# nschloe/flow

Measured on AMD Instinct MI355X. Metric: ipcs_time_steps_per_sec, higher is better.
Workload: dtype f64

## Files before the change

flow_amd/_hip.py:

```python
import ctypes
import os

import torch

from . import device

_HERE = os.path.dirname(os.path.abspath(__file__))
LIB_PATH = os.path.join(_HERE, 'csrc', 'libflow_hip.so')

REDUCE_WORK = 4096
MULTI_DOT_BLOCKS = 1024
GMRES_MAX_RESTART = 30
GMRES_PARTIALS = (GMRES_MAX_RESTART + 2) * 1024
GMRES_STATE = 1280
SPMV_ROWS_PER_BLOCK = 256
SPMV_NNZ_PER_BLOCK = 1022
PMG_NNZ_PER_BLOCK = 2044

c_double_p = ctypes.c_void_p
c_int_p = ctypes.c_void_p


class Operator(ctypes.Structure):
    _fields_ = [
# ... 38 lines not shown
        ('n', ctypes.c_int),
        ('nc', ctypes.c_int),
        ('agg_ptr', ctypes.c_void_p),
        ('agg_dofs', ctypes.c_void_p),
        ('agg_of', ctypes.c_void_p),
        ('lda', ctypes.c_int),
        ('Ainv', ctypes.c_void_p),
        ]


MG_MAX_LEVELS = 8


class MgS(ctypes.Structure):
    _fields_ = [
        ('nlevels', ctypes.c_int),
        ('Ah', Operator * MG_MAX_LEVELS),
        ('dinv', ctypes.c_void_p * MG_MAX_LEVELS),
        ('Ps', Operator * MG_MAX_LEVELS),
        ('R', Operator * MG_MAX_LEVELS),
        ('r', ctypes.c_void_p * MG_MAX_LEVELS),
        ('x', ctypes.c_void_p * MG_MAX_LEVELS),
        ('t', ctypes.c_void_p * MG_MAX_LEVELS),
        ('nc', ctypes.c_int), ('lda', ctypes.c_int),
        ('Ainv', ctypes.c_void_p),
        ('omega', ctypes.c_double),
        ('C', Operator * MG_MAX_LEVELS),
        ('up_rowblocks', ctypes.c_void_p * MG_MAX_LEVELS),
        ('up_nblocks', ctypes.c_int * MG_MAX_LEVELS),
        ]


class IluPlanS(ctypes.Structure):
    _fields_ = [
        ('n', ctypes.c_int), ('nnz', ctypes.c_int), ('ncolors', ctypes.c_int),
        ('nnz_l', ctypes.c_int), ('nnz_u', ctypes.c_int),
        ('off_l', ctypes.c_int), ('off_u', ctypes.c_int),
        ('off_d', ctypes.c_int), ('lu_size', ctypes.c_int),
        ('max_row', ctypes.c_int), ('nslices', ctypes.c_int),
        ('color_ptr_host', ctypes.c_void_p),
        ('slice_ptr_host', ctypes.c_void_p),
        ('rowptr', ctypes.c_void_p), ('cols', ctypes.c_void_p),
        ('diag', ctypes.c_void_p), ('src_pos', ctypes.c_void_p),
        ('old_of_new', ctypes.c_void_p), ('new_of_old', ctypes.c_void_p),
        ('slice_row', ctypes.c_void_p),
        ('l_slice_off', ctypes.c_void_p), ('l_cols', ctypes.c_void_p),
        ('l_pos', ctypes.c_void_p),
        ('u_slice_off', ctypes.c_void_p), ('u_cols', ctypes.c_void_p),
        ('u_pos', ctypes.c_void_p),
        ]


class IluS(ctypes.Structure):
    _fields_ = [
        ('plan', ctypes.POINTER(IluPlanS)),
        ('nblocks', ctypes.c_int),
        ('lu', ctypes.c_void_p),
        ('packed', ctypes.c_void_p),
        ('single_vector', ctypes.c_int),
        ('cycle', ctypes.c_void_p),
        ]


class TlS(ctypes.Structure):
    _fields_ = [
        ('fine', ctypes.POINTER(IluS)), ('coarse', ctypes.POINTER(IluS)),
        ('fine_op', ctypes.c_void_p), ('coarse_op', ctypes.c_void_p),
        ('pre', ctypes.c_int), ('post', ctypes.c_int),
        ('coarse_sweeps', ctypes.c_int),
        ('ends', ctypes.c_void_p), ('rptr', ctypes.c_void_p),
        ('rsrc', ctypes.c_void_p),
        ('bc_fine', ctypes.c_void_p), ('bc_coarse', ctypes.c_void_p),
        ('rscale', ctypes.c_void_p), ('work', ctypes.c_void_p),
        ]


class PmgLevelS(ctypes.Structure):
    _fields_ = [
        ('n', ctypes.c_int), ('nnz', ctypes.c_int), ('nblocks', ctypes.c_int),
        ('rowptr', ctypes.c_void_p), ('cols', ctypes.c_void_p),
        ('rowblocks', ctypes.c_void_p),
        ('vals', ctypes.c_void_p), ('diag', ctypes.c_void_p),
        ('dinv', ctypes.c_void_p),
        ('lam_min', ctypes.c_double), ('lam_max', ctypes.c_double),
        ('cols16', ctypes.c_void_p), ('cbase', ctypes.c_void_p),
        ('packed', ctypes.c_void_p), ('idrows', ctypes.c_void_p),
        ]


class PmgS(ctypes.Structure):
    _fields_ = [
        ('fine', PmgLevelS), ('coarse', PmgLevelS),
        ('pre', ctypes.c_int), ('post', ctypes.c_int),
        ('coarse_steps', ctypes.c_int),
        ('ends', ctypes.c_void_p),
        ('rptr', ctypes.c_void_p), ('rsrc', ctypes.c_void_p),
        ('bc_fine', ctypes.c_void_p), ('bc_coarse', ctypes.c_void_p),
        ('work', ctypes.c_void_p),
        ('scalar', ctypes.c_int),
        ]


class MassS(ctypes.Structure):
    _fields_ = [
        ('A', ctypes.POINTER(Operator)),
        ('dinv', ctypes.c_void_p),
        ('nblocks16', ctypes.c_int),
        ('rowblocks16', ctypes.c_void_p),
        ('vals16', ctypes.c_void_p),
        ('lam_min', ctypes.c_double), ('lam_max', ctypes.c_double),
        ('steps', ctypes.c_int),
        ('contraction', ctypes.c_double),
        ('work16', ctypes.c_void_p),
        ('packed16', ctypes.c_void_p),
        ('cbase16', ctypes.c_void_p),
        ('work16_rows', ctypes.c_int),
        ]


class MassStripsS(ctypes.Structure):
    _fields_ = [
        ('nlevels', ctypes.c_int),
        ('rowblocks16', ctypes.c_void_p * 16),
        ('nblocks16', ctypes.c_int * 16),
        ('row_lo_last', ctypes.c_int), ('row_hi_last', ctypes.c_int),
        ]


class MeshS(ctypes.Structure):
    _fields_ = [('nc', ctypes.c_int), ('xy', ctypes.c_void_p),
                ('c0', ctypes.c_int), ('c1', ctypes.c_int)]


class SpaceS(ctypes.Structure):
    _fields_ = [
        ('deg', ctypes.c_int),
        ('n', ctypes.c_int),
        ('nnz', ctypes.c_int),
        ('cell_dofs', ctypes.c_void_p),
        ('cptr', ctypes.c_void_p),
        ('csrc', ctypes.c_void_p),
        ('vptr', ctypes.c_void_p),
        ('vsrc', ctypes.c_void_p),
        ('r0', ctypes.c_int), ('r1', ctypes.c_int),
        ('nnz0', ctypes.c_int), ('nnz1', ctypes.c_int),
        ]


class CoefS(ctypes.Structure):
    _fields_ = [
        ('nl', ctypes.c_int),
        ('cell_stride', ctypes.c_int),
        ('values', ctypes.c_void_p),
        ('G', ctypes.c_void_p),
        ]


FORM_MAX_PROGRAM = 64
FORM_REGISTERS = 8
FORM_MAX_CONSTANTS = 32
FORM_MAX_FIELDS = 6
FORM_MAX_EXPRESSIONS = 4
FORM_MAX_POINTS = 256
FORM_SLOTS = 9
FORM_NEWTON_SLOTS = 12
PROFILE_CURVES_PER_LAUNCH = 32


class FormS(ctypes.Structure):
    _fields_ = [
        ('nprog', ctypes.c_int),
        ('prog', ctypes.c_int * (4 * FORM_MAX_PROGRAM)),
        ('nconst', ctypes.c_int),
        ('consts', ctypes.c_double * FORM_MAX_CONSTANTS),
        ('nfield', ctypes.c_int),
        ('field', ctypes.c_void_p * FORM_MAX_FIELDS),
        ('field_deg', ctypes.c_int * FORM_MAX_FIELDS),
        ('cell_dofs', ctypes.c_void_p * 2),
        ('nexpr', ctypes.c_int),
        ('expr', ctypes.c_void_p * FORM_MAX_EXPRESSIONS),
        ('expr_nl', ctypes.c_int * FORM_MAX_EXPRESSIONS),
        ('expr_table', ctypes.c_int * FORM_MAX_EXPRESSIONS),
        ('nq', ctypes.c_int),
        ('rule', ctypes.c_void_p),
        ('tables', ctypes.c_void_p),
        ('ntables', ctypes.c_int),
        ('nout', ctypes.c_int),
        ]


class PointGridS(ctypes.Structure):
    _fields_ = [
        ('nx', ctypes.c_int), ('ny', ctypes.c_int),
        ('x0', ctypes.c_double), ('y0', ctypes.c_double),
        ('hx_inv', ctypes.c_double), ('hy_inv', ctypes.c_double),
        ('start', ctypes.c_void_p),
        ('cells', ctypes.c_void_p),
        ]


STATS_MAX_FREQ = 8
STATS_COVARIANCE = 1
STATS_EXTREMA = 2


class StatsFreq(ctypes.Structure):
    _fields_ = [
        ('n', ctypes.c_int),
        ('c', ctypes.c_double * STATS_MAX_FREQ),
        ('s', ctypes.c_double * STATS_MAX_FREQ),
        ]


ISOLINE_LEVELS_PER_LAUNCH = 32


class IsolineLevels(ctypes.Structure):
    _fields_ = [
        ('n', ctypes.c_int),
        ('base', ctypes.c_int),
        ('c', ctypes.c_double * ISOLINE_LEVELS_PER_LAUNCH),
        ]


class NsParams(ctypes.Structure):
    _fields_ = [
        ('dt', ctypes.c_double), ('rho', ctypes.c_double),
        ('mu', ctypes.c_double), ('theta_i', ctypes.c_double),
        ('theta_e', ctypes.c_double),
        ]


ALLREDUCE_FN = ctypes.CFUNCTYPE(ctypes.c_int, ctypes.c_void_p, ctypes.c_int)


class PeerS(ctypes.Structure):
    _fields_ = [
        ('flags', ctypes.c_void_p), ('land', ctypes.c_void_p),
        ('land_cap', ctypes.c_int), ('spin_limit', ctypes.c_int),
        ('nb_flags', ctypes.c_void_p * 2), ('nb_land', ctypes.c_void_p * 2),
        ('seq_host', ctypes.POINTER(ctypes.c_ulonglong * 5)),
        ]


PEER_FLAGS = 16


class CommS(ctypes.Structure):
    _fields_ = [
        ('rank', ctypes.c_int), ('world', ctypes.c_int),
        ('buf', ctypes.c_void_p), ('capacity', ctypes.c_int),
        ('allreduce', ALLREDUCE_FN), ('user', ctypes.c_void_p),
        ('peer', ctypes.POINTER(PeerS)),
        ]


class RcclBinding(ctypes.Structure):
    _fields_ = [('comm', ctypes.c_void_p), ('buf', ctypes.c_void_p),
                ('stream', ctypes.c_void_p)]


class RowsS(ctypes.Structure):
    _fields_ = [
        ('n', ctypes.c_int), ('r0', ctypes.c_int), ('r1', ctypes.c_int),
        ('e0', ctypes.c_int), ('e1', ctypes.c_int), ('nhalo', ctypes.c_int),
        ('send_row', ctypes.c_int * 2), ('send_len', ctypes.c_int * 2),
        ('send_slot', ctypes.c_int * 2),
        ('recv_row', ctypes.c_int * 2), ('recv_len', ctypes.c_int * 2),
        ('recv_slot', ctypes.c_int * 2),
        ]


class MgShardS(ctypes.Structure):
    _fields_ = [
        ('mg', ctypes.POINTER(MgS)),
        ('Ah0', Operator), ('Ps0', Operator), ('Rg', Operator),
        ('Cg', Operator),
        ('up_rowblocks0', ctypes.c_void_p), ('up_nblocks0', ctypes.c_int),
        ('z_lo', ctypes.c_int), ('z_hi', ctypes.c_int),
        ]


class MomentumJvp(ctypes.Structure):
    _fields_ = [
        ('mesh', ctypes.POINTER(MeshS)),
        ('W', ctypes.POINTER(SpaceS)),
        ('bfmask', ctypes.c_void_p),
        ('ui', ctypes.c_void_p),
        ('prm', NsParams),
        ('scratch', ctypes.c_void_p),
        ('nbc', ctypes.c_int),
        ('bc_dofs', ctypes.c_void_p),
        ('bc_mask', ctypes.c_void_p),
        ]


_VP = ctypes.c_void_p
_I = ctypes.c_int
_D = ctypes.c_double
_P = ctypes.POINTER
SYMBOLS = {
    'flow_abi_version': [],
    'flow_launch_count': [_P(ctypes.c_ulonglong)],
    'flow_graph_mode': [_I, ctypes.c_longlong],
    'flow_graph_stats': [_P(ctypes.c_ulonglong)],
    'flow_xcd_tile_host': [_I, _I],
    'flow_spmv_tile_nnz': [_I],
    'flow_operator_apply': [_P(Operator), _VP, _VP, _VP],
    'flow_profile_spmv_begin': [_I, _I],
    'flow_profile_spmv_end': [_P(_D), _P(_I)],
    'flow_profile_event_overhead': [_P(_D), _VP],
    'flow_profile_marker': [_I, _VP],
    'flow_profile_stream_copy': [ctypes.c_size_t, _VP, _VP, _VP],
    'flow_profile_stream_read': [ctypes.c_size_t, _VP, _VP, _VP],
    'flow_operator_diag_inv': [_P(Operator), _VP, _VP, _VP],
    'flow_dot_host': [_I, _VP, _VP, _VP, _P(_D), _VP],
    'flow_norm_host': [_I, _VP, _I, _VP, _P(_D), _VP],
    'flow_axpby': [_I, _D, _VP, _D, _VP, _VP],
    'flow_vmul': [_I, _D, _VP, _VP, _VP, _VP],
    'flow_fill': [_I, _D, _VP, _VP],
    'flow_lincomb': [_I, _I, _P(_D), _P(_VP), _VP, _VP],
    'flow_fingerprint': [_I, _P(_VP), _P(_I), _VP, _VP, _VP],
    'flow_read_doubles': [_VP, _I, _P(_D), _VP],
    'flow_extrapolation_weights': [_I, _P(_D), _D, _I, _I, _P(_D)],
    'flow_scale_rows': [_I, _VP, _VP, _VP, _VP],
    'flow_cg_solve': [_P(Operator), _VP, _P(CoarseS), _P(MgS), _VP, _VP, _D, _D,
                      _I, _I, _I, _VP, ctypes.c_size_t, _P(_I), _P(_D), _VP],
    'flow_cg_solve_guarded': [_P(Operator), _VP, _P(CoarseS), _P(MgS), _VP, _VP,
                              _VP, _D, _D, _I, _I, _I, _VP, ctypes.c_size_t,
                              _P(_I), _P(_D), _P(_I), _VP],
    'flow_mg_apply': [_P(MgS), _I, _VP, _VP, _VP],
    'flow_two_level_apply': [_P(CoarseS), _VP, _VP, _VP, _VP, _VP],
    'flow_bicgstab_solve': [_P(Operator), _VP, _P(IluS), _VP, _VP, _D, _D, _I,
                            _I, _I, _VP, ctypes.c_size_t, _P(_I), _P(_D), _VP],
    'flow_gmres_solve': [_P(Operator), _VP, _P(IluS), _P(PmgS), _VP, _VP, _D,
                         _D, _I, _I, _I, _I, _I, _VP, ctypes.c_size_t, _P(_I),
                         _P(_D), _VP],
    'flow_pmg_pack': [_I, _I, _VP, _VP, _VP, _VP, _VP, _VP, _VP, _VP, _VP],
    'flow_pmg_pack1': [_I, _I, _I, _VP, _VP, _VP, _VP, _VP, _VP, _VP, _VP, _VP,
                       _VP, _VP, _VP, _VP],
    'flow_pmg_cols16': [_I, _VP, _VP, _VP, _VP, _VP, _VP, _VP],
    'flow_pmg_lambda_max': [_P(PmgLevelS), _I, _VP, _VP, _VP, _P(_D), _VP],
    'flow_pmg_apply': [_P(PmgS), _VP, _VP, _VP],
    'flow_tl_apply': [_P(TlS), _VP, _VP, _VP],
    'flow_aggregate_host': [_I, _VP, _VP, _VP, ctypes.c_double, _VP, _VP,
                            _P(ctypes.c_int)],
    'flow_peer_alloc': [ctypes.c_int, _P(ctypes.c_void_p), ctypes.c_char_p],
    'flow_peer_open': [ctypes.c_char_p, _P(ctypes.c_void_p)],
    'flow_peer_close': [_VP],
    'flow_peer_free': [_VP],
    'flow_peer_status': [_P(PeerS), _P(ctypes.c_ulonglong), _VP],
    'flow_mass_pack': [_I, _VP, _VP, _VP, _VP, _VP],
    'flow_mass_pack16': [_I, _I, _VP, _VP, _VP, _VP, _VP, _VP, _VP, _VP, _VP],
    'flow_mass_solve': [_P(MassS), _VP, _VP, _D, _D, _I, _I, _VP,
                        ctypes.c_size_t, _P(_I), _P(_D), _VP],
    'flow_mass_solve_increment': [_P(MassS), _VP, _VP, _VP, _VP, _D, _D, _I, _I, _VP,
                                  ctypes.c_size_t, _P(_I), _P(_D), _VP],
    'flow_gather_rows': [_I, _VP, _I, _VP, _I, _VP, _I, _VP],
    'flow_color_greedy_host': [_I, _VP, _VP, _VP, _P(_I)],
    'flow_color_iterate_host': [_I, _VP, _VP, _VP, _P(_I), _I],
    'flow_ilu0_factor': [_P(IluPlanS), _I, _VP, _VP, _VP, _VP],
    'flow_ilu0_pack': [_P(IluS), _VP, _VP],
    'flow_ilu0_solve': [_P(IluS), _VP, _VP, _VP, _VP],
    'flow_rccl_load': [ctypes.c_char_p],
    'flow_rccl_unique_id': [_VP],
    'flow_rccl_comm_create': [_VP, _I, _I, _P(_VP)],
    'flow_rccl_comm_destroy': [_VP],
    'flow_rccl_allreduce': [_VP, _I],
    'flow_shard_halo': [_P(CommS), _P(RowsS), _I, _VP, _I, _VP],
    'flow_shard_reduce_host': [_P(CommS), _P(RowsS), _I, _VP, _VP, _I, _I, _VP,
                               _P(_D), _VP],
    'flow_shard_cg_solve': [_P(CommS), _P(RowsS), _P(Operator), _VP, _VP, _VP,
                            _D, _D, _I, _I, _I, _VP, ctypes.c_size_t, _P(_I),
                            _P(_D), _P(_I), _VP],
    'flow_shard_mgcg_solve': [_P(CommS), _P(RowsS), _P(Operator), _VP,
                              _P(MgShardS), _VP, _VP, _D, _D, _I, _I, _I, _VP,
                              ctypes.c_size_t, _P(_I), _P(_D), _P(_I), _VP],
    'flow_shard_mass_solve': [_P(CommS), _P(RowsS), _P(MassS), _P(MassStripsS),
                              _VP, _VP, _VP, _VP, _D, _D, _I, _I, _VP,
                              ctypes.c_size_t, _P(_I), _P(_D), _VP],
    'flow_shard_gmres_solve': [_P(CommS), _P(RowsS), _P(Operator), _P(IluS),
                               _P(PmgS), _VP, _VP, _D, _D, _I, _I, _I, _I, _I,
                               _VP, ctypes.c_size_t, _P(_I), _P(_D), _VP],
    'flow_assemble_scalar_matrix': [_I, _P(MeshS), _P(SpaceS), _VP, _VP, _VP],
    'flow_assemble_pressure_rhs': [_P(MeshS), _P(SpaceS), _P(SpaceS), _VP, _VP,
                                   _D, _D, _I, _VP, _VP, _VP],
    'flow_assemble_correction_rhs': [_P(MeshS), _P(SpaceS), _P(SpaceS), _VP,
                                     _VP, _VP, _D, _D, _I, _VP, _VP, _VP],
    'flow_assemble_momentum': [_P(MeshS), _P(SpaceS), _P(SpaceS), _VP, _VP, _VP,
                               _VP, _P(CoefS), _P(CoefS), _P(NsParams), _VP,
                               _VP, _VP, ctypes.c_size_t, _VP],
    'flow_momentum_jvp_apply': [_P(MomentumJvp), _VP, _VP, _VP],
    'flow_assemble_source': [_P(MeshS), _P(SpaceS), _I, _P(CoefS), _VP, _VP,
                             _VP],
    'flow_assemble_magnitude': [_P(MeshS), _P(SpaceS), _I, _VP, _VP, _VP, _VP],
    'flow_assemble_div_adjoint': [_P(MeshS), _P(SpaceS), _P(SpaceS), _VP, _VP,
                                  _VP, _VP],
    'flow_bc_identity_rows': [_P(Operator), _VP, _VP, _I, _VP, _VP],
    'flow_bc_residual': [_I, _VP, _VP, _VP, _VP, _VP],
    'flow_bc_set_values': [_I, _VP, _VP, _VP, _VP],
    'flow_bc_symmetric_matrix': [_I, _VP, _VP, _VP, _VP, _VP, _VP],
    'flow_assemble_heat': [_P(MeshS), _P(SpaceS), _P(SpaceS), _VP, _D, _D, _I,
                           _VP, _VP, _VP, _VP, _VP, _VP],
    'flow_supg_tau': [_P(MeshS), _P(SpaceS), _VP, _D, _I, _VP, _VP, _VP],
    'flow_assemble_heat_supg_source': [_P(MeshS), _P(SpaceS), _P(SpaceS), _VP,
                                       _D, _D, _P(CoefS), _VP, _VP, _VP, _VP],
    'flow_form_functional': [_P(MeshS), _P(FormS), _VP, _VP, _P(_D), _VP],
    'flow_form_cell_values': [_P(MeshS), _P(FormS), _VP, _VP],
    'flow_form_load_vector': [_P(MeshS), _P(SpaceS), _P(FormS), _VP, _VP, _VP],
    'flow_form_matrix': [_P(MeshS), _P(SpaceS), _P(FormS), _VP, _VP, _VP],
    'flow_form_vector': [_P(MeshS), _P(SpaceS), _P(FormS), _VP, _VP, _VP],
    'flow_form_newton': [_P(MeshS), _P(SpaceS), _P(FormS), _VP, _VP, _VP,
                         _VP],
    'flow_form_facet_functional': [_P(MeshS), _P(FormS), _I, _VP, _VP, _VP, _VP,
                                   _P(_D), _VP],
    'flow_form_facet_values': [_P(MeshS), _P(FormS), _I, _VP, _VP, _VP, _VP,
                               _VP, _VP, _VP],
    'flow_form_interior_facet_functional': [_P(MeshS), _P(FormS), _I, _VP, _VP,
                                            _VP, _VP, _VP, _P(_D), _VP],
    'flow_form_interior_facet_values': [_P(MeshS), _P(FormS), _I, _VP, _VP,
                                        _VP, _VP, _VP],
    'flow_facet_cell_shares': [_P(MeshS), _I, _VP, _VP, _D, _VP, _VP],
    'flow_form_facet_matrix': [_P(MeshS), _P(SpaceS), _P(FormS), _I, _VP, _VP,
                               _I, _VP, _VP, _VP, _VP, _VP, _VP],
    'flow_form_facet_vector': [_P(MeshS), _P(SpaceS), _P(FormS), _I, _VP, _VP,
                               _I, _VP, _VP, _VP, _VP, _VP, _VP],
    'flow_form_cells_functional': [_P(MeshS), _P(FormS), _I, _VP, _VP, _VP,
                                   _P(_D), _VP],
    'flow_form_cells_values': [_P(MeshS), _P(FormS), _I, _VP, _VP, _VP],
    'flow_form_cells_matrix': [_P(MeshS), _P(SpaceS), _P(FormS), _I, _VP, _I,
                               _VP, _VP, _VP, _VP, _VP, _VP],
    'flow_form_cells_vector': [_P(MeshS), _P(SpaceS), _P(FormS), _I, _VP, _I,
                               _VP, _VP, _VP, _VP, _VP, _VP],
    'flow_form_rect_matrix': [_P(MeshS), _P(SpaceS), _P(SpaceS), _P(FormS),
                              _VP, _VP, _VP, _VP, _I, _VP],
    'flow_form_rect_facet_matrix': [_P(MeshS), _P(SpaceS), _P(SpaceS),
                                    _P(FormS), _I, _VP, _VP, _I, _VP, _VP,
                                    _VP, _VP, _VP, _I, _VP],
    'flow_form_rect_cells_matrix': [_P(MeshS), _P(SpaceS), _P(SpaceS),
                                    _P(FormS), _I, _VP, _I, _VP, _VP, _VP,
                                    _VP, _VP, _I, _VP],
    'flow_bc_rect_mask': [_VP, _VP, _I, _VP, _VP, _VP, _VP],
    'flow_plane_symmetric_part': [_I, _VP, _VP, _I, _VP, _VP, _VP],
    'flow_form_block_matrix': [_P(MeshS), _P(SpaceS), _I, _P(FormS), _P(_I),
                               _VP, _VP, ctypes.c_size_t, _VP],
    'flow_form_block_vector': [_P(MeshS), _P(SpaceS), _I, _P(FormS), _P(_I),
                               _VP, _VP, _VP],
    'flow_form_block_newton': [_P(MeshS), _P(SpaceS), _I, _P(FormS), _P(_I),
                               _P(_I), _VP, ctypes.c_size_t, _VP,
                               ctypes.c_size_t, _VP, _VP],
    'flow_bc_symmetric_blocks': [_I, _I, _VP, _VP, _VP, ctypes.c_size_t, _VP,
                                 _VP, ctypes.c_size_t, _VP],
    'flow_profile_cumsum': [_I, _P(_I), _I, _I, _VP, _VP, _VP],
    'flow_locate_points': [_P(MeshS), _P(PointGridS), _I, _VP, _VP, _VP, _VP],
    'flow_form_points': [_P(MeshS), _P(FormS), _I, _VP, _VP, _VP, _VP],
    'flow_advect_points': [_P(MeshS), _P(PointGridS), _P(SpaceS), _VP, _VP, _I,
                           _VP, _VP, _VP, _D, _I, _I, _VP],
    'flow_nearest_cells': [_P(MeshS), _P(PointGridS), _I, _VP, _VP, _I, _VP,
                           _VP, _VP, _VP, _VP],
    'flow_transfer_apply': [_P(SpaceS), _I, _I, _VP, _VP, _VP, _VP, _VP],
    'flow_project_load': [_P(MeshS), _P(SpaceS), _P(MeshS), _P(SpaceS), _I, _VP,
                          _VP, _I, _VP, _I, _VP, _VP, _VP, _VP],
    'flow_supermesh_norms': [_P(MeshS), _P(SpaceS), _P(MeshS), _P(SpaceS), _I,
                             _VP, _VP, _I, _VP, _VP, _I, _VP, _VP, _P(_D), _VP],
    'flow_jump_indicator': [_P(MeshS), _P(SpaceS), _I, _VP, _VP, _VP, _VP],
    'flow_recover_gradient': [_P(MeshS), _P(SpaceS), _I, _VP, _VP, _VP],
    'flow_zz_indicator': [_P(MeshS), _P(SpaceS), _I, _VP, _VP, _I, _VP, _VP,
                          _VP],
    'flow_distance_sweeps': [_P(MeshS), _P(SpaceS), _I, _VP, _VP, _VP, _VP],
    'flow_isoline_count': [_P(MeshS), _P(SpaceS), _VP, _P(IsolineLevels), _VP,
                           _VP],
    'flow_isoline_emit': [_P(MeshS), _P(SpaceS), _VP, _P(IsolineLevels), _VP,
                          _VP, _I, _VP, _VP, _VP, _VP, _VP, _VP],
    'flow_isoline_measure': [_P(MeshS), _P(SpaceS), _VP, _P(IsolineLevels),
                             _VP, _VP, _VP],
    'flow_region_init': [_P(SpaceS), _VP, _D, _I, _VP, _VP],
    'flow_region_sweeps': [_P(MeshS), _P(SpaceS), _I, _VP, _VP, _VP, _VP],
    'flow_region_moments': [_P(MeshS), _P(SpaceS), _VP, _D, _VP, _P(SpaceS), _I,
                            _VP, _VP, _VP, _VP],
    'flow_region_segment_sum': [_I, _VP, _VP, _I, _I, _VP, _VP, _VP],
    'flow_region_segment_minmax': [_I, _VP, _VP, _I, _I, _VP, _VP, _VP, _VP],
    'flow_multi_dot': [_I, _I, _VP, ctypes.c_size_t, _VP, _VP, _VP, _VP],
    'flow_combine': [_I, _I, _VP, ctypes.c_size_t, _I, _VP, _VP, _VP,
                     ctypes.c_size_t, _VP],
    'flow_operator_apply_block': [_P(Operator), _I, _VP, ctypes.c_size_t, _VP,
                                  ctypes.c_size_t, _VP],
    'flow_operator_apply_block_chunk': [_P(Operator), _I, _VP, ctypes.c_size_t,
                                        _VP, ctypes.c_size_t, _I, _VP],
    'flow_block_gram': [_I, _I, _VP, ctypes.c_size_t, _I, _VP, ctypes.c_size_t,
                        _VP, _VP, _VP],
    'flow_mixed_apply': [_P(MixedS), _VP, _VP, _VP],
    'flow_stats_update': [_I, _I, _I, _P(StatsFreq), _D, _D, _D, _VP, _VP,
                          ctypes.c_size_t, _VP],
    'flow_stats_merge': [_I, _I, _I, _I, _D, _D, _VP, _VP, ctypes.c_size_t,
                         _VP],
    }

_LIB = None


class HipError(RuntimeError):
    pass


class NotConverged(RuntimeError):
    '''Krylov / Newton non-convergence.  A RuntimeError, because callers of the
    reference catch exactly that (tests/test_boussinesq.py:254).'''


ABI_VERSION = 30


def load_library():
    global _LIB
    if _LIB is None:
        if not os.path.isfile(LIB_PATH):
            raise HipError(
                'libflow_hip.so not found at %s -- build it with '
                '`python -c "import __graft_entry__ as g; g.build()"` or '
                '`make -C flow_amd/csrc`' % LIB_PATH
                )
        lib = ctypes.CDLL(LIB_PATH)
        lib.flow_last_error.restype = ctypes.c_char_p
        lib.flow_last_error.argtypes = []
        for name, argtypes in SYMBOLS.items():
            fn = getattr(lib, name)
            fn.restype = ctypes.c_int
            fn.argtypes = argtypes
        got = lib.flow_abi_version()
        if got != ABI_VERSION:
            raise HipError(
                '%s is ABI version %d, these bindings are version %d: '
                'rebuild it (`make -C flow_amd/csrc`)'
                % (LIB_PATH, got, ABI_VERSION))
        _LIB = lib
    return _LIB


def launch_count():
    n = ctypes.c_ulonglong(0)
    check(load_library().flow_launch_count(ctypes.byref(n)))
    return int(n.value)


_GRAPHS = {'mode': None}


def graph_mode(mode, auto_rows=-1, sites=0):
    check(load_library().flow_graph_mode(int(mode) | (int(sites) << 4),
                                         int(auto_rows)))
    _GRAPHS['mode'] = int(mode)


def graphs_possible():
    if _GRAPHS['mode'] is not None:
        return _GRAPHS['mode'] != 0
    return os.environ.get('FLOW_AMD_GRAPHS', '0') not in ('', '0')


def graph_stats():
    v = (ctypes.c_ulonglong * 8)()
    check(load_library().flow_graph_stats(v))
    return {'graphs': int(v[0]), 'captures': int(v[1]), 'replays': int(v[2]),
            'nodes': int(v[3]), 'captures_cg': int(v[4]),
            'captures_gmres': int(v[5]), 'captures_mass': int(v[6])}


def spmv_tile_nnz(kind=0):
    return int(load_library().flow_spmv_tile_nnz(int(kind)))


def lib():
    handle = load_library()
    if not device.on_gpu():
        raise HipError(
            'flow_amd needs an AMD GPU (MI355X): the hot path has no CPU '
            'fallback'
            )
    return handle


def check(rc):
    if rc == 0:
        return
    msg = load_library().flow_last_error().decode('utf-8', 'replace')
    if rc == 1:
        raise NotConverged(msg)
    if rc == 2:
        raise ValueError(msg)
    raise HipError(msg)


def _ptr(t, dtype, numel=None, name='operand'):
    if t is None:
        return None
    if not isinstance(t, torch.Tensor):
        raise TypeError('%s: expected a torch tensor' % name)
    if t.dtype != dtype:
        raise TypeError('%s: dtype %s, expected %s' % (name, t.dtype, dtype))
    if not t.is_cuda:
        raise HipError('%s is not in device memory' % name)
    if not t.is_contiguous():
        raise ValueError('%s is not contiguous' % name)
    if numel is not None and t.numel() < numel:
        raise ValueError(
            '%s has %d elements, needs %d' % (name, t.numel(), numel)
            )
    return ctypes.c_void_p(t.data_ptr())


def f64(t, numel=None, name='fp64 operand'):
    return _ptr(t, torch.float64, numel, name)


def f32(t, numel=None, name='fp32 operand'):
    return _ptr(t, torch.float32, numel, name)


def f16(t, numel=None, name='fp16 operand'):
    return _ptr(t, torch.float16, numel, name)


def i32(t, numel=None, name='int32 operand'):
    return _ptr(t, torch.int32, numel, name)


def u8(t, numel=None, name='uint8 operand'):
    return _ptr(t, torch.uint8, numel, name)


def stream():
    return ctypes.c_void_p(device.stream_handle())


def copy(dst, src):
    assert dst.numel() == src.numel()
    if not dst.is_cuda:
        dst.copy_(src)
    elif dst.data_ptr() != src.data_ptr():
        check(lib().flow_axpby(dst.numel(), 1.0, f64(src, name='src'), 0.0,
                               f64(dst, name='dst'), stream()))
    return dst


def fill(t, value=0.0):
    if not t.is_cuda:
        t.fill_(float(value))
    elif t.numel() > 0:
        check(lib().flow_fill(t.numel(), float(value), f64(t), stream()))
    return t


def clone(t):
    out = torch.empty_like(t)
    return copy(out, t)
```

flow_amd/csrc/common.h:

```cpp
#pragma once
#include <hip/hip_runtime.h>

#include <algorithm>
#include <cstdarg>
#include <cstdio>
#include <functional>
#include <vector>

#include "../../include/flow_hip.h"

namespace flow {
extern unsigned long long g_launches;
}
#undef hipLaunchKernelGGL
#define hipLaunchKernelGGL(kernelName, numBlocks, numThreads, memPerBlock,        \
                           streamId, ...)                                       \
  do {                                                                          \
    ++flow::g_launches;                                                         \
    (kernelName)<<<(numBlocks), (numThreads), (memPerBlock), (streamId)>>>(     \
        __VA_ARGS__);                                                           \
  } while (0)

namespace flow {

void set_error(const char* fmt, ...);

inline hipStream_t as_stream(void* s) { return static_cast<hipStream_t>(s); }

int ilu_apply(const flow_ilu* ilu, const double* in, double* out, double* work,
              hipStream_t st, const double* stop = nullptr);
int ilu_check(const flow_ilu* ilu, int op_size);

int pmg_apply(const flow_pmg* M, const double* r, double* z, hipStream_t st,
              const double* stop = nullptr);
int pmg_check(const flow_pmg* M, int op_size);
int tl_apply(const flow_tl* T, const double* r, double* z, hipStream_t st,
             const double* stop = nullptr);
int tl_check(const flow_tl* T, int op_size);
int operator_apply(const flow_operator* A, const double* x, double* y,
                   hipStream_t st, const double* stop = nullptr);
int operator_size(const flow_operator* A);
int sum_partials_host(double* work, int nparts, double* host, hipStream_t st);
int check_operator(const flow_operator* A);
int fill(int n, double value, double* y, hipStream_t st);
struct NoEarly {
  __device__ __forceinline__ void operator()(int, bool) const {}
};

enum Slot {
  kGamma = 0, kAlpha, kBeta, kRes2, kB2, kRho, kOmega, kRhoNew, kTmp,
  kBreak, kTarget2, kDone, kConvIt, kIter, kNumSlots = 16
};
int read_state(const double* S, double* host, hipStream_t st);
int check_comm(const flow_comm* c, long long need);
int check_rows(const flow_rows* R);
int exchange(const flow_comm* c, int count);
int exchange_halo(const flow_comm* C, const flow_rows* R, int ncomp, int sum_count,
                  int hoff, hipStream_t st);

int gather(int nout, int nplanes, const int* ptr, const int* src,
           const double* scratch, size_t plane_stride, double* out,
           hipStream_t st, size_t out_stride = 0, int r0 = 0, int r1 = 0,
           const double* stop = nullptr, const unsigned char* idrow = nullptr,
           const double* v = nullptr, size_t v_stride = 0);
int momentum_jvp_check(const flow_momentum_jvp* J);
int momentum_jvp_apply(const flow_momentum_jvp* J, const double* v, double* out,
                       hipStream_t st, int v_stride = 0, int out_stride = 0,
                       const double* stop = nullptr,
                       const double* prm_dev = nullptr);
int momentum_jvp_params(const flow_momentum_jvp* J, double* dst, hipStream_t st);

constexpr long long kReplayAutoRows = 1500000;
struct KeyHash {
  unsigned long long h = 1469598103934665603ull;
  void bytes(const void* p, size_t n) {
    const unsigned char* c = static_cast<const unsigned char*>(p);
    for (size_t i = 0; i < n; ++i) h = (h ^ c[i]) * 1099511628211ull;
  }
  template <class T> KeyHash& pod(const T& v) {
    bytes(&v, sizeof(T));
    return *this;
  }
  template <class T> KeyHash& obj(const T* p) {
    const unsigned char tag = p ? 1 : 0;
    bytes(&tag, 1);
    if (p) bytes(p, sizeof(T));
    return *this;
  }
};
enum ReplaySite { kReplayCg = 1, kReplayGmres = 2, kReplayMass = 4 };
bool replay_wanted(long long rows, int site);
int replay_prepare(unsigned long long key, int site, hipStream_t st,
                   const std::function<int()>& body, hipGraphExec_t* exec,
                   int* nodes);
int replay_launch(hipGraphExec_t exec, int nodes, hipStream_t st);
void key_operator(KeyHash& k, const flow_operator* A, bool skip_prm = false);

#define FLOW_CHECK_HIP(expr)                                                 \
  do {                                                                       \
    hipError_t err_ = (expr);                                                \
    if (err_ != hipSuccess) {                                                \
      flow::set_error("%s failed: %s (%s:%d)", #expr, hipGetErrorString(err_), \
                      __FILE__, __LINE__);                                   \
      return FLOW_HIP_ERROR;                                                 \
    }                                                                        \
  } while (0)

#define FLOW_REQUIRE(cond, msg)                                  \
  do {                                                           \
    if (!(cond)) {                                               \
      flow::set_error("invalid argument: %s (%s)", msg, #cond);  \
      return FLOW_INVALID;                                       \
    }                                                            \
  } while (0)

#define FLOW_CHECK_LAUNCH() FLOW_CHECK_HIP(hipGetLastError())

constexpr int kBlock = 256;
constexpr int kRedBlocks = 1024;
constexpr int kMaxGrid = 2048;

inline int grid_for(long long n, int per_block = kBlock, int cap = kMaxGrid) {
  long long g = (n + per_block - 1) / per_block;
  if (g < 1) g = 1;
  if (g > cap) g = cap;
  return static_cast<int>(g);
}

__device__ __forceinline__ double load_scalar(const double* p) {
  return __hip_atomic_load(const_cast<double*>(p), __ATOMIC_RELAXED,
                           __HIP_MEMORY_SCOPE_SYSTEM);
}
__device__ __forceinline__ void store_scalar(double* p, double v) {
  __hip_atomic_store(p, v, __ATOMIC_RELAXED, __HIP_MEMORY_SCOPE_SYSTEM);
}

__device__ __forceinline__ bool stopped(const double* stop) {
  return stop != nullptr && load_scalar(stop) != 0.0;
}

constexpr int kXcdRun = 64;
__host__ __device__ __forceinline__ int xcd_tile(int b, int nwg) {
  constexpr int kGroup = 8 * kXcdRun;
  const int full = (nwg / kGroup) * kGroup;
  if (b < full) {
    const int g = b / kGroup, i = b - g * kGroup;
    return g * kGroup + (i & 7) * kXcdRun + (i >> 3);
  }
  const int nt = nwg - full, i = b - full;
  const int q = nt >> 3, r = nt & 7, xcd = i & 7;
  return full + (xcd < r ? xcd * (q + 1) : r * (q + 1) + (xcd - r) * q) +
         (i >> 3);
}

__device__ inline double block_sum(double v) {
  __shared__ double wave_part[4];
#pragma unroll
  for (int off = 32; off > 0; off >>= 1) v += __shfl_down(v, off, 64);
  const int lane = threadIdx.x & 63;
  const int wave = threadIdx.x >> 6;
  __syncthreads();
  if (lane == 0) wave_part[wave] = v;
  __syncthreads();
  if (threadIdx.x == 0) v = wave_part[0] + wave_part[1] + wave_part[2] + wave_part[3];
  return v;
}

__device__ inline double block_sum_once(double v) {
  __shared__ double wave_part_once[4];
#pragma unroll
  for (int off = 32; off > 0; off >>= 1) v += __shfl_down(v, off, 64);
  if ((threadIdx.x & 63) == 0) wave_part_once[threadIdx.x >> 6] = v;
  __syncthreads();
  if (threadIdx.x == 0)
    v = wave_part_once[0] + wave_part_once[1] + wave_part_once[2] +
        wave_part_once[3];
  return v;
}

__device__ inline double block_max(double v) {
  __shared__ double wave_part_m[4];
#pragma unroll
  for (int off = 32; off > 0; off >>= 1) v = fmax(v, __shfl_down(v, off, 64));
  const int lane = threadIdx.x & 63;
  const int wave = threadIdx.x >> 6;
  __syncthreads();
  if (lane == 0) wave_part_m[wave] = v;
  __syncthreads();
  if (threadIdx.x == 0)
    v = fmax(fmax(wave_part_m[0], wave_part_m[1]), fmax(wave_part_m[2], wave_part_m[3]));
  return v;
}

}
```

flow_amd/csrc/krylov_kernels.hip:

```cpp
#include "common.h"
#include "csr_stream.h"
#include "la_internal.h"

namespace flow {

template <int UP, bool DOTS>
__global__ __launch_bounds__(kBlock) void mg_level_kernel(
    const int* __restrict__ rowptr, const int* __restrict__ cols,
    const double* __restrict__ vals, const int* __restrict__ rowblocks,
    const double* __restrict__ x, const double* __restrict__ c,
    const double* __restrict__ t, const double* __restrict__ dinv, double omega,
    double* __restrict__ y, double* __restrict__ gpart,
    double* __restrict__ rpart, const double* __restrict__ stop) {
  __shared__ double prod[kTile];
  if (stopped(stop)) return;
  int r, r1;
  const double s =
      stream_tile_row_sum(rowptr, cols, vals, rowblocks, x, prod, r, r1);
  double g = 0.0, rr = 0.0;
  if (r < r1) {
    const double ci = c[r];
    if (UP) {
      const double yi = s + omega * dinv[r] * (ci + t[r]);
      y[r] = yi;
      if (DOTS) {
        g = ci * yi;
        rr = yi * yi;
      }
    } else {
      y[r] = ci - s;
    }
  }
  if (DOTS) {
    g = block_sum(g);
    rr = block_sum(rr);
    if (threadIdx.x == 0) {
      gpart[blockIdx.x] = g;
      rpart[blockIdx.x] = rr;
    }
  }
}

template <bool DOTS>
__global__ __launch_bounds__(kBlock) void mg_up2_kernel(
    const int* __restrict__ rowblocks, const int* __restrict__ p_rowptr,
    const int* __restrict__ p_cols, const double* __restrict__ p_vals,
    const int* __restrict__ a_rowptr, const int* __restrict__ a_cols,
    const double* __restrict__ a_vals, const double* __restrict__ xc,
    const double* __restrict__ c, const double* __restrict__ dinv, double omega,
    double* __restrict__ y, double* __restrict__ gpart,
    double* __restrict__ rpart, const double* __restrict__ stop,
    int own_lo, int own_hi) {
  __shared__ double prod_p[kTile];
  __shared__ double prod_a[kTile];
  if (stopped(stop)) return;
  const int tile = xcd_tile(blockIdx.x, gridDim.x);
  const int r0 = rowblocks[tile];
  const int r1 = rowblocks[tile + 1];
  const int r = r0 + threadIdx.x;
  double ci = 0.0, di = 0.0;
  if (r < r1) {
    ci = c[r];
    di = dinv[r];
  }
  const double sp = stream_rows_sum(r0, r1, p_rowptr, p_cols, p_vals, xc, prod_p);
  const double sa = stream_rows_sum(r0, r1, a_rowptr, a_cols, a_vals, c, prod_a);
  double g = 0.0, rr = 0.0;
  if (r < r1) {
    const double yi = sp + omega * di * (2.0 * ci - sa);
    y[r] = yi;
    if (DOTS && r >= own_lo && r < own_hi) {
      g = ci * yi;
      rr = yi * yi;
    }
  }
  if (DOTS) {
    g = block_sum(g);
    rr = block_sum(rr);
    if (threadIdx.x == 0) {
      gpart[blockIdx.x] = g;
      rpart[blockIdx.x] = rr;
    }
  }
}

__global__ __launch_bounds__(kScalarBlock) void cg_scalar_kernel(
    int nparts, int ndelta, int first, const double* __restrict__ gpart,
    const double* __restrict__ rpart, const double* __restrict__ dpart,
    double rtol2, double atol2, double* __restrict__ S) {
  __shared__ double wsum[3][kScalarBlock / 64];
  if (stopped(S + kDone)) return;
  double g = 0.0, rr = 0.0;
  for (int i = threadIdx.x; i < nparts; i += kScalarBlock) {
    g += load_scalar(gpart + i);
    rr += load_scalar(rpart + i);
  }
  double d0 = 0.0, d1 = 0.0, d2 = 0.0, d3 = 0.0;
  int i = threadIdx.x;
  for (; i + 3 * kScalarBlock < ndelta; i += 4 * kScalarBlock) {
    d0 += load_scalar(dpart + i);
    d1 += load_scalar(dpart + i + kScalarBlock);
    d2 += load_scalar(dpart + i + 2 * kScalarBlock);
    d3 += load_scalar(dpart + i + 3 * kScalarBlock);
  }
  for (; i < ndelta; i += kScalarBlock) d0 += load_scalar(dpart + i);
  double d = (d0 + d1) + (d2 + d3);
#pragma unroll
  for (int off = 32; off > 0; off >>= 1) {
    g += __shfl_down(g, off, 64);
    d += __shfl_down(d, off, 64);
    rr += __shfl_down(rr, off, 64);
  }
  if ((threadIdx.x & 63) == 0) {
    wsum[0][threadIdx.x >> 6] = g;
    wsum[1][threadIdx.x >> 6] = d;
    wsum[2][threadIdx.x >> 6] = rr;
  }
  __syncthreads();
  if (threadIdx.x == 0) {
    g = d = rr = 0.0;
    for (int w = 0; w < kScalarBlock / 64; ++w) {
      g += wsum[0][w];
      d += wsum[1][w];
      rr += wsum[2][w];
    }
  }
  if (threadIdx.x == 0) {
    double alpha, beta;
    if (first) {
      beta = 0.0;
      alpha = (d != 0.0) ? g / d : 0.0;
      const double b2 = load_scalar(S + kB2);
      store_scalar(S + kTarget2, fmax(rtol2 * b2, atol2));
      store_scalar(S + kIter, 0.0);
      if (first == 2 && rr > b2) {
        store_scalar(S + kConvIt, 0.0);
        store_scalar(S + kRes2, rr);
        store_scalar(S + kDone, 5.0);
        return;
      }
    } else {
      const double g_old = load_scalar(S + kGamma);
      const double a_old = load_scalar(S + kAlpha);
      beta = (g_old != 0.0) ? g / g_old : 0.0;
      const double den = (a_old != 0.0) ? d - beta * g / a_old : 0.0;
      alpha = (den != 0.0) ? g / den : 0.0;
    }
    const double k = load_scalar(S + kIter);
    const bool nan = !(rr == rr);
    if (nan || rr <= load_scalar(S + kTarget2)) {
      store_scalar(S + kConvIt, k);
      store_scalar(S + kDone, nan ? 2.0 : 1.0);
      alpha = beta = 0.0;
    }
    store_scalar(S + kIter, k + 1.0);
    store_scalar(S + kGamma, g);
    store_scalar(S + kAlpha, alpha);
    store_scalar(S + kBeta, beta);
    store_scalar(S + kRes2, rr);
  }
}

template <bool DOTS>
__global__ __launch_bounds__(kBlock) void cg_update_kernel(
    int n, const double* __restrict__ S, const double* __restrict__ dinv,
    const double* __restrict__ w, double* __restrict__ z, double* __restrict__ p,
    double* __restrict__ s, double* __restrict__ x, double* __restrict__ r,
    int want_z, double* __restrict__ partial,
    const double* __restrict__ own) {
  if (stopped(S + kDone)) return;
  const double alpha = load_scalar(S + kAlpha);
  const double beta = load_scalar(S + kBeta);
  double g = 0.0, rr = 0.0;
  for (int i = blockIdx.x * blockDim.x + threadIdx.x; i < n;
       i += gridDim.x * blockDim.x) {
    const double pi = z[i] + beta * p[i];
    const double si = w[i] + beta * s[i];
    p[i] = pi;
    s[i] = si;
    x[i] += alpha * pi;
    const double ri = r[i] - alpha * si;
    r[i] = ri;
    if (want_z) {
      const double zi = dinv ? dinv[i] * ri : ri;
      z[i] = zi;
      if (DOTS && (!own || own[i] != 0.0)) {
        g += ri * zi;
        rr += zi * zi;
      }
    }
  }
  if (DOTS) {
    g = block_sum(g);
    rr = block_sum(rr);
    if (threadIdx.x == 0) {
      partial[blockIdx.x] = g;
      partial[2 * kRedBlocks + blockIdx.x] = rr;
    }
  }
}

FLOW_KRYLOV_INSTANCES(template)

__global__ __launch_bounds__(kBlock) void coarse_restrict_kernel(
    int nc, const int* __restrict__ agg_ptr, const int* __restrict__ agg_dofs,
    const double* __restrict__ r, int r0, int r1, double* __restrict__ rc,
    const double* __restrict__ stop) {
  if (stopped(stop)) return;
  const int lane = threadIdx.x & 63;
  for (int a = blockIdx.x * 4 + (threadIdx.x >> 6); a < nc; a += gridDim.x * 4) {
    double sum = 0.0;
    for (int k = agg_ptr[a] + lane; k < agg_ptr[a + 1]; k += 64) {
      const int d = agg_dofs[k];
      if (d >= r0 && d < r1) sum += r[d];
    }
#pragma unroll
    for (int off = 32; off > 0; off >>= 1) sum += __shfl_down(sum, off, 64);
    if (lane == 0) rc[a] = sum;
  }
}

__global__ __launch_bounds__(kBlock) void coarse_gemv_kernel(
    int nc, int lda, const float* __restrict__ Ainv,
    const double* __restrict__ rc, double* __restrict__ zc,
    const double* __restrict__ stop) {
  if (stopped(stop)) return;
  const int lane = threadIdx.x & 63;
  const int nq = lda >> 2;
  for (int row = blockIdx.x * 4 + (threadIdx.x >> 6); row < nc;
       row += gridDim.x * 4) {
    const float4* __restrict__ a =
        reinterpret_cast<const float4*>(Ainv + static_cast<size_t>(row) * lda);
    const double2* __restrict__ x = reinterpret_cast<const double2*>(rc);
    double s0 = 0.0, s1 = 0.0;
    for (int q = lane; q < nq; q += 64) {
      const float4 v = a[q];
      double2 x0, x1;
      if (4 * q + 3 < nc) {
        x0 = x[2 * q];
        x1 = x[2 * q + 1];
      } else {
        const int j = 4 * q;
        x0.x = rc[j];
        x0.y = (j + 1 < nc) ? rc[j + 1] : 0.0;
        x1.x = (j + 2 < nc) ? rc[j + 2] : 0.0;
        x1.y = 0.0;
      }
      s0 += static_cast<double>(v.x) * x0.x + static_cast<double>(v.z) * x1.x;
      s1 += static_cast<double>(v.y) * x0.y + static_cast<double>(v.w) * x1.y;
    }
    double sum = s0 + s1;
#pragma unroll
    for (int off = 32; off > 0; off >>= 1) sum += __shfl_down(sum, off, 64);
    if (lane == 0) zc[row] = sum;
  }
}

template <bool DOTS>
__global__ __launch_bounds__(kBlock) void coarse_prolong_kernel(
    int n, const int* __restrict__ agg_of, const double* __restrict__ dinv,
    const double* __restrict__ r, const double* __restrict__ zc,
    double* __restrict__ z, double* __restrict__ partial,
    const double* __restrict__ stop) {
  if (stopped(stop)) return;
  double g = 0.0, rr = 0.0;
  for (int i = blockIdx.x * blockDim.x + threadIdx.x; i < n;
       i += gridDim.x * blockDim.x) {
    const int a = agg_of[i];
    const double ri = r[i];
    const double zi = dinv[i] * ri + (a >= 0 ? zc[a] : 0.0);
    z[i] = zi;
    if (DOTS) {
      g += ri * zi;
      rr += zi * zi;
    }
  }
  if (DOTS) {
    g = block_sum(g);
    rr = block_sum(rr);
    if (threadIdx.x == 0) {
      partial[blockIdx.x] = g;
      partial[2 * kRedBlocks + blockIdx.x] = rr;
    }
  }
}

static int check_coarse(const flow_coarse* C, int n) {
  FLOW_REQUIRE(C->nc > 0 && C->n == n, "coarse space size");
  FLOW_REQUIRE(C->agg_ptr && C->agg_dofs && C->agg_of && C->Ainv,
               "coarse space pointers");
  FLOW_REQUIRE(C->lda >= C->nc && C->lda % 4 == 0 &&
                   reinterpret_cast<uintptr_t>(C->Ainv) % 16 == 0,
               "coarse inverse: row stride must be a multiple of 4 floats, "
               "base 16-byte aligned");
  return FLOW_OK;
}

static int two_level(const flow_coarse* C, const double* dinv, const double* r,
                     double* z, double* rc, double* zc, hipStream_t st,
                     double* partial = nullptr, int* nparts = nullptr,
                     const double* stop = nullptr) {
  const int g = grid_for(C->nc, 4, kMaxGrid);
  hipLaunchKernelGGL(coarse_restrict_kernel, dim3(g), dim3(kBlock), 0, st, C->nc,
                     C->agg_ptr, C->agg_dofs, r, 0, C->n, rc, stop);
  hipLaunchKernelGGL(coarse_gemv_kernel, dim3(g), dim3(kBlock), 0, st, C->nc,
                     C->lda, C->Ainv, rc, zc, stop);
  if (partial) {
    const int gp = grid_for(C->n, kBlock, kRedBlocks);
    hipLaunchKernelGGL(coarse_prolong_kernel<true>, dim3(gp), dim3(kBlock), 0,
                       st, C->n, C->agg_of, dinv, r, zc, z, partial, stop);
    *nparts = gp;
  } else {
    hipLaunchKernelGGL(coarse_prolong_kernel<false>, dim3(grid_for(C->n)),
                       dim3(kBlock), 0, st, C->n, C->agg_of, dinv, r, zc, z,
                       partial, stop);
  }
  FLOW_CHECK_LAUNCH();
  return FLOW_OK;
}

int check_mg(const flow_mg* M, int n) {
  FLOW_REQUIRE(M->nlevels >= 1 && M->nlevels <= FLOW_MG_MAX_LEVELS, "mg levels");
  FLOW_REQUIRE(M->omega > 0.0 && M->omega < 2.0, "mg damping");
  int rows = n;
  for (int l = 0; l + 1 < M->nlevels; ++l) {
    int rc = check_operator(&M->Ah[l]);
    if (rc) return rc;
    if ((rc = check_operator(&M->Ps[l]))) return rc;
    if ((rc = check_operator(&M->R[l]))) return rc;
    FLOW_REQUIRE(M->Ah[l].kind == 0 && M->Ps[l].kind == 0 && M->R[l].kind == 0,
                 "mg operators are scalar");
    FLOW_REQUIRE(M->Ah[l].n == rows && M->Ps[l].n == rows, "mg level sizes");
    FLOW_REQUIRE(M->dinv[l] && M->t[l], "mg level vectors");
    FLOW_REQUIRE(l == 0 || (M->r[l] && M->x[l]), "mg level vectors");
    if (M->C[0].rowptr) {
      if ((rc = check_operator(&M->C[l]))) return rc;
      FLOW_REQUIRE(M->C[l].kind == 0 && M->C[l].n == M->R[l].n &&
                       M->up_rowblocks[l] && M->up_nblocks[l] > 0,
                   "mg two-launch form: C and the common row blocks");
    }
    rows = M->R[l].n;
  }
  const int last = M->nlevels - 1;
  FLOW_REQUIRE(M->nc == rows && M->Ainv && M->lda >= M->nc && M->lda % 4 == 0 &&
                   reinterpret_cast<uintptr_t>(M->Ainv) % 16 == 0,
               "mg coarsest level");
  FLOW_REQUIRE(last == 0 || (M->r[last] && M->x[last] &&
                             reinterpret_cast<uintptr_t>(M->r[last]) % 16 == 0),
               "mg coarsest vectors");
  return FLOW_OK;
}

int vcycle(const flow_mg* M, const double* r0, double* z0, hipStream_t st,
           double* gpart, double* rpart, int* nparts, const double* stop,
           int l0) {
  const int L = M->nlevels;
  int rc;
  double* const none = nullptr;
  const bool fused = M->C[0].rowptr != nullptr;
  for (int l = l0; l + 1 < L; ++l) {
    const double* r = l == l0 ? r0 : M->r[l];
    if (fused) {
      if ((rc = apply(&M->C[l], r, M->r[l + 1], st, nullptr, stop))) return rc;
      continue;
    }
    const flow_operator* A = &M->Ah[l];
    hipLaunchKernelGGL((mg_level_kernel<0, false>), dim3(A->nblocks), dim3(kBlock),
                       0, st, A->rowptr, A->cols, A->vals[0], A->rowblocks, r, r,
                       none, none, M->omega, M->t[l], none, none, stop);
    if ((rc = apply(&M->R[l], M->t[l], M->r[l + 1], st, nullptr, stop)))
      return rc;
  }
  {
    const double* r = l0 == L - 1 ? r0 : M->r[L - 1];
    double* x = l0 == L - 1 ? z0 : M->x[L - 1];
    hipLaunchKernelGGL(coarse_gemv_kernel, dim3(grid_for(M->nc, 4, kMaxGrid)),
                       dim3(kBlock), 0, st, M->nc, M->lda, M->Ainv, r, x, stop);
  }
  for (int l = L - 2; l >= l0; --l) {
    const double* r = l == l0 ? r0 : M->r[l];
    double* x = l == l0 ? z0 : M->x[l];
    const flow_operator* P = &M->Ps[l];
    const bool with_dots = l == 0 && gpart;
    if (fused) {
      const flow_operator* A = &M->Ah[l];
      const dim3 grid(M->up_nblocks[l]);
      if (with_dots)
        hipLaunchKernelGGL(mg_up2_kernel<true>, grid, dim3(kBlock), 0, st,
                           M->up_rowblocks[l], P->rowptr, P->cols, P->vals[0],
                           A->rowptr, A->cols, A->vals[0], M->x[l + 1], r,
                           M->dinv[l], M->omega, x, gpart, rpart, stop);
      else
        hipLaunchKernelGGL(mg_up2_kernel<false>, grid, dim3(kBlock), 0, st,
                           M->up_rowblocks[l], P->rowptr, P->cols, P->vals[0],
                           A->rowptr, A->cols, A->vals[0], M->x[l + 1], r,
                           M->dinv[l], M->omega, x, none, none, stop);
      if (with_dots) *nparts = M->up_nblocks[l];
      continue;
    }
    if (with_dots) {
      hipLaunchKernelGGL((mg_level_kernel<1, true>), dim3(P->nblocks),
                         dim3(kBlock), 0, st, P->rowptr, P->cols, P->vals[0],
                         P->rowblocks, M->x[l + 1], r, M->t[l], M->dinv[l],
                         M->omega, x, gpart, rpart, stop);
      *nparts = P->nblocks;
    } else {
      hipLaunchKernelGGL((mg_level_kernel<1, false>), dim3(P->nblocks),
                         dim3(kBlock), 0, st, P->rowptr, P->cols, P->vals[0],
                         P->rowblocks, M->x[l + 1], r, M->t[l], M->dinv[l],
                         M->omega, x, none, none, stop);
    }
  }
  FLOW_CHECK_LAUNCH();
  return FLOW_OK;
}

static inline int mg_parts(const flow_mg* M) {
  if (!M || M->nlevels < 2) return 0;
  return M->C[0].rowptr ? M->up_nblocks[0] : M->Ps[0].nblocks;
}

static inline size_t cg_work_len(const flow_operator* A, const flow_coarse* C,
                                 const flow_mg* M) {
  const size_t N = op_size(A);
  return FLOW_REDUCE_WORK + 5 * N + dot_parts(A) + 2 +
         (C ? 2 * static_cast<size_t>(C->lda) : 0) +
         2 * static_cast<size_t>(mg_parts(M));
}

static int run_batches(const char* solver, const char* norm, int maxit,
                       int first_check, int check_every, const double* S,
                       hipStream_t st, bool* rejected,
                       const std::function<int(int)>& iteration,
                       int* iters_host, double* resid_host) {
  if (rejected) *rejected = false;
  double state[kNumSlots];
  int launched = 0, rc;
  while (true) {
    const int batch = (launched == 0 && first_check > 0) ? first_check
                                                         : check_every;
    const int todo = (maxit - launched < batch) ? maxit - launched : batch;
    for (int k = 0; k < todo; ++k)
      if ((rc = iteration(launched + k))) return rc;
    FLOW_CHECK_LAUNCH();
    launched += todo;
    if ((rc = read_state(S, state, st))) return rc;
    const double res2 = state[kRes2];
    if (state[kDone] == 2.0 || !(res2 == res2)) {
      *iters_host = static_cast<int>(state[kConvIt]);
      *resid_host = res2;
      set_error("%s broke down (NaN residual) at iteration %d", solver,
                *iters_host);
      return FLOW_NOT_CONVERGED;
    }
    if (state[kDone] == 1.0) {
      *iters_host = static_cast<int>(state[kConvIt]);
      *resid_host = sqrt(res2);
      return FLOW_OK;
    }
    if (state[kDone] == 5.0 && rejected) {
      *rejected = true;
      *iters_host = 0;
      *resid_host = sqrt(res2);
      return FLOW_OK;
    }
    if (launched >= maxit) {
      *iters_host = launched;
      *resid_host = sqrt(res2);
      set_error("%s did not converge in %d iterations: %s = %.3e > %.3e", solver,
                launched, norm, sqrt(res2), sqrt(state[kTarget2]));
      return FLOW_NOT_CONVERGED;
    }
  }
}

static int cg(const flow_operator* A, const double* dinv,
              const flow_coarse* C, const flow_mg* M, const double* b,
              double* x, double rtol, double atol, int maxit, int check_every,
              int first_check, double* work, int* iters_host,
              double* resid_host, hipStream_t st, bool* rejected = nullptr) {
  const int N = op_size(A);
  const int nd = dot_parts(A);
  double* partial = work;
  double* S = work + 3 * kRedBlocks;
  double* r = work + FLOW_REDUCE_WORK;
  double* z = r + N;
  double* w = z + N;
  double* p = w + N;
  double* s = p + N;
  double* dpart = s + N;
  double* crc = dpart + nd + ((N + nd) & 1);
  double* czc = crc + (C ? C->lda : 0);
  double* mpart = czc + (C ? C->lda : 0);
  const int nm = mg_parts(M);
  const double* gpart = M ? mpart : partial;
  const double* rpart = M ? mpart + nm : partial + 2 * kRedBlocks;
  const int gv = grid_for(N);
  const int gu = grid_for(N, kBlock, kRedBlocks);
  int np = 0, rc;

  const double* stop = S + kDone;
  double* const r_ = r;
  const double rtol2 = rtol * rtol, atol2 = atol * atol;
  if ((rc = fill(kNumSlots, 0.0, S, st))) return rc;
  if ((rc = fill(2 * N, 0.0, p, st))) return rc;
  if (C) {
    if ((rc = two_level(C, dinv, b, z, crc, czc, st))) return rc;
  } else if (M) {
    if ((rc = vcycle(M, b, z, st))) return rc;
  } else if (dinv) {
    hipLaunchKernelGGL(vmul_kernel, dim3(gv), dim3(kBlock), 0, st, N, 1.0, dinv,
                       b, z);
  }
  const double* Bb = (C || M || dinv) ? z : b;
  if ((rc = dots(N, 1, Bb, Bb, Bb, Bb, Bb, Bb, partial, &np, st))) return rc;
  hipLaunchKernelGGL(finish_kernel, dim3(1), dim3(kBlock), 0, st, np, 1, 0,
                     partial, S + kB2);
  if ((rc = apply(A, x, w, st))) return rc;
  hipLaunchKernelGGL(residual_kernel, dim3(gv), dim3(kBlock), 0, st, N, b, w,
                     dinv, r, z);
  if (C && (rc = two_level(C, dinv, r, z, crc, czc, st))) return rc;
  if (M && (rc = vcycle(M, r, z, st))) return rc;
  if ((rc = apply(A, z, w, st, dpart))) return rc;
  if ((rc = dots(N, 3, r, z, z, w, z, z, partial, &np, st))) return rc;
  hipLaunchKernelGGL(cg_scalar_kernel, dim3(1), dim3(kScalarBlock), 0, st, np,
                     nd, rejected ? 2 : 1, partial, partial + 2 * kRedBlocks,
                     dpart, rtol2, atol2, S);
  FLOW_CHECK_LAUNCH();

  auto body = [&]() -> int {
    int r;
    if (C) {
      hipLaunchKernelGGL(cg_update_kernel<false>, dim3(gv), dim3(kBlock), 0,
                         st, N, S, dinv, w, z, p, s, x, r_, 0, partial,
                         static_cast<const double*>(nullptr));
      if ((r = two_level(C, dinv, r_, z, crc, czc, st, partial, &np, stop)))
        return r;
    } else if (M) {
      hipLaunchKernelGGL(cg_update_kernel<false>, dim3(gv), dim3(kBlock), 0,
                         st, N, S, dinv, w, z, p, s, x, r_, 0, partial,
                         static_cast<const double*>(nullptr));
      if ((r = vcycle(M, r_, z, st, mpart, mpart + nm, &np, stop))) return r;
    } else {
      hipLaunchKernelGGL(cg_update_kernel<true>, dim3(gu), dim3(kBlock), 0, st,
                         N, S, dinv, w, z, p, s, x, r_, 1, partial,
                         static_cast<const double*>(nullptr));
      np = gu;
    }
    if ((r = apply(A, z, w, st, dpart, stop))) return r;
    hipLaunchKernelGGL(cg_scalar_kernel, dim3(1), dim3(kScalarBlock), 0, st,
                       np, nd, 0, gpart, rpart, dpart, 0.0, 0.0, S);
    FLOW_CHECK_LAUNCH();
    return FLOW_OK;
  };
  hipGraphExec_t graph = nullptr;
  int graph_nodes = 0;
  if (replay_wanted(N, kReplayCg) && g_spmv_profile.ev == nullptr) {
    KeyHash key;
    key.pod(0x6367ull);
    key_operator(key, A);
    key.obj(C).obj(M).pod(dinv).pod(x).pod(work).pod(N);
    if ((rc = replay_prepare(key.h, kReplayCg, st, body, &graph, &graph_nodes))) return rc;
  }

  return run_batches(
      "CG", "|B r|", maxit, first_check, check_every, S, st, rejected,
      [&](int) { return graph ? replay_launch(graph, graph_nodes, st) : body(); },
      iters_host, resid_host);
}

__global__ __launch_bounds__(kBlock) void bicg_scalar_kernel(
    int nparts, int mode, int first, double rtol2, double atol2,
    const double* __restrict__ partial, double* __restrict__ S) {
  if (stopped(S + kDone)) return;
  double a = 0.0, b = 0.0;
  for (int i = threadIdx.x; i < nparts; i += kBlock) {
    a += load_scalar(partial + i);
    b += load_scalar(partial + kRedBlocks + i);
  }
  a = block_sum(a);
  b = block_sum(b);
  if (threadIdx.x != 0) return;
  if (mode == 1) {
    store_scalar(S + kAlpha, (a != 0.0) ? load_scalar(S + kRhoNew) / a : 0.0);
    if (a == 0.0) store_scalar(S + kBreak, 1.0);
  } else if (mode == 2) {
    store_scalar(S + kOmega, (b != 0.0) ? a / b : 0.0);
  } else {
    const double rho_old = load_scalar(S + kRhoNew);
    const double omega = load_scalar(S + kOmega);
    const double alpha = load_scalar(S + kAlpha);
    store_scalar(S + kRho, rho_old);
    store_scalar(S + kRhoNew, a);
    store_scalar(S + kRes2, b);
    store_scalar(S + kBeta, (rho_old != 0.0 && omega != 0.0)
                                ? (a / rho_old) * (alpha / omega)
                                : 0.0);
    if (first) {
      store_scalar(S + kTarget2, fmax(rtol2 * load_scalar(S + kB2), atol2));
      store_scalar(S + kIter, 0.0);
    }
    const double k = load_scalar(S + kIter);
    const bool nan = !(b == b);
    if (nan || b <= load_scalar(S + kTarget2)) {
      store_scalar(S + kConvIt, k);
      store_scalar(S + kDone, nan ? 2.0 : 1.0);
    }
    store_scalar(S + kIter, k + 1.0);
  }
}

__global__ void bicg_p_kernel(int n, const double* __restrict__ S,
                              const double* __restrict__ dinv,
                              const double* __restrict__ r,
                              const double* __restrict__ v,
                              double* __restrict__ p, double* __restrict__ y) {
  if (stopped(S + kDone)) return;
  const double beta = load_scalar(S + kBeta);
  const double omega = load_scalar(S + kOmega);
  for (int i = blockIdx.x * blockDim.x + threadIdx.x; i < n;
       i += gridDim.x * blockDim.x) {
    const double pi = r[i] + beta * (p[i] - omega * v[i]);
    p[i] = pi;
    y[i] = dinv ? dinv[i] * pi : pi;
  }
}

__global__ void bicg_s_kernel(int n, const double* __restrict__ S,
                              const double* __restrict__ dinv,
                              const double* __restrict__ v,
                              double* __restrict__ r, double* __restrict__ z) {
  if (stopped(S + kDone)) return;
  const double alpha = load_scalar(S + kAlpha);
  for (int i = blockIdx.x * blockDim.x + threadIdx.x; i < n;
       i += gridDim.x * blockDim.x) {
    const double si = r[i] - alpha * v[i];
    r[i] = si;
    z[i] = dinv ? dinv[i] * si : si;
  }
}

__global__ void bicg_x_kernel(int n, const double* __restrict__ S,
                              const double* __restrict__ y,
                              const double* __restrict__ z,
                              const double* __restrict__ t,
                              double* __restrict__ x, double* __restrict__ r) {
  if (stopped(S + kDone)) return;
  const double alpha = load_scalar(S + kAlpha);
  const double omega = load_scalar(S + kOmega);
  for (int i = blockIdx.x * blockDim.x + threadIdx.x; i < n;
       i += gridDim.x * blockDim.x) {
    x[i] += alpha * y[i] + omega * z[i];
    r[i] -= omega * t[i];
  }
}

static int bicgstab(const flow_operator* A, const double* dinv,
                    const flow_ilu* ilu, const double* b,
                    double* x, double rtol, double atol, int maxit,
                    int check_every, int first_check, double* work,
                    int* iters_host, double* resid_host, hipStream_t st) {
  const int N = op_size(A);
  double* partial = work;
  double* S = work + 3 * kRedBlocks;
  double* r = work + FLOW_REDUCE_WORK;
  double* rhat = r + N;
  double* p = rhat + N;
  double* v = p + N;
  double* y = v + N;
  double* z = y + N;
  double* t = z + N;
  double* iwork = t + N;
  if (ilu) dinv = nullptr;
  const int gv = grid_for(N);
  int np = 0, rc;

  if ((rc = fill(kNumSlots, 0.0, S, st))) return rc;
  if ((rc = fill(2 * N, 0.0, p, st))) return rc;
  if ((rc = dots(N, 1, b, b, b, b, b, b, partial, &np, st))) return rc;
  hipLaunchKernelGGL(finish_kernel, dim3(1), dim3(kBlock), 0, st, np, 1, 0,
                     partial, S + kB2);
  if ((rc = apply(A, x, t, st))) return rc;
  hipLaunchKernelGGL(residual_kernel, dim3(gv), dim3(kBlock), 0, st, N, b, t,
                     static_cast<const double*>(nullptr), r,
                     static_cast<double*>(nullptr));
  hipLaunchKernelGGL(axpby_kernel, dim3(gv), dim3(kBlock), 0, st, N, 1.0, r, 0.0,
                     rhat);
  const double rtol2 = rtol * rtol, atol2 = atol * atol;
  if ((rc = dots(N, 2, rhat, r, r, r, r, r, partial, &np, st))) return rc;
  hipLaunchKernelGGL(bicg_scalar_kernel, dim3(1), dim3(kBlock), 0, st, np, 3, 1,
                     rtol2, atol2, partial, S);
  FLOW_CHECK_LAUNCH();

  auto body = [&](int) -> int {
    int rc;
    hipLaunchKernelGGL(bicg_p_kernel, dim3(gv), dim3(kBlock), 0, st, N, S, dinv,
                       r, v, p, y);
    if (ilu && (rc = ilu_apply(ilu, p, y, iwork, st))) return rc;
    if ((rc = apply(A, y, v, st))) return rc;
    if ((rc = dots(N, 1, rhat, v, v, v, v, v, partial, &np, st))) return rc;
    hipLaunchKernelGGL(bicg_scalar_kernel, dim3(1), dim3(kBlock), 0, st, np, 1,
                       0, rtol2, atol2, partial, S);
    hipLaunchKernelGGL(bicg_s_kernel, dim3(gv), dim3(kBlock), 0, st, N, S, dinv,
                       v, r, z);
    if (ilu && (rc = ilu_apply(ilu, r, z, iwork, st))) return rc;
    if ((rc = apply(A, z, t, st))) return rc;
    if ((rc = dots(N, 2, t, r, t, t, t, t, partial, &np, st))) return rc;
    hipLaunchKernelGGL(bicg_scalar_kernel, dim3(1), dim3(kBlock), 0, st, np, 2,
                       0, rtol2, atol2, partial, S);
    hipLaunchKernelGGL(bicg_x_kernel, dim3(gv), dim3(kBlock), 0, st, N, S, y, z,
                       t, x, r);
    if ((rc = dots(N, 2, rhat, r, r, r, r, r, partial, &np, st))) return rc;
    hipLaunchKernelGGL(bicg_scalar_kernel, dim3(1), dim3(kBlock), 0, st, np, 3,
                       0, rtol2, atol2, partial, S);
    return FLOW_OK;
  };
  return run_batches("BiCGStab", "|r|", maxit, first_check, check_every, S, st,
                     nullptr, body, iters_host, resid_host);
}

}

using namespace flow;

static_assert((kGmresMax + 2) * kRedBlocks == FLOW_GMRES_PARTIALS, "gmres work");
static_assert(kGmresMax + 2 <= kMailbox, "mailbox size");
struct Coef8 {
  double c[8];
};

template <int NV>
__global__ __launch_bounds__(kBlock) void gmres_dots_kernel(
    int n, const double* __restrict__ w, const double* __restrict__ V,
    size_t stride, int with_ww, double* __restrict__ partial,
    double* __restrict__ ww_partial, const double* __restrict__ stop) {
  if (stopped(stop)) return;
  double acc[NV];
#pragma unroll
  for (int k = 0; k < NV; ++k) acc[k] = 0.0;
  double ww = 0.0;
  for (int i = blockIdx.x * blockDim.x + threadIdx.x; i < n;
       i += gridDim.x * blockDim.x) {
    const double wi = w[i];
#pragma unroll
    for (int k = 0; k < NV; ++k) acc[k] += wi * V[k * stride + i];
    ww += wi * wi;
  }
#pragma unroll
  for (int k = 0; k < NV; ++k) {
    const double a = block_sum(acc[k]);
    if (threadIdx.x == 0) partial[k * kRedBlocks + blockIdx.x] = a;
  }
  if (with_ww) {
    ww = block_sum(ww);
    if (threadIdx.x == 0) ww_partial[blockIdx.x] = ww;
  }
}
#define FLOW_GMRES_DOTS_DEFINE(NV)                                     \
  template __global__ void gmres_dots_kernel<NV>(                      \
      int, const double*, const double*, size_t, int, double*, double*, \
      const double*);
FLOW_GMRES_DOTS_INSTANCES(FLOW_GMRES_DOTS_DEFINE)
#undef FLOW_GMRES_DOTS_DEFINE

template <int NV>
__global__ __launch_bounds__(kBlock) void gmres_combine_kernel(
    int n, Coef8 coef, double cw, int first, const double* w,
    const double* __restrict__ V, size_t stride, double* out,
    double* __restrict__ nn_partial) {
  double nn = 0.0;
  for (int i = blockIdx.x * blockDim.x + threadIdx.x; i < n;
       i += gridDim.x * blockDim.x) {
    double acc = first ? (w ? cw * w[i] : 0.0) : out[i];
#pragma unroll
    for (int k = 0; k < NV; ++k) acc += coef.c[k] * V[k * stride + i];
    out[i] = acc;
    nn += acc * acc;
  }
  if (nn_partial) {
    nn = block_sum(nn);
    if (threadIdx.x == 0) nn_partial[blockIdx.x] = nn;
  }
}

template <int NV>
__global__ __launch_bounds__(kBlock) void gmres_combine_dev_kernel(
    int n, const double* __restrict__ coef, const double* __restrict__ cw,
    int first, const double* w, const double* __restrict__ V, size_t stride,
    double* out, double* __restrict__ nn_partial,
    const double* __restrict__ stop) {
  if (stopped(stop)) return;
  double c[NV];
#pragma unroll
  for (int k = 0; k < NV; ++k) c[k] = load_scalar(coef + k);
  const double c_w = (first && w) ? load_scalar(cw) : 0.0;
  double nn = 0.0;
  for (int i = blockIdx.x * blockDim.x + threadIdx.x; i < n;
       i += gridDim.x * blockDim.x) {
    double acc = first ? (w ? c_w * w[i] : 0.0) : out[i];
#pragma unroll
    for (int k = 0; k < NV; ++k) acc += c[k] * V[k * stride + i];
    out[i] = acc;
    nn += acc * acc;
  }
  if (nn_partial) {
    nn = block_sum(nn);
    if (threadIdx.x == 0) nn_partial[blockIdx.x] = nn;
  }
}


__global__ __launch_bounds__(kBlock) void gmres_step_kernel(
    int nparts, int j, int last, double beta, double target,
    const double* __restrict__ partial, double* __restrict__ G,
    double* __restrict__ S) {
  constexpr int ld = kGmresMax + 1;
  __shared__ double val[kGmresMax + 2];
  __shared__ double Hs[kGmresMax * ld];
  __shared__ double nrm[kGmresMax + 1], eta[kGmresMax];
  __shared__ double g[kGmresMax + 1], cs[kGmresMax], sn[kGmresMax], y[kGmresMax];
  if (stopped(S + kDone)) return;
  if (beta < 0.0) {
    beta = load_scalar(S + kBeta);
    target = load_scalar(S + kTarget2);
  }
  const int nd = j + 1;
  const int nval = nd + 1 + (j > 0 ? 1 : 0);
  const int lane = threadIdx.x & 63;
  if (nparts == 0 && threadIdx.x < nval)
    val[threadIdx.x] = load_scalar(partial + threadIdx.x);
  for (int v = threadIdx.x >> 6; nparts > 0 && v < nval; v += kBlock / 64) {
    const int list = v < nd ? v : kGmresMax + (v - nd);
    const double* __restrict__ p = partial + list * kRedBlocks;
    double s0 = 0.0, s1 = 0.0, s2 = 0.0, s3 = 0.0;
    int i = lane;
    for (; i + 192 < nparts; i += 256) {
      const double a0 = load_scalar(p + i), a1 = load_scalar(p + i + 64);
      const double a2 = load_scalar(p + i + 128), a3 = load_scalar(p + i + 192);
      s0 += a0;
      s1 += a1;
      s2 += a2;
      s3 += a3;
    }
    for (; i < nparts; i += 64) s0 += load_scalar(p + i);
    double s = (s0 + s1) + (s2 + s3);
#pragma unroll
    for (int off = 32; off > 0; off >>= 1) s += __shfl_down(s, off, 64);
    if (lane == 0) val[v] = s;
  }
  for (int i = threadIdx.x; i < j * ld; i += kBlock)
    Hs[i] = load_scalar(G + kGH + i);
  if (threadIdx.x < j) {
    nrm[threadIdx.x] = load_scalar(G + kGNrm + threadIdx.x);
    eta[threadIdx.x] = load_scalar(G + kGEta + threadIdx.x);
    cs[threadIdx.x] = load_scalar(G + kGRot + 2 * threadIdx.x);
    sn[threadIdx.x] = load_scalar(G + kGRot + 2 * threadIdx.x + 1);
    g[threadIdx.x] = load_scalar(G + kGRhs + threadIdx.x);
  }
  __syncthreads();
  if (threadIdx.x != 0) return;
  if (j == 0) {
    nrm[0] = beta;
    g[0] = beta;
  }
  if (j > 0) {
    nrm[j] = sqrt(val[nd + 1]);
    const int c = j - 1;
    Hs[c * ld + j] = eta[c] * nrm[j];
    const double a = Hs[c * ld + c], bsub = Hs[c * ld + c + 1];
    const double d = hypot(a, bsub);
    cs[c] = d > 0.0 ? a / d : 1.0;
    sn[c] = d > 0.0 ? bsub / d : 0.0;
    Hs[c * ld + c] = d;
    G[kGH + c * ld + c] = d;
    G[kGRot + 2 * c] = cs[c];
    G[kGRot + 2 * c + 1] = sn[c];
    const double gc = g[c];
    g[c + 1] = -sn[c] * gc;
    g[c] = cs[c] * gc;
    G[kGRhs + c] = g[c];
  }
  const double nj = nrm[j];
  G[kGNrm + j] = nj;
  const double ww = val[nd] / (nj * nj);
  double sum = 0.0;
  double* col = Hs + j * ld;
  for (int k = 0; k <= j; ++k) {
    const double h = val[k] / (nj * nrm[k]);
    y[k] = h;
    col[k] = h;
    sum += h * h;
  }
  if (!(ww == ww) || !(nj > 0.0)) {
    store_scalar(S + kConvIt, static_cast<double>(j));
    store_scalar(S + kDone, 2.0);
    return;
  }
  const double e2 = ww - sum;
  const bool lucky = !(e2 > 1.0e-12 * ww);
  const double et = e2 > 0.0 ? sqrt(e2) : 0.0;
  G[kGEta + j] = et;
  if (!lucky) {
    const double inv = 1.0 / et;
    for (int k = 0; k <= j; ++k)
      store_scalar(G + kGCoef + k, -y[k] * inv / nrm[k]);
    store_scalar(G + kGCw, inv / nj);
  }
  for (int i = 0; i < j; ++i) {
    const double t = cs[i] * col[i] + sn[i] * col[i + 1];
    col[i + 1] = -sn[i] * col[i] + cs[i] * col[i + 1];
    col[i] = t;
  }
  col[j + 1] = et;
  for (int r = 0; r <= j + 1; ++r) G[kGH + j * ld + r] = col[r];
  G[kGRhs + j] = g[j];
  const double dj = hypot(col[j], et);
  const double csj = dj > 0.0 ? col[j] / dj : 1.0;
  const double snj = dj > 0.0 ? et / dj : 0.0;
  const double resid = fabs(snj * g[j]);
  store_scalar(S + kRes2, resid);
  store_scalar(S + kConvIt, static_cast<double>(j + 1));
  const bool done = resid <= target && !lucky;
  if (done || lucky || last) {
    const int nc = j + 1;
    col[j] = dj;
    g[j] = csj * g[j];
    for (int i = nc - 1; i >= 0; --i) {
      double t = g[i];
      for (int c = i + 1; c < nc; ++c) t -= Hs[c * ld + i] * y[c];
      const double rii = Hs[i * ld + i];
      y[i] = rii != 0.0 ? t / rii : 0.0;
    }
    for (int k = 0; k < nc; ++k) store_scalar(G + kGYc + k, y[k] / nrm[k]);
    if (done) store_scalar(S + kDone, 1.0);
    if (lucky) store_scalar(S + kDone, 3.0);
  }
}

__global__ __launch_bounds__(kBlock) void gmres_begin_kernel(
    int nparts, int have_b2, int first, int accept10, double rtol, double atol,
    const double* __restrict__ partial, double* __restrict__ S) {
  double r = 0.0, b = 0.0;
  for (int i = threadIdx.x; i < nparts; i += kBlock) {
    r += load_scalar(partial + i);
    if (have_b2) b += load_scalar(partial + kRedBlocks + i);
  }
  r = block_sum(r);
  b = block_sum(b);
  if (threadIdx.x != 0) return;
  double target;
  if (first) {
    const double b2 = have_b2 ? b : r;
    target = fmax(rtol * sqrt(b2), atol);
    store_scalar(S + kB2, b2);
    store_scalar(S + kTarget2, target);
    if (have_b2 && r > b2) {
      store_scalar(S + kTmp, 1.0);
      r = b2;
    }
  } else {
    target = load_scalar(S + kTarget2);
  }
  const double beta = sqrt(r);
  store_scalar(S + kBeta, beta);
  store_scalar(S + kRes2, beta);
  store_scalar(S + kConvIt, 0.0);
  if (!(r == r))
    store_scalar(S + kDone, 2.0);
  else if (beta <= target || (accept10 && beta <= 10.0 * target))
    store_scalar(S + kDone, 4.0);
}

__global__ void gmres_drop_start_kernel(int n, const double* __restrict__ S,
                                        const double* __restrict__ b,
                                        double* __restrict__ v0,
                                        double* __restrict__ x) {
  if (load_scalar(S + kTmp) == 0.0) return;
  for (int i = blockIdx.x * blockDim.x + threadIdx.x; i < n;
       i += gridDim.x * blockDim.x) {
    v0[i] = b[i];
    x[i] = 0.0;
  }
}


static int gmres_combine(int N, int nv, const double* c, double cw,
                         const double* w, const double* V, double* out,
                         double* nn_partial, bool accumulate, hipStream_t st) {
  const int g = grid_for(N, kBlock, kRedBlocks);
  if (nv == 0) {
    FLOW_REQUIRE(w != nullptr, "gmres combine");
    Coef8 none = {};
    hipLaunchKernelGGL(gmres_combine_kernel<1>, dim3(g), dim3(kBlock), 0, st, N,
                       none, cw, 1, w, V, static_cast<size_t>(N), out,
                       nn_partial);
  }
  for (int k0 = 0; k0 < nv; k0 += 8) {
    const int chunk = nv - k0 < 8 ? nv - k0 : 8;
    Coef8 coef = {};
    for (int k = 0; k < chunk; ++k) coef.c[k] = c[k0 + k];
    double* nnp = (k0 + 8 >= nv) ? nn_partial : nullptr;
#define FLOW_CALL(NV)                                                          \
  hipLaunchKernelGGL(gmres_combine_kernel<NV>, dim3(g), dim3(kBlock), 0, st, N, \
                     coef, cw, (k0 == 0 && !accumulate) ? 1 : 0, w,            \
                     V + static_cast<size_t>(k0) * N, static_cast<size_t>(N),  \
                     out, nnp)
    FLOW_NV_SWITCH(chunk, FLOW_CALL)
#undef FLOW_CALL
  }
  FLOW_CHECK_LAUNCH();
  return FLOW_OK;
}

int flow::gmres_combine_dev(int N, int nv, const double* coef, const double* cw,
                            const double* w, const double* V, double* out,
                            double* nn_partial, bool accumulate,
                            const double* stop, hipStream_t st) {
  const int g = grid_for(N, kBlock, kRedBlocks);
  for (int k0 = 0; k0 < nv; k0 += 8) {
    const int chunk = nv - k0 < 8 ? nv - k0 : 8;
    double* nnp = (k0 + 8 >= nv) ? nn_partial : nullptr;
#define FLOW_CALL(NV)                                                           \
  hipLaunchKernelGGL(gmres_combine_dev_kernel<NV>, dim3(g), dim3(kBlock), 0, st, \
                     N, coef + k0, cw, (k0 == 0 && !accumulate) ? 1 : 0, w,     \
                     V + static_cast<size_t>(k0) * N, static_cast<size_t>(N),   \
                     out, nnp, stop)
    FLOW_NV_SWITCH(chunk, FLOW_CALL)
#undef FLOW_CALL
  }
  FLOW_CHECK_LAUNCH();
  return FLOW_OK;
}

static void arnoldi_dots(int N, int j, const double* w, const double* V, int gd,
                         double* P, double* Pww, const double* stop,
                         hipStream_t st) {
  for (int k0 = 0; k0 <= j; k0 += 8) {
    const int chunk = j + 1 - k0 < 8 ? j + 1 - k0 : 8;
#define FLOW_CALL(NV)                                                         \
  hipLaunchKernelGGL(gmres_dots_kernel<NV>, dim3(gd), dim3(kBlock), 0, st, N,  \
                     w, V + static_cast<size_t>(k0) * N,                      \
                     static_cast<size_t>(N), k0 == 0 ? 1 : 0,                 \
                     P + k0 * kRedBlocks, Pww, stop)
    FLOW_NV_SWITCH(chunk, FLOW_CALL)
#undef FLOW_CALL
  }
}

static int gmres_cycle(const char* solver, int m, int maxit, int it0,
                       int expected, const double* S, hipStream_t st,
                       const std::function<int(int, bool)>& arnoldi, int* cols,
                       double* resid, int* done, int* iters_host,
                       double* resid_host) {
  double state[kNumSlots];
  int enq = 0, rc;
  *cols = *done = 0;
  while (true) {
    const int room = (m < maxit - it0 ? m : maxit - it0) - enq;
    if (room <= 0) return FLOW_OK;
    int plan = expected - (it0 + enq);
    if (plan < 1) plan = 1;
    if (plan > room) plan = room;
    for (int k = 0; k < plan; ++k, ++enq) {
      const bool last = enq + 1 >= m || it0 + enq + 1 >= maxit;
      if ((rc = arnoldi(enq, last))) return rc;
    }
    if ((rc = read_state(S, state, st))) return rc;
    *cols = static_cast<int>(state[kConvIt]);
    if (state[kDone] == 2.0) {
      *iters_host = it0 + *cols;
      *resid_host = state[kRes2];
      set_error("%s broke down (NaN) at iteration %d", solver, it0 + *cols);
      return FLOW_NOT_CONVERGED;
    }
    *resid = state[kRes2];
    *done = static_cast<int>(state[kDone]);
    if (*done != 0) return FLOW_OK;
  }
}

static int gmres(const flow_operator* A, const double* dinv, const flow_ilu* ilu,
                 const flow_pmg* pmg, const double* b, double* x, double rtol,
                 double atol, int maxit, int m, int x_is_zero, int expected,
                 int verify, double* work, int* iters_host, double* resid_host,
                 hipStream_t st) {
  const int N = op_size(A);
  double* partial = work;
  double* S = work + 3 * kRedBlocks;
  double* V = work + FLOW_REDUCE_WORK;
  double* Z = V + static_cast<size_t>(m + 1) * N;
  double* iwork = Z + static_cast<size_t>(m) * N;
  double* P = iwork + N;
  double* Pww = P + kGmresMax * kRedBlocks;
  double* Pnn = Pww + kRedBlocks;
  double* G = P + FLOW_GMRES_PARTIALS;
  const double* stop = S + kDone;
  const int gv = grid_for(N);
  const int gd = grid_for(N, kBlock, kRedBlocks);
  int np = 0, rc;

  const double* jprm = nullptr;
  const bool precond = pmg || ilu || dinv;
  const double* Zbase = precond ? Z : V;
  auto precondition = [&](int j) -> int {
    const double* in = V + static_cast<size_t>(j) * N;
    double* out = Z + static_cast<size_t>(j) * N;
    if (pmg) return pmg_apply(pmg, in, out, st, stop);
    if (ilu) return ilu_apply(ilu, in, out, iwork, st, stop);
    if (dinv)
      hipLaunchKernelGGL(vmul_kernel, dim3(gv), dim3(kBlock), 0, st, N, 1.0, dinv,
                         in, out, stop);
    return FLOW_OK;
  };
  auto arnoldi = [&](int j, double beta, double target, bool last) -> int {
    int r;
    double* w = V + static_cast<size_t>(j + 1) * N;
    if ((r = precondition(j))) return r;
    if ((r = apply(A, Zbase + static_cast<size_t>(j) * N, w, st, nullptr, stop, 0,
                   0, jprm)))
      return r;
    arnoldi_dots(N, j, w, V, gd, P, Pww, stop, st);
    hipLaunchKernelGGL(gmres_step_kernel, dim3(1), dim3(kBlock), 0, st, gd, j,
                       last ? 1 : 0, beta, target, P, G, S);
    FLOW_CHECK_LAUNCH();
    if (!last &&
        (r = gmres_combine_dev(N, j + 1, G + kGCoef, G + kGCw, w, V, w, Pnn, false,
                               stop, st)))
      return r;
    return FLOW_OK;
  };

  const bool replay = replay_wanted(N, kReplayGmres);
  KeyHash base;
  if (replay) {
    base.pod(0x676dull);
    key_operator(base, A, true);
    base.pod(dinv).obj(ilu).obj(ilu ? ilu->plan : nullptr).obj(pmg);
    base.pod(work).pod(N).pod(m);
    if (A->kind == 3) {
      jprm = G + kGJvp;
      if ((rc = momentum_jvp_params(
               static_cast<const flow_momentum_jvp*>(A->matfree), G + kGJvp, st)))
        return rc;
    }
  }
  auto arnoldi_replayed = [&](int j, bool last) -> int {
    if (!replay) return arnoldi(j, -1.0, 0.0, last);
    KeyHash key = base;
    key.pod(j).pod(last);
    hipGraphExec_t graph = nullptr;
    int nodes = 0, r;
    if ((r = replay_prepare(key.h, kReplayGmres, st,
                            [&]() { return arnoldi(j, -1.0, 0.0, last); }, &graph,
                            &nodes)))
      return r;
    return graph ? replay_launch(graph, nodes, st) : arnoldi(j, -1.0, 0.0, last);
  };

  if ((rc = fill(kNumSlots, 0.0, S, st))) return rc;
  double resid = 0.0;
  int it = 0;
  bool first = true;
  bool claimed = false;
  double state[kNumSlots];
  while (true) {
    const bool b_is_r0 = x_is_zero && it == 0;
    if (b_is_r0) {
      hipLaunchKernelGGL(axpby_kernel, dim3(gv), dim3(kBlock), 0, st, N, 1.0, b,
                         0.0, V);
    } else {
      if ((rc = apply(A, x, iwork, st))) return rc;
      hipLaunchKernelGGL(residual_kernel, dim3(gv), dim3(kBlock), 0, st, N, b,
                         iwork,
                         static_cast<const double*>(nullptr), V,
                         static_cast<double*>(nullptr));
    }
    const int have_b2 = first && !b_is_r0;
    if ((rc = dots(N, have_b2 ? 2 : 1, V, V, b, b, V, V, partial, &np, st)))
      return rc;
    hipLaunchKernelGGL(gmres_begin_kernel, dim3(1), dim3(kBlock), 0, st, np,
                       have_b2, first ? 1 : 0, claimed ? 1 : 0, rtol, atol,
                       partial, S);
    if (have_b2)
      hipLaunchKernelGGL(gmres_drop_start_kernel, dim3(gv), dim3(kBlock), 0, st,
                         N, S, b, V, x);
    FLOW_CHECK_LAUNCH();
    first = false;
    claimed = false;
    if (it >= maxit) {
      if ((rc = read_state(S, state, st))) return rc;
      resid = state[kBeta];
      if (state[kDone] == 4.0) break;
      *iters_host = it;
      *resid_host = resid;
      if (state[kDone] == 2.0) {
        set_error("GMRES broke down (NaN residual) at iteration %d", it);
      } else {
        set_error("GMRES did not converge in %d iterations: |r| = %.3e > %.3e",
                  it, resid, state[kTarget2]);
      }
      return FLOW_NOT_CONVERGED;
    }

    int cols, done;
    if ((rc = gmres_cycle("GMRES", m, maxit, it, expected, S, st,
                          arnoldi_replayed, &cols, &resid, &done, iters_host,
                          resid_host)))
      return rc;
    if (done == 4) break;
    const bool converged = done == 1;
    it += cols > 0 ? cols : 1;
    if ((rc = fill(1, 0.0, S + kDone, st))) return rc;
    if (cols > 0 &&
        (rc = gmres_combine_dev(N, cols, G + kGYc, nullptr, nullptr, Zbase, x,
                                nullptr, true, nullptr, st)))
      return rc;
    x_is_zero = 0;
    if (converged && !verify) break;
    claimed = converged;
  }
  *iters_host = it;
  *resid_host = resid;
  return FLOW_OK;
}

static int check_solver_args(const flow_operator* A, const double* b,
                             const double* x, double rtol, double atol,
                             int maxit, int check_every, int first_check,
                             const double* work, size_t work_len, size_t nvec,
                             const int* iters_host, const double* resid_host) {
  int rc = check_operator(A);
  if (rc) return rc;
  FLOW_REQUIRE(b && x && work && iters_host && resid_host, "solver pointers");
  FLOW_REQUIRE(rtol >= 0.0 && atol >= 0.0 && maxit >= 0 && check_every > 0 &&
                   first_check >= 0,
               "solver tolerances");
  FLOW_REQUIRE(work_len >= FLOW_REDUCE_WORK + nvec * (size_t)op_size(A),
               "solver workspace too small");
  return FLOW_OK;
}

static int check_cg_args(const flow_operator* A, const double* dinv,
                         const flow_coarse* coarse, const flow_mg* mg,
                         const double* b, const double* x, double rtol,
                         double atol, int maxit, int check_every,
                         int first_check, const double* work, size_t work_len,
                         const int* iters_host, const double* resid_host) {
  int rc = check_solver_args(A, b, x, rtol, atol, maxit, check_every,
                             first_check, work, work_len, 5, iters_host,
                             resid_host);
  if (rc) return rc;
  FLOW_REQUIRE(A->kind != 3, "CG: assembled (symmetric) operators only");
  if (coarse) {
    FLOW_REQUIRE(dinv != nullptr, "two-level preconditioner needs dinv");
    FLOW_REQUIRE(A->kind == 0, "two-level preconditioner: scalar operators");
    if ((rc = check_coarse(coarse, A->n))) return rc;
  }
  if (mg) {
    FLOW_REQUIRE(coarse == nullptr, "multigrid and two-level are exclusive");
    FLOW_REQUIRE(dinv != nullptr && A->kind == 0,
                 "multigrid preconditioner: scalar operators with dinv");
    if ((rc = check_mg(mg, A->n))) return rc;
    FLOW_REQUIRE(mg->nlevels >= 2, "multigrid: at least two levels");
  }
  FLOW_REQUIRE(work_len >= cg_work_len(A, coarse, mg),
               "solver workspace too small (FLOW_REDUCE_WORK + 5 N + SpMV "
               "workgroups + 2 [+ 2 lda] [+ 2 mg->Ps[0].nblocks])");
  FLOW_REQUIRE(reinterpret_cast<uintptr_t>(work) % 16 == 0,
               "solver workspace must be 16-byte aligned");
  return FLOW_OK;
}

extern "C" int flow_cg_solve(const flow_operator* A, const double* dinv,
                             const flow_coarse* coarse, const flow_mg* mg,
                             const double* b,
                             double* x, double rtol, double atol, int maxit,
                             int check_every, int first_check, double* work,
                             size_t work_len, int* iters_host,
                             double* resid_host, void* stream) {
  int rc = check_cg_args(A, dinv, coarse, mg, b, x, rtol, atol, maxit,
                         check_every, first_check, work, work_len, iters_host,
                         resid_host);
  if (rc) return rc;
  return cg(A, dinv, coarse, mg, b, x, rtol, atol, maxit, check_every,
            first_check, work, iters_host, resid_host, as_stream(stream));
}

extern "C" int flow_cg_solve_guarded(
    const flow_operator* A, const double* dinv, const flow_coarse* coarse,
    const flow_mg* mg, const double* b, double* x, const double* x_fallback,
    double rtol, double atol, int maxit, int check_every, int first_check,
    double* work, size_t work_len, int* iters_host, double* resid_host,
    int* starts_dropped_host, void* stream) {
  FLOW_REQUIRE(starts_dropped_host != nullptr, "starts_dropped_host is NULL");
  *starts_dropped_host = 0;
  int rc = check_cg_args(A, dinv, coarse, mg, b, x, rtol, atol, maxit,
                         check_every, first_check, work, work_len, iters_host,
                         resid_host);
  if (rc) return rc;
  FLOW_REQUIRE(x_fallback != x, "the fallback start must not alias x");
  hipStream_t st = as_stream(stream);
  const int N = op_size(A);
  bool rejected = false;
  rc = cg(A, dinv, coarse, mg, b, x, rtol, atol, maxit, check_every,
          first_check, work, iters_host, resid_host, st, &rejected);
  if (rc || !rejected) return rc;
  *starts_dropped_host = 1;
  if (x_fallback) {
    hipLaunchKernelGGL(axpby_kernel, dim3(grid_for(N)), dim3(kBlock), 0, st, N,
                       1.0, x_fallback, 0.0, x);
    FLOW_CHECK_LAUNCH();
    rc = cg(A, dinv, coarse, mg, b, x, rtol, atol, maxit, check_every, 0, work,
            iters_host, resid_host, st, &rejected);
    if (rc || !rejected) return rc;
    *starts_dropped_host = 2;
  }
  if ((rc = fill(N, 0.0, x, st))) return rc;
  return cg(A, dinv, coarse, mg, b, x, rtol, atol, maxit, check_every, 0, work,
            iters_host, resid_host, st);
}

extern "C" int flow_mg_apply(const flow_mg* mg, int n, const double* r,
                             double* z, void* stream) {
  FLOW_REQUIRE(mg && r && z && r != z && n > 0, "mg apply");
  int rc = check_mg(mg, n);
  if (rc) return rc;
  return vcycle(mg, r, z, as_stream(stream));
}

extern "C" int flow_two_level_apply(const flow_coarse* coarse,
                                    const double* dinv, const double* r,
                                    double* z, double* work, void* stream) {
  FLOW_REQUIRE(coarse && dinv && r && z && work && r != z, "two-level apply");
  int rc = check_coarse(coarse, coarse->n);
  if (rc) return rc;
  FLOW_REQUIRE(reinterpret_cast<uintptr_t>(work) % 16 == 0,
               "two-level workspace must be 16-byte aligned");
  return two_level(coarse, dinv, r, z, work, work + coarse->lda,
                   as_stream(stream));
}

extern "C" int flow_bicgstab_solve(const flow_operator* A, const double* dinv,
                                   const flow_ilu* ilu, const double* b,
                                   double* x, double rtol, double atol,
                                   int maxit, int check_every,
                                   int first_check, double* work,
                                   size_t work_len, int* iters_host,
                                   double* resid_host, void* stream) {
  int rc = check_solver_args(A, b, x, rtol, atol, maxit, check_every,
                             first_check, work, work_len, 7, iters_host,
                             resid_host);
  if (rc) return rc;
  if (ilu) {
    if ((rc = ilu_check(ilu, op_size(A)))) return rc;
    FLOW_REQUIRE(work_len >= FLOW_REDUCE_WORK + 8 * (size_t)op_size(A),
                 "solver workspace too small for the ILU sweep buffer");
  }
  return bicgstab(A, dinv, ilu, b, x, rtol, atol, maxit, check_every,
                  first_check, work, iters_host, resid_host, as_stream(stream));
}

int flow::check_gmres_args(int restart, int expected_its) {
  FLOW_REQUIRE(restart >= 1 && restart <= FLOW_GMRES_MAX_RESTART,
               "GMRES restart length");
  FLOW_REQUIRE(expected_its >= 0, "expected iterations");
  return FLOW_OK;
}

extern "C" int flow_gmres_solve(const flow_operator* A, const double* dinv,
                                const flow_ilu* ilu, const flow_pmg* pmg,
                                const double* b, double* x,
                                double rtol, double atol, int maxit, int restart,
                                int x_is_zero, int expected_its, int verify,
                                double* work, size_t work_len, int* iters_host,
                                double* resid_host, void* stream) {
  int rc = check_solver_args(A, b, x, rtol, atol, maxit, 1, 0, work, work_len, 0,
                             iters_host, resid_host);
  if (rc || (rc = check_gmres_args(restart, expected_its))) return rc;
  FLOW_REQUIRE(work_len >= FLOW_REDUCE_WORK +
                               (2 * static_cast<size_t>(restart) + 2) *
                                   op_size(A) +
                               FLOW_GMRES_PARTIALS + FLOW_GMRES_STATE,
               "solver workspace too small (FLOW_REDUCE_WORK + (2 restart + 2) N "
               "+ FLOW_GMRES_PARTIALS + FLOW_GMRES_STATE)");
  FLOW_REQUIRE(!(ilu && pmg), "one preconditioner: ilu or pmg");
  if (ilu && (rc = ilu_check(ilu, op_size(A)))) return rc;
  if (pmg && (rc = pmg_check(pmg, op_size(A)))) return rc;
  return gmres(A, dinv, ilu, pmg, b, x, rtol, atol, maxit, restart, x_is_zero,
               expected_its, verify, work, iters_host, resid_host,
               as_stream(stream));
}
```

flow_amd/csrc/la_internal.h:

```cpp
#pragma once
#include "common.h"

namespace flow {

inline int op_size(const flow_operator* A) {
  return A->kind == 0 ? A->n : 2 * A->n;
}

inline int dot_parts(const flow_operator* A) {
  return A->kind == 1 ? 2 * A->nblocks : A->nblocks;
}

struct SpmvProfile {
  int rows = 0, cap = 0, used = 0;
  hipEvent_t* ev = nullptr;
};
extern SpmvProfile g_spmv_profile;

int apply(const flow_operator* A, const double* x, double* y, hipStream_t st,
          double* dpart = nullptr, const double* stop = nullptr,
          int vec_stride = 0, int out_stride = 0,
          const double* jvp_prm = nullptr);

int dots(int n, int nd, const double* a0, const double* b0, const double* a1,
         const double* b1, const double* a2, const double* b2, double* partial,
         int* nparts, hipStream_t st);

constexpr int kMailbox = 64;
int read_values(const double* dev, int n, double* host, hipStream_t st);

__global__ __launch_bounds__(kBlock) void absmax_kernel(
    int n, const double* __restrict__ x, double* __restrict__ partial);
__global__ __launch_bounds__(kBlock) void finish_kernel(
    int nparts, int nd, int is_max, const double* __restrict__ partial,
    double* __restrict__ out);
__global__ void axpby_kernel(int n, double a, const double* __restrict__ x,
                             double b, double* __restrict__ y);
__global__ void vmul_kernel(int n, double a, const double* x, const double* y,
                            double* out, const double* stop = nullptr);
__global__ void residual_kernel(int n, const double* __restrict__ b,
                                const double* __restrict__ q,
                                const double* __restrict__ dinv,
                                double* __restrict__ r, double* __restrict__ z);

constexpr int kScalarBlock = 1024;

template <int UP, bool DOTS>
__global__ __launch_bounds__(kBlock) void mg_level_kernel(
    const int* __restrict__ rowptr, const int* __restrict__ cols,
    const double* __restrict__ vals, const int* __restrict__ rowblocks,
    const double* __restrict__ x, const double* __restrict__ c,
    const double* __restrict__ t, const double* __restrict__ dinv, double omega,
    double* __restrict__ y, double* __restrict__ gpart,
    double* __restrict__ rpart, const double* __restrict__ stop);
template <bool DOTS>
__global__ __launch_bounds__(kBlock) void mg_up2_kernel(
    const int* __restrict__ rowblocks, const int* __restrict__ p_rowptr,
    const int* __restrict__ p_cols, const double* __restrict__ p_vals,
    const int* __restrict__ a_rowptr, const int* __restrict__ a_cols,
    const double* __restrict__ a_vals, const double* __restrict__ xc,
    const double* __restrict__ c, const double* __restrict__ dinv, double omega,
    double* __restrict__ y, double* __restrict__ gpart,
    double* __restrict__ rpart, const double* __restrict__ stop,
    int own_lo = 0, int own_hi = 0x7fffffff);
template <bool DOTS>
__global__ __launch_bounds__(kBlock) void cg_update_kernel(
    int n, const double* __restrict__ S, const double* __restrict__ dinv,
    const double* __restrict__ w, double* __restrict__ z, double* __restrict__ p,
    double* __restrict__ s, double* __restrict__ x, double* __restrict__ r,
    int want_z, double* __restrict__ partial,
    const double* __restrict__ own);

#define FLOW_KRYLOV_INSTANCES(X)                                               \
  X __global__ void mg_level_kernel<0, false>(                                 \
      const int*, const int*, const double*, const int*, const double*,        \
      const double*, const double*, const double*, double, double*, double*,   \
      double*, const double*);                                                 \
  X __global__ void mg_level_kernel<1, false>(                                 \
      const int*, const int*, const double*, const int*, const double*,        \
      const double*, const double*, const double*, double, double*, double*,   \
      double*, const double*);                                                 \
  X __global__ void mg_level_kernel<1, true>(                                  \
      const int*, const int*, const double*, const int*, const double*,        \
      const double*, const double*, const double*, double, double*, double*,   \
      double*, const double*);                                                 \
  X __global__ void mg_up2_kernel<false>(                                      \
      const int*, const int*, const int*, const double*, const int*,           \
      const int*, const double*, const double*, const double*, const double*,  \
      double, double*, double*, double*, const double*, int, int);             \
  X __global__ void mg_up2_kernel<true>(                                       \
      const int*, const int*, const int*, const double*, const int*,           \
      const int*, const double*, const double*, const double*, const double*,  \
      double, double*, double*, double*, const double*, int, int);             \
  X __global__ void cg_update_kernel<false>(                                   \
      int, const double*, const double*, const double*, double*, double*,      \
      double*, double*, double*, int, double*, const double*);                 \
  X __global__ void cg_update_kernel<true>(                                    \
      int, const double*, const double*, const double*, double*, double*,      \
      double*, double*, double*, int, double*, const double*);
FLOW_KRYLOV_INSTANCES(extern template)

int check_mg(const flow_mg* M, int n);
int vcycle(const flow_mg* M, const double* r0, double* z0, hipStream_t st,
           double* gpart = nullptr, double* rpart = nullptr,
           int* nparts = nullptr, const double* stop = nullptr, int l0 = 0);

constexpr int kGmresMax = FLOW_GMRES_MAX_RESTART;
constexpr int kGH = 0;
constexpr int kGNrm = kGH + kGmresMax * (kGmresMax + 1);
constexpr int kGEta = kGNrm + kGmresMax + 1;
constexpr int kGCoef = kGEta + kGmresMax;
constexpr int kGCw = kGCoef + kGmresMax;
constexpr int kGYc = kGCw + 1;
constexpr int kGRot = kGYc + kGmresMax;
constexpr int kGRhs = kGRot + 2 * kGmresMax;
constexpr int kGJvp = kGRhs + kGmresMax + 1;
constexpr int kGState = kGJvp + 3;
static_assert(kGState <= FLOW_GMRES_STATE, "gmres device state");

int gmres_combine_dev(int N, int nv, const double* coef, const double* cw,
                      const double* w, const double* V, double* out,
                      double* nn_partial, bool accumulate, const double* stop,
                      hipStream_t st);
int check_gmres_args(int restart, int expected_its);

}

template <int NV>
__global__ __launch_bounds__(flow::kBlock) void gmres_dots_kernel(
    int n, const double* __restrict__ w, const double* __restrict__ V,
    size_t stride, int with_ww, double* __restrict__ partial,
    double* __restrict__ ww_partial, const double* __restrict__ stop = nullptr);
#define FLOW_GMRES_DOTS_INSTANCES(X)                                           \
  X(1) X(2) X(3) X(4) X(5) X(6) X(7) X(8)
#define FLOW_GMRES_DOTS_EXTERN(NV)                                             \
  extern template __global__ void gmres_dots_kernel<NV>(                       \
      int, const double*, const double*, size_t, int, double*, double*,        \
      const double*);
FLOW_GMRES_DOTS_INSTANCES(FLOW_GMRES_DOTS_EXTERN)
#undef FLOW_GMRES_DOTS_EXTERN
#define FLOW_NV_SWITCH(nv, CALL) \
  switch (nv) {                  \
    case 1: CALL(1); break;      \
    case 2: CALL(2); break;      \
    case 3: CALL(3); break;      \
    case 4: CALL(4); break;      \
    case 5: CALL(5); break;      \
    case 6: CALL(6); break;      \
    case 7: CALL(7); break;      \
    default: CALL(8); break;     \
  }
__global__ __launch_bounds__(flow::kBlock) void gmres_step_kernel(
    int nparts, int j, int last, double beta, double target,
    const double* __restrict__ partial, double* __restrict__ G,
    double* __restrict__ S);
```

flow_amd/csrc/la_kernels.hip:

```cpp
#include "common.h"
#include "csr_stream.h"
#include "la_internal.h"

namespace flow {

thread_local char g_error[512] = "";

void set_error(const char* fmt, ...) {
  va_list ap;
  va_start(ap, fmt);
  vsnprintf(g_error, sizeof(g_error), fmt, ap);
  va_end(ap);
}

static_assert(3 * kRedBlocks + kNumSlots <= FLOW_REDUCE_WORK, "work size");


template <bool DOT>
__global__ __launch_bounds__(kBlock) void spmv_stream_kernel(
    int n, const int* __restrict__ rowptr, const int* __restrict__ cols,
    const double* __restrict__ vals0, const double* __restrict__ vals1,
    const int* __restrict__ rowblocks, const double* __restrict__ x,
    double* __restrict__ y, double* __restrict__ dpart,
    const double* __restrict__ stop) {
  __shared__ double prod[kTile];
  if (stopped(stop)) return;
  const double* __restrict__ vals = blockIdx.y == 0 ? vals0 : vals1;
  x += static_cast<size_t>(blockIdx.y) * n;
  y += static_cast<size_t>(blockIdx.y) * n;
  int r, r1;
  double xi = 0.0;
  auto early = [&](int row, bool has) {
    if (DOT && has) xi = x[row];
  };
  const double s =
      stream_tile_row_sum(rowptr, cols, vals, rowblocks, x, prod, r, r1, early);
  double t = 0.0;
  if (r < r1) {
    y[r] = s;
    if (DOT) t = s * xi;
  }
  if (DOT) {
    t = block_sum_once(t);
    if (threadIdx.x == 0) dpart[blockIdx.y * gridDim.x + blockIdx.x] = t;
  }
}

template <bool DOT>
__global__ __launch_bounds__(kBlock) void spmv_stream_block2_kernel(
    int n, const int* __restrict__ rowptr, const int* __restrict__ cols,
    const double* __restrict__ vxx, const double* __restrict__ vxy,
    const double* __restrict__ vyx, const double* __restrict__ vyy,
    const int* __restrict__ rowblocks, const double* __restrict__ x,
    double* __restrict__ y, double* __restrict__ dpart,
    const double* __restrict__ stop) {
  __shared__ double prod0[kTile2];
  __shared__ double prod1[kTile2];
  if (stopped(stop)) return;
  const int tile = xcd_tile(blockIdx.x, gridDim.x);
  const int r0 = rowblocks[tile];
  const int r1 = rowblocks[tile + 1];
  const int k0 = rowptr[r0];
  const int k1 = rowptr[r1];
  const int ka = k0 & ~1;
  const int r = r0 + threadIdx.x;
  int a = 0, b = 0;
  if (r < r1) {
    a = rowptr[r] - ka;
    b = rowptr[r + 1] - ka;
  }
  const int npair = (k1 - ka + 1) >> 1;
  const int2* __restrict__ c2p = reinterpret_cast<const int2*>(cols + ka);
  const double2* __restrict__ pxx = reinterpret_cast<const double2*>(vxx + ka);
  const double2* __restrict__ pxy = reinterpret_cast<const double2*>(vxy + ka);
  const double2* __restrict__ pyx = reinterpret_cast<const double2*>(vyx + ka);
  const double2* __restrict__ pyy = reinterpret_cast<const double2*>(vyy + ka);
#pragma unroll
  for (int j = 0; j < kPairs2; ++j) {
    const int p = threadIdx.x + j * kBlock;
    if (p < npair) {
      const int2 c = c2p[p];
      const double2 axx = pxx[p], axy = pxy[p], ayx = pyx[p], ayy = pyy[p];
      const int cx = 2 * p >= k0 - ka ? c.x : cols[k0];
      const int cy = 2 * p + 1 < k1 - ka ? c.y : cols[k0];
      const double u0 = x[cx], u1 = x[n + cx];
      const double w0 = x[cy], w1 = x[n + cy];
      prod0[2 * p] = axx.x * u0 + axy.x * u1;
      prod1[2 * p] = ayx.x * u0 + ayy.x * u1;
      prod0[2 * p + 1] = axx.y * w0 + axy.y * w1;
      prod1[2 * p + 1] = ayx.y * w0 + ayy.y * w1;
    }
  }
  __syncthreads();
  double t = 0.0;
  if (r < r1) {
    double s0 = 0.0, s1 = 0.0;
    for (int k = a; k < b; ++k) {
      s0 += prod0[k];
      s1 += prod1[k];
    }
    y[r] = s0;
    y[n + r] = s1;
    if (DOT) t = s0 * x[r] + s1 * x[n + r];
  }
  if (DOT) {
    t = block_sum_once(t);
    if (threadIdx.x == 0) dpart[blockIdx.x] = t;
  }
}

template <bool DOT>
__global__ __launch_bounds__(kBlock) void spmv_stream_pair_kernel(
    int n, const int* __restrict__ rowptr, const int* __restrict__ cols,
    const double* __restrict__ vals, const int* __restrict__ rowblocks,
    const unsigned char* __restrict__ mask, const double* __restrict__ x,
    double* __restrict__ y, int xs, double* __restrict__ dpart,
    const double* __restrict__ stop) {
  __shared__ double2 prod[kTile2];
  if (stopped(stop)) return;
  int r, r1;
  const double2 s =
      stream_tile_pair_row_sum(rowptr, cols, vals, rowblocks, x, xs, prod, r, r1);
  double s0 = s.x, s1 = s.y;
  double t = 0.0;
  if (r < r1) {
    const double x0 = x[r], x1 = x[xs + r];
    if (!mask[r]) s0 = x0;
    if (!mask[n + r]) s1 = x1;
    y[r] = s0;
    y[xs + r] = s1;
    if (DOT) t = s0 * x0 + s1 * x1;
  }
  if (DOT) {
    t = block_sum_once(t);
    if (threadIdx.x == 0) dpart[blockIdx.x] = t;
  }
}

int check_operator(const flow_operator* A) {
  FLOW_REQUIRE(A != nullptr, "operator is NULL");
  FLOW_REQUIRE(A->kind >= 0 && A->kind <= 4, "operator kind");
  if (A->kind == 3) {
    const flow_momentum_jvp* J =
        static_cast<const flow_momentum_jvp*>(A->matfree);
    int rc = momentum_jvp_check(J);
    if (rc) return rc;
    FLOW_REQUIRE(A->n == J->W->n, "matrix-free operator size");
    return FLOW_OK;
  }
  FLOW_REQUIRE(A->n > 0 && A->nnz > 0 && A->nblocks > 0, "operator sizes");
  FLOW_REQUIRE(A->rowptr && A->cols && A->rowblocks, "operator pattern");
  const int planes = (A->kind == 0 || A->kind == 4) ? 1 : (A->kind == 1 ? 2 : 4);
  FLOW_REQUIRE(A->kind != 4 || A->rowmask != nullptr, "operator row mask");
  for (int p = 0; p < planes; ++p) {
    FLOW_REQUIRE(A->vals[p] != nullptr, "operator value plane");
    FLOW_REQUIRE((reinterpret_cast<size_t>(A->vals[p]) & 15) == 0,
                 "value planes must be 16-byte aligned");
  }
  FLOW_REQUIRE((reinterpret_cast<size_t>(A->cols) & 7) == 0,
               "cols must be 8-byte aligned");
  return FLOW_OK;
}

SpmvProfile g_spmv_profile;

void key_operator(KeyHash& k, const flow_operator* A, bool skip_prm) {
  k.obj(A);
  if (A && A->kind == 3 && A->matfree) {
    flow_momentum_jvp J = *static_cast<const flow_momentum_jvp*>(A->matfree);
    if (skip_prm) J.prm = flow_ns_params{0.0, 0.0, 0.0, 0.0, 0.0};
    k.obj(&J).obj(J.mesh).obj(J.W);
  }
}

int apply(const flow_operator* A, const double* x, double* y, hipStream_t st,
          double* dpart, const double* stop, int vec_stride, int out_stride,
          const double* jvp_prm) {
  if (A->kind == 3) {
    FLOW_REQUIRE(dpart == nullptr, "matrix-free operators carry no fused dot");
    return momentum_jvp_apply(static_cast<const flow_momentum_jvp*>(A->matfree),
                              x, y, st, vec_stride, out_stride, stop, jvp_prm);
  }
  const int xs = vec_stride ? vec_stride : A->n;
  const dim3 grid(A->nblocks, A->kind == 1 ? 2 : 1);
  const double* v1 = A->kind == 1 ? A->vals[1] : A->vals[0];
  if (A->kind == 4) {
    if (dpart)
      hipLaunchKernelGGL(spmv_stream_pair_kernel<true>, grid, dim3(kBlock), 0, st,
                         A->n, A->rowptr, A->cols, A->vals[0], A->rowblocks,
                         A->rowmask, x, y, xs, dpart, stop);
    else
      hipLaunchKernelGGL(spmv_stream_pair_kernel<false>, grid, dim3(kBlock), 0,
                         st, A->n, A->rowptr, A->cols, A->vals[0], A->rowblocks,
                         A->rowmask, x, y, xs, dpart, stop);
  } else if (A->kind == 2) {
    if (dpart)
      hipLaunchKernelGGL(spmv_stream_block2_kernel<true>, grid, dim3(kBlock), 0,
                         st, A->n, A->rowptr, A->cols, A->vals[0], A->vals[1],
                         A->vals[2], A->vals[3], A->rowblocks, x, y, dpart,
                         stop);
    else
      hipLaunchKernelGGL(spmv_stream_block2_kernel<false>, grid, dim3(kBlock), 0,
                         st, A->n, A->rowptr, A->cols, A->vals[0], A->vals[1],
                         A->vals[2], A->vals[3], A->rowblocks, x, y, dpart,
                         stop);
  } else if (dpart) {
    SpmvProfile& pf = g_spmv_profile;
    const bool timed = pf.used < pf.cap && A->kind == 0 && A->n == pf.rows;
    if (timed) FLOW_CHECK_HIP(hipEventRecord(pf.ev[2 * pf.used], st));
    hipLaunchKernelGGL(spmv_stream_kernel<true>, grid, dim3(kBlock), 0, st, A->n,
                       A->rowptr, A->cols, A->vals[0], v1, A->rowblocks, x, y,
                       dpart, stop);
    if (timed) FLOW_CHECK_HIP(hipEventRecord(pf.ev[2 * pf.used++ + 1], st));
  } else {
    hipLaunchKernelGGL(spmv_stream_kernel<false>, grid, dim3(kBlock), 0, st,
                       A->n, A->rowptr, A->cols, A->vals[0], v1, A->rowblocks, x,
                       y, dpart, stop);
  }
  FLOW_CHECK_LAUNCH();
  return FLOW_OK;
}

int operator_apply(const flow_operator* A, const double* x, double* y,
                   hipStream_t st, const double* stop) {
  return apply(A, x, y, st, nullptr, stop);
}
int operator_size(const flow_operator* A) { return op_size(A); }

__global__ void diag_inv_kernel(int n, int planes_kind,
                                const int* __restrict__ diag_idx,
                                const double* __restrict__ v0,
                                const double* __restrict__ v1,
                                const unsigned char* __restrict__ mask,
                                double* __restrict__ dinv) {
  for (int i = blockIdx.x * blockDim.x + threadIdx.x; i < n;
       i += gridDim.x * blockDim.x) {
    const int k = diag_idx[i];
    dinv[i] = (mask && !mask[i]) ? 1.0 : 1.0 / v0[k];
    if (planes_kind > 0)
      dinv[n + i] = (mask && !mask[n + i]) ? 1.0 : 1.0 / v1[k];
  }
}

__global__ __launch_bounds__(kBlock) void dot3_kernel(
    int n, int nd, const double* __restrict__ a0, const double* __restrict__ b0,
    const double* __restrict__ a1, const double* __restrict__ b1,
    const double* __restrict__ a2, const double* __restrict__ b2,
    double* __restrict__ partial) {
  double s0 = 0.0, s1 = 0.0, s2 = 0.0;
  for (int i = blockIdx.x * blockDim.x + threadIdx.x; i < n;
       i += gridDim.x * blockDim.x) {
    s0 += a0[i] * b0[i];
    if (nd > 1) s1 += a1[i] * b1[i];
    if (nd > 2) s2 += a2[i] * b2[i];
  }
  s0 = block_sum(s0);
  if (nd > 1) s1 = block_sum(s1);
  if (nd > 2) s2 = block_sum(s2);
  if (threadIdx.x == 0) {
    partial[blockIdx.x] = s0;
    if (nd > 1) partial[kRedBlocks + blockIdx.x] = s1;
    if (nd > 2) partial[2 * kRedBlocks + blockIdx.x] = s2;
  }
}

__global__ __launch_bounds__(kBlock) void absmax_kernel(
    int n, const double* __restrict__ x, double* __restrict__ partial) {
  double m = 0.0;
  for (int i = blockIdx.x * blockDim.x + threadIdx.x; i < n;
       i += gridDim.x * blockDim.x)
    m = fmax(m, fabs(x[i]));
  m = block_max(m);
  if (threadIdx.x == 0) partial[blockIdx.x] = m;
}

__global__ __launch_bounds__(kBlock) void finish_kernel(
    int nparts, int nd, int is_max, const double* __restrict__ partial,
    double* __restrict__ out) {
  for (int j = 0; j < nd; ++j) {
    double v = 0.0;
    for (int i = threadIdx.x; i < nparts; i += kBlock) {
      const double p = load_scalar(partial + j * kRedBlocks + i);
      v = is_max ? fmax(v, p) : v + p;
    }
    v = is_max ? block_max(v) : block_sum(v);
    if (threadIdx.x == 0) store_scalar(out + j, v);
  }
}

__global__ void axpby_kernel(int n, double a, const double* __restrict__ x,
                             double b, double* __restrict__ y) {
  for (int i = blockIdx.x * blockDim.x + threadIdx.x; i < n;
       i += gridDim.x * blockDim.x)
    y[i] = (b == 0.0) ? a * x[i] : a * x[i] + b * y[i];
}

__global__ void fill_kernel(int n, double value, double* __restrict__ y) {
  for (int i = blockIdx.x * blockDim.x + threadIdx.x; i < n;
       i += gridDim.x * blockDim.x)
    y[i] = value;
}

int fill(int n, double value, double* y, hipStream_t st) {
  hipLaunchKernelGGL(fill_kernel, dim3(grid_for(n)), dim3(kBlock), 0, st, n,
                     value, y);
  FLOW_CHECK_LAUNCH();
  return FLOW_OK;
}

__global__ void vmul_kernel(int n, double a, const double* x, const double* y,
                            double* out, const double* stop) {
  if (stopped(stop)) return;
  for (int i = blockIdx.x * blockDim.x + threadIdx.x; i < n;
       i += gridDim.x * blockDim.x)
    out[i] = a * x[i] * y[i];
}

__global__ void residual_kernel(int n, const double* __restrict__ b,
                                const double* __restrict__ q,
                                const double* __restrict__ dinv,
                                double* __restrict__ r, double* __restrict__ z) {
  for (int i = blockIdx.x * blockDim.x + threadIdx.x; i < n;
       i += gridDim.x * blockDim.x) {
    const double ri = b[i] - q[i];
    r[i] = ri;
    if (z) z[i] = dinv ? dinv[i] * ri : ri;
  }
}

int dots(int n, int nd, const double* a0, const double* b0, const double* a1,
         const double* b1, const double* a2, const double* b2, double* partial,
         int* nparts, hipStream_t st) {
  const int g = grid_for(n, kBlock * 4, kRedBlocks);
  hipLaunchKernelGGL(dot3_kernel, dim3(g), dim3(kBlock), 0, st, n, nd, a0, b0,
                     a1, b1, a2, b2, partial);
  FLOW_CHECK_LAUNCH();
  *nparts = g;
  return FLOW_OK;
}

__global__ void mailbox_kernel(const double* __restrict__ src0,
                               const double* __restrict__ src1,
                               volatile double* __restrict__ mailbox) {
  mailbox[0] = load_scalar(src0);
  mailbox[1] = load_scalar(src1);
  __threadfence_system();
}

static int mailbox_of_thread(double** host, double** dev) {
  static thread_local double* mailbox = nullptr;
  if (!mailbox)
    FLOW_CHECK_HIP(hipHostMalloc(reinterpret_cast<void**>(&mailbox),
                                 kMailbox * sizeof(double), hipHostMallocMapped));
  *host = mailbox;
  FLOW_CHECK_HIP(
      hipHostGetDevicePointer(reinterpret_cast<void**>(dev), mailbox, 0));
  return FLOW_OK;
}

static int read_slots(const double* S, int slot0, int slot1, double* host0,
                      double* host1, hipStream_t st) {
  double *mailbox = nullptr, *dev_view = nullptr;
  int rc = mailbox_of_thread(&mailbox, &dev_view);
  if (rc) return rc;
  hipLaunchKernelGGL(mailbox_kernel, dim3(1), dim3(1), 0, st, S + slot0,
                     S + slot1, dev_view);
  FLOW_CHECK_LAUNCH();
  FLOW_CHECK_HIP(hipStreamSynchronize(st));
  *host0 = static_cast<volatile double*>(mailbox)[0];
  *host1 = static_cast<volatile double*>(mailbox)[1];
  return FLOW_OK;
}

__global__ void mailbox_state_kernel(const double* __restrict__ S,
                                     volatile double* __restrict__ mailbox) {
  if (threadIdx.x < kNumSlots) mailbox[threadIdx.x] = load_scalar(S + threadIdx.x);
  __threadfence_system();
}

int read_state(const double* S, double* host, hipStream_t st) {
  double *mailbox = nullptr, *dev_view = nullptr;
  int rc = mailbox_of_thread(&mailbox, &dev_view);
  if (rc) return rc;
  hipLaunchKernelGGL(mailbox_state_kernel, dim3(1), dim3(64), 0, st, S, dev_view);
  FLOW_CHECK_LAUNCH();
  FLOW_CHECK_HIP(hipStreamSynchronize(st));
  for (int i = 0; i < kNumSlots; ++i)
    host[i] = static_cast<volatile double*>(mailbox)[i];
  return FLOW_OK;
}

static int read_slot(const double* S, int slot, double* host, hipStream_t st) {
  double again;
  return read_slots(S, slot, slot, host, &again, st);
}

int sum_partials_host(double* work, int nparts, double* host, hipStream_t st) {
  FLOW_REQUIRE(nparts >= 1 && nparts <= kRedBlocks, "partial count");
  double* S = work + 3 * kRedBlocks;
  hipLaunchKernelGGL(finish_kernel, dim3(1), dim3(kBlock), 0, st, nparts, 1, 0,
                     work, S);
  FLOW_CHECK_LAUNCH();
  return read_slot(S, 0, host, st);
}

__global__ void mailbox_copy_kernel(int n, const double* __restrict__ src,
                                    volatile double* __restrict__ mailbox) {
  if (threadIdx.x < n) mailbox[threadIdx.x] = load_scalar(src + threadIdx.x);
  __threadfence_system();
}

int read_values(const double* dev, int n, double* host, hipStream_t st) {
  double *mailbox = nullptr, *dev_view = nullptr;
  int rc = mailbox_of_thread(&mailbox, &dev_view);
  if (rc) return rc;
  FLOW_REQUIRE(n <= kMailbox, "mailbox size");
  hipLaunchKernelGGL(mailbox_copy_kernel, dim3(1), dim3(64), 0, st, n, dev,
                     dev_view);
  FLOW_CHECK_LAUNCH();
  FLOW_CHECK_HIP(hipStreamSynchronize(st));
  for (int i = 0; i < n; ++i) host[i] = static_cast<volatile double*>(mailbox)[i];
  return FLOW_OK;
}

}

using namespace flow;

extern "C" const char* flow_last_error(void) { return g_error; }
extern "C" int flow_abi_version(void) { return 30; }

namespace flow {
unsigned long long g_launches = 0;
}
extern "C" int flow_launch_count(unsigned long long* count_host) {
  FLOW_REQUIRE(count_host != nullptr, "flow_launch_count argument");
  *count_host = flow::g_launches;
  return FLOW_OK;
}

extern "C" int flow_read_doubles(const double* dev, int n, double* host,
                                 void* stream) {
  FLOW_REQUIRE(dev && host && n >= 1 && n <= flow::kMailbox,
               "read_doubles arguments (1..64 values)");
  return flow::read_values(dev, n, host, flow::as_stream(stream));
}

extern "C" int flow_operator_apply(const flow_operator* A, const double* x,
                                   double* y, void* stream) {
  int rc = check_operator(A);
  if (rc) return rc;
  FLOW_REQUIRE(x && y && x != y, "x, y");
  return apply(A, x, y, as_stream(stream));
}

extern "C" int flow_operator_diag_inv(const flow_operator* A,
                                      const int* diag_idx, double* dinv,
                                      void* stream) {
  int rc = check_operator(A);
  if (rc) return rc;
  FLOW_REQUIRE(diag_idx && dinv, "diag_idx, dinv");
  FLOW_REQUIRE(A->kind != 3, "a matrix-free operator has no stored diagonal");
  const double* v1 = (A->kind == 0 || A->kind == 4)
                         ? A->vals[0]
                         : (A->kind == 1 ? A->vals[1] : A->vals[3]);
  hipLaunchKernelGGL(diag_inv_kernel, dim3(grid_for(A->n)), dim3(kBlock), 0,
                     as_stream(stream), A->n, A->kind, diag_idx, A->vals[0], v1,
                     A->kind == 4 ? A->rowmask
                                  : static_cast<const unsigned char*>(nullptr),
                     dinv);
  FLOW_CHECK_LAUNCH();
  return FLOW_OK;
}

__global__ void scale_rows_kernel(int n, const int* __restrict__ rowptr,
                                  const double* __restrict__ d,
                                  double* __restrict__ vals) {
  for (int r = blockIdx.x * blockDim.x + threadIdx.x; r < n;
       r += gridDim.x * blockDim.x) {
    const double di = d[r];
    for (int k = rowptr[r]; k < rowptr[r + 1]; ++k) vals[k] *= di;
  }
}

extern "C" int flow_scale_rows(int n, const int* rowptr, const double* d,
                               double* vals, void* stream) {
  FLOW_REQUIRE(n > 0 && rowptr && d && vals, "scale rows arguments");
  hipLaunchKernelGGL(scale_rows_kernel, dim3(grid_for(n)), dim3(kBlock), 0,
                     as_stream(stream), n, rowptr, d, vals);
  FLOW_CHECK_LAUNCH();
  return FLOW_OK;
}

extern "C" int flow_dot_host(int n, const double* x, const double* y,
                             double* work, double* result_host, void* stream) {
  FLOW_REQUIRE(n > 0 && x && y && work && result_host, "dot arguments");
  hipStream_t st = as_stream(stream);
  int np = 0;
  int rc = dots(n, 1, x, y, x, y, x, y, work, &np, st);
  if (rc) return rc;
  double* S = work + 3 * kRedBlocks;
  hipLaunchKernelGGL(finish_kernel, dim3(1), dim3(kBlock), 0, st, np, 1, 0, work,
                     S);
  FLOW_CHECK_LAUNCH();
  return read_slot(S, 0, result_host, st);
}

extern "C" int flow_norm_host(int n, const double* x, int kind, double* work,
                              double* result_host, void* stream) {
  FLOW_REQUIRE(n > 0 && x && work && result_host, "norm arguments");
  FLOW_REQUIRE(kind == 0 || kind == 1, "norm kind");
  hipStream_t st = as_stream(stream);
  double* S = work + 3 * kRedBlocks;
  if (kind == 0) {
    int rc = flow_dot_host(n, x, x, work, result_host, stream);
    if (rc) return rc;
    *result_host = sqrt(*result_host);
    return FLOW_OK;
  }
  const int g = grid_for(n, kBlock * 4, kRedBlocks);
  hipLaunchKernelGGL(absmax_kernel, dim3(g), dim3(kBlock), 0, st, n, x, work);
  hipLaunchKernelGGL(finish_kernel, dim3(1), dim3(kBlock), 0, st, g, 1, 1, work,
                     S);
  FLOW_CHECK_LAUNCH();
  return read_slot(S, 0, result_host, st);
}

extern "C" int flow_axpby(int n, double a, const double* x, double b, double* y,
                          void* stream) {
  FLOW_REQUIRE(n > 0 && x && y, "axpby arguments");
  hipLaunchKernelGGL(axpby_kernel, dim3(grid_for(n)), dim3(kBlock), 0,
                     as_stream(stream), n, a, x, b, y);
  FLOW_CHECK_LAUNCH();
  return FLOW_OK;
}

__global__ void gather_rows_kernel(int ncomp, int m, const int* __restrict__ idx,
                                   const double* __restrict__ src, int src_stride,
                                   double* __restrict__ dst, int dst_stride) {
  for (int t = blockIdx.x * blockDim.x + threadIdx.x; t < ncomp * m;
       t += gridDim.x * blockDim.x) {
    const int a = t / m, k = t - a * m;
    dst[static_cast<size_t>(a) * dst_stride + k] =
        src[static_cast<size_t>(a) * src_stride + idx[k]];
  }
}

extern "C" int flow_gather_rows(int ncomp, const int* idx, int m,
                                const double* src, int src_stride, double* dst,
                                int dst_stride, void* stream) {
  FLOW_REQUIRE(ncomp >= 1 && m > 0 && idx && src && dst && src_stride > 0 &&
                   dst_stride >= m,
               "gather_rows arguments");
  hipLaunchKernelGGL(gather_rows_kernel, dim3(grid_for(static_cast<long long>(ncomp) * m)),
                     dim3(kBlock), 0, as_stream(stream), ncomp, m, idx, src,
                     src_stride, dst, dst_stride);
  FLOW_CHECK_LAUNCH();
  return FLOW_OK;
}

constexpr int kLincombMax = 6;
struct LincombArgs {
  double a[kLincombMax];
  const double* x[kLincombMax];
};
template <int NT>
__global__ void lincomb_kernel(int n, LincombArgs t, double* __restrict__ y) {
  for (int i = blockIdx.x * blockDim.x + threadIdx.x; i < n;
       i += gridDim.x * blockDim.x) {
    double v = 0.0;
#pragma unroll
    for (int k = 0; k < NT; ++k) v += t.a[k] * t.x[k][i];
    y[i] = v;
  }
}

extern "C" int flow_extrapolation_weights(int m, const double* dts_host, double dt,
                                          int power, int degree,
                                          double* w_host) {
  FLOW_REQUIRE(m >= 1 && m <= kLincombMax && dts_host && w_host && dt > 0.0,
               "extrapolation weights: 1..6 past steps");
  const int q = (degree <= 0 || degree > m - 1) ? m - 1 : degree;
  const int n = q + 1;
  double x[kLincombMax], t = 0.0;
  for (int i = 0; i < m; ++i) {
    FLOW_REQUIRE(dts_host[i] > 0.0, "extrapolation weights: step sizes");
    x[i] = t - 0.5 * dts_host[i];
    t -= dts_host[i];
  }
  const double scale = -t;
  for (int i = 0; i < m; ++i) x[i] /= scale;
  const double xs = 0.5 * dt / scale;
  double V[kLincombMax][kLincombMax], N[kLincombMax][kLincombMax + 1];
  for (int i = 0; i < m; ++i) {
    double p = 1.0;
    for (int k = 0; k < n; ++k, p *= x[i]) V[i][k] = p;
  }
  double e = 1.0;
  for (int a = 0; a < n; ++a, e *= xs) {
    for (int b = 0; b < n; ++b) {
      double sum = 0.0;
      for (int i = 0; i < m; ++i) sum += V[i][a] * V[i][b];
      N[a][b] = sum;
    }
    N[a][n] = e;
  }
  for (int c = 0; c < n; ++c) {
    int piv = c;
    for (int r = c + 1; r < n; ++r)
      if (fabs(N[r][c]) > fabs(N[piv][c])) piv = r;
    FLOW_REQUIRE(N[piv][c] != 0.0, "extrapolation weights: singular fit");
    for (int k = 0; k <= n; ++k) {
      const double tmp = N[c][k];
      N[c][k] = N[piv][k];
      N[piv][k] = tmp;
    }
    const double d = N[c][c];
    for (int k = 0; k <= n; ++k) N[c][k] /= d;
    for (int r = 0; r < n; ++r) {
      if (r == c) continue;
      const double f = N[r][c];
      for (int k = 0; k <= n; ++k) N[r][k] -= f * N[c][k];
    }
  }
  for (int i = 0; i < m; ++i) {
    double w = 0.0;
    for (int a = 0; a < n; ++a) w += V[i][a] * N[a][n];
    w_host[i] = w * pow(dt / dts_host[i], power);
  }
  return FLOW_OK;
}

extern "C" int flow_lincomb(int n, int nterms, const double* coef_host,
                            const double* const* x_host, double* y,
                            void* stream) {
  FLOW_REQUIRE(n >= 0 && nterms >= 1 && nterms <= kLincombMax && coef_host &&
                   x_host && y,
               "lincomb arguments (1..6 terms)");
  if (n == 0) return FLOW_OK;
  LincombArgs t = {};
  for (int k = 0; k < nterms; ++k) {
    FLOW_REQUIRE(x_host[k] != nullptr && x_host[k] != y, "lincomb term");
    t.a[k] = coef_host[k];
    t.x[k] = x_host[k];
  }
  const dim3 grid(grid_for(n)), blk(kBlock);
  hipStream_t st = as_stream(stream);
  switch (nterms) {
    case 1: hipLaunchKernelGGL(lincomb_kernel<1>, grid, blk, 0, st, n, t, y); break;
    case 2: hipLaunchKernelGGL(lincomb_kernel<2>, grid, blk, 0, st, n, t, y); break;
    case 3: hipLaunchKernelGGL(lincomb_kernel<3>, grid, blk, 0, st, n, t, y); break;
    case 4: hipLaunchKernelGGL(lincomb_kernel<4>, grid, blk, 0, st, n, t, y); break;
    case 5: hipLaunchKernelGGL(lincomb_kernel<5>, grid, blk, 0, st, n, t, y); break;
    default: hipLaunchKernelGGL(lincomb_kernel<6>, grid, blk, 0, st, n, t, y); break;
  }
  FLOW_CHECK_LAUNCH();
  return FLOW_OK;
}

constexpr int kFingerprintFields = 2;
struct FingerprintArgs {
  const double* x[kFingerprintFields];
  int n[kFingerprintFields];
  int line_stride[kFingerprintFields];
  int sampled[kFingerprintFields];
};

__global__ __launch_bounds__(kBlock) void fingerprint_kernel(
    FingerprintArgs a, unsigned long long* __restrict__ part) {
  __shared__ unsigned long long wave_part[kBlock / 64];
  const int f = blockIdx.y;
  const double* __restrict__ x = a.x[f];
  const int n = a.n[f], k = a.line_stride[f], m = a.sampled[f];
  unsigned long long h = 0;
  for (int e = blockIdx.x * blockDim.x + threadIdx.x; e < m;
       e += gridDim.x * blockDim.x) {
    const long long idx = static_cast<long long>(e >> 3) * k * 8 + (e & 7);
    if (idx < n) {
      const unsigned long long bits =
          static_cast<unsigned long long>(__double_as_longlong(x[idx]));
      h += (bits ^ (bits >> 29)) *
           ((2ull * static_cast<unsigned long long>(idx) + 1ull) *
            0x9E3779B97F4A7C15ull);
    }
  }
#pragma unroll
  for (int off = 32; off > 0; off >>= 1) h += __shfl_down(h, off, 64);
  if ((threadIdx.x & 63) == 0) wave_part[threadIdx.x >> 6] = h;
  __syncthreads();
  if (threadIdx.x == 0) {
    h = 0;
    for (int w = 0; w < kBlock / 64; ++w) h += wave_part[w];
    part[static_cast<size_t>(f) * kRedBlocks + blockIdx.x] = h;
  }
}

__global__ __launch_bounds__(kBlock) void fingerprint_finish_kernel(
    int nparts, const unsigned long long* __restrict__ part,
    double* __restrict__ slots) {
  __shared__ unsigned long long wave_part[kBlock / 64];
  const int f = blockIdx.x;
  unsigned long long h = 0;
  for (int i = threadIdx.x; i < nparts; i += kBlock)
    h += part[static_cast<size_t>(f) * kRedBlocks + i];
#pragma unroll
  for (int off = 32; off > 0; off >>= 1) h += __shfl_down(h, off, 64);
  if ((threadIdx.x & 63) == 0) wave_part[threadIdx.x >> 6] = h;
  __syncthreads();
  if (threadIdx.x == 0) {
    h = 0;
    for (int w = 0; w < kBlock / 64; ++w) h += wave_part[w];
    store_scalar(slots + 2 * f, static_cast<double>(h & 0xffffffffull));
    store_scalar(slots + 2 * f + 1, static_cast<double>(h >> 32));
  }
}

extern "C" int flow_fingerprint(int nfields, const double* const* x_host,
                                const int* n_host, double* work, double* slots,
                                void* stream) {
  FLOW_REQUIRE(nfields >= 1 && nfields <= kFingerprintFields && x_host &&
                   n_host && work && slots,
               "fingerprint arguments (1 or 2 fields)");
  FingerprintArgs a = {};
  int most = 0;
  for (int f = 0; f < nfields; ++f) {
    FLOW_REQUIRE(x_host[f] != nullptr && n_host[f] > 0, "fingerprint field");
    const long long lines = (static_cast<long long>(n_host[f]) + 7) / 8;
    const long long cap = (1ll << 22) / 8;
    const long long k = (lines + cap - 1) / cap;
    a.x[f] = x_host[f];
    a.n[f] = n_host[f];
    a.line_stride[f] = static_cast<int>(k);
    a.sampled[f] = static_cast<int>(((lines + k - 1) / k) * 8);
    if (a.sampled[f] > most) most = a.sampled[f];
  }
  hipStream_t st = as_stream(stream);
  const int g = grid_for(most, kBlock * 4, kRedBlocks);
  unsigned long long* part = reinterpret_cast<unsigned long long*>(work);
  hipLaunchKernelGGL(fingerprint_kernel, dim3(g, nfields), dim3(kBlock), 0, st,
                     a, part);
  hipLaunchKernelGGL(fingerprint_finish_kernel, dim3(nfields), dim3(kBlock), 0,
                     st, g, part, slots);
  FLOW_CHECK_LAUNCH();
  return FLOW_OK;
}

extern "C" int flow_fill(int n, double value, double* y, void* stream) {
  FLOW_REQUIRE(n > 0 && y, "fill arguments");
  return fill(n, value, y, as_stream(stream));
}

extern "C" int flow_vmul(int n, double a, const double* x, const double* y,
                         double* out, void* stream) {
  FLOW_REQUIRE(n > 0 && x && y && out, "vmul arguments");
  hipLaunchKernelGGL(vmul_kernel, dim3(grid_for(n)), dim3(kBlock), 0,
                     as_stream(stream), n, a, x, y, out);
  FLOW_CHECK_LAUNCH();
  return FLOW_OK;
}
```

flow_amd/csrc/mass_kernels.hip:

```cpp
#include "common.h"
#include "csr_stream.h"
#include "csr_stream16.h"

#include <hip/hip_fp16.h>

namespace flow {

__global__ __launch_bounds__(kBlock) void mass_residual_kernel(
    const int* __restrict__ rowptr, const int* __restrict__ cols,
    const double* __restrict__ vals, const int* __restrict__ rowblocks,
    const double* __restrict__ x, const double* __restrict__ b,
    const double* __restrict__ dinv, float* __restrict__ rho0,
    const double* __restrict__ stop) {
  __shared__ double prod[kTile];
  if (stopped(stop)) return;
  int r, r1;
  double bi = 0.0, di = 0.0;
  auto early = [&](int row, bool has) {
    if (has) {
      bi = b[row];
      di = dinv[row];
    }
  };
  const double s =
      stream_tile_row_sum(rowptr, cols, vals, rowblocks, x, prod, r, r1, early);
  if (r < r1) rho0[r] = static_cast<float>(di * (bi - s));
}

__global__ __launch_bounds__(kBlock) void mass_residual_pair_kernel(
    int n, const int* __restrict__ rowptr, const int* __restrict__ cols,
    const double* __restrict__ vals, const int* __restrict__ rowblocks,
    const unsigned char* __restrict__ mask, const double* __restrict__ x, int xs,
    const double* __restrict__ b, const double* __restrict__ dinv,
    float2* __restrict__ rho0, const double* __restrict__ stop) {
  __shared__ double2 prod[kTile2];
  if (stopped(stop)) return;
  int r, r1;
  double b0 = 0.0, b1 = 0.0, d0 = 0.0, d1 = 0.0, x0 = 0.0, x1 = 0.0;
  bool m0 = true, m1 = true;
  auto early = [&](int row, bool has) {
    if (!has) return;
    b0 = b[row];
    b1 = b[static_cast<size_t>(n) + row];
    d0 = dinv[row];
    d1 = dinv[static_cast<size_t>(n) + row];
    m0 = mask[row] != 0;
    m1 = mask[n + row] != 0;
    x0 = x[row];
    x1 = x[xs + row];
  };
  const double2 s = stream_tile_pair_row_sum(rowptr, cols, vals, rowblocks, x, xs,
                                             prod, r, r1, early);
  if (r < r1) {
    const double s0 = m0 ? s.x : x0;
    const double s1 = m1 ? s.y : x1;
    rho0[r] = make_float2(static_cast<float>(d0 * (b0 - s0)),
                          static_cast<float>(d1 * (b1 - s1)));
  }
}

__global__ void mass_rho0_kernel(int n, int ncomp, const double* __restrict__ g,
                                 const double* __restrict__ dinv,
                                 float* __restrict__ rho0,
                                 const double* __restrict__ stop, int r0 = 0,
                                 int r1 = 0x7fffffff) {
  if (stopped(stop)) return;
  if (r1 > n) r1 = n;
  for (int i = r0 + blockIdx.x * blockDim.x + threadIdx.x; i < r1;
       i += gridDim.x * blockDim.x)
    for (int a = 0; a < ncomp; ++a) {
      const size_t k = static_cast<size_t>(a) * n + i;
      rho0[static_cast<size_t>(i) * ncomp + a] = static_cast<float>(dinv[k] * g[k]);
    }
}

__device__ __forceinline__ void apply_mask(const unsigned char* mask, int n, int r,
                                           float own, float& s) {
  if (mask && !mask[r]) s = own;
}
__device__ __forceinline__ void apply_mask(const unsigned char* mask, int n, int r,
                                           float2 own, float2& s) {
  if (mask) {
    if (!mask[r]) s.x = own.x;
    if (!mask[n + r]) s.y = own.y;
  }
}
__device__ __forceinline__ float vaxpby(float a, float x, float b, float y) {
  return a * x + b * y;
}
__device__ __forceinline__ float2 vaxpby(float a, float2 x, float b, float2 y) {
  return make_float2(a * x.x + b * y.x, a * x.y + b * y.y);
}
struct XRow {
  double x0 = 0.0, x1 = 0.0, b0 = 0.0, b1 = 0.0;
};
__device__ __forceinline__ void load_xrow(XRow& q, const double* x,
                                          const double* base, int xs, int r,
                                          float) {
  q.x0 = x[r];
  if (base) q.b0 = base[r];
}
__device__ __forceinline__ void load_xrow(XRow& q, const double* x,
                                          const double* base, int xs, int r,
                                          float2) {
  q.x0 = x[r];
  q.x1 = x[xs + r];
  if (base) {
    q.b0 = base[r];
    q.b1 = base[xs + r];
  }
}
__device__ __forceinline__ double2 add_to_x(double* x, const XRow& q, int xs,
                                           int r, float z) {
  const double xn = q.x0 + static_cast<double>(z);
  x[r] = xn;
  const double y = q.b0 + xn;
  return make_double2(static_cast<double>(z) * z, y * y);
}
__device__ __forceinline__ double2 add_to_x(double* x, const XRow& q, int xs,
                                           int r, float2 z) {
  const double x0 = q.x0 + static_cast<double>(z.x);
  const double x1 = q.x1 + static_cast<double>(z.y);
  x[r] = x0;
  x[xs + r] = x1;
  const double y0 = q.b0 + x0;
  const double y1 = q.b1 + x1;
  return make_double2(static_cast<double>(z.x) * z.x + static_cast<double>(z.y) * z.y,
                      y0 * y0 + y1 * y1);
}

template <class V, int MODE, bool PACKED>
__global__ __launch_bounds__(kBlock) void mass_cheb_kernel(
    int n, const int* __restrict__ rowptr, const int* __restrict__ cols,
    const void* __restrict__ vals, const int* __restrict__ rowblocks,
    const unsigned char* __restrict__ mask, const V* __restrict__ g,
    const V* rho_in, V* rho_out, float c0, float c1, float c2,
    V* __restrict__ d_out, V* __restrict__ acc, double* __restrict__ x,
    const double* __restrict__ xbase, int xs,
    double* __restrict__ zz_part, double* __restrict__ xx_part,
    const double* __restrict__ stop, int own_lo = 0, int own_hi = 0x7fffffff) {
  __shared__ V prod[kTile16];
  if (stopped(stop)) return;
  int r, r1;
  V own, rho_old, acc_old;
  vzero(own);
  vzero(rho_old);
  vzero(acc_old);
  XRow xr;
  auto early = [&](int row, bool has) {
    if (!has) return;
    own = g[row];
    if (MODE >= 1) {
      rho_old = rho_in[row];
      acc_old = acc[row];
    }
    if (MODE == 2) load_xrow(xr, x, xbase, xs, row, V());
  };
  V s = PACKED
            ? fp16_tile_row_sum(
                  rowptr, PackedStream{static_cast<const unsigned*>(vals), cols},
                  rowblocks, g, prod, r, r1, early)
            : fp16_tile_row_sum(
                  rowptr,
                  Cols32Stream<__half>{static_cast<const __half*>(vals), cols},
                  rowblocks, g, prod, r, r1, early);
  double2 dots = make_double2(0.0, 0.0);
  if (r < r1) {
    apply_mask(mask, n, r, own, s);
    if (MODE == 0) {
      const V rho = vaxpby(1.f, own, -c0, s);
      const V d = vaxpby(c1 * c0, own, c2, rho);
      rho_out[r] = rho;
      d_out[r] = d;
      acc[r] = vaxpby(c0, own, 1.f, d);
    } else {
      const V rho = vaxpby(1.f, rho_old, -1.f, s);
      const V d = vaxpby(c1, own, c2, rho);
      if (MODE == 1) {
        rho_out[r] = rho;
        d_out[r] = d;
        acc[r] = vaxpby(1.f, acc_old, 1.f, d);
      } else {
        dots = add_to_x(x, xr, xs, r, vaxpby(1.f, acc_old, 1.f, d));
        if (r < own_lo || r >= own_hi) dots = make_double2(0.0, 0.0);
      }
    }
  }
  if (MODE == 2) {
    const double zz = block_sum(dots.x);
    const double xx = block_sum(dots.y);
    if (threadIdx.x == 0) {
      zz_part[blockIdx.x] = zz;
      xx_part[blockIdx.x] = xx;
    }
  }
}

constexpr int kMassScalarBlock = 1024;
__global__ __launch_bounds__(kMassScalarBlock) void mass_scalar_kernel(
    int nparts, const double* __restrict__ zz_part,
    const double* __restrict__ xx_part, double contraction2, double rtol2,
    double atol2, double* __restrict__ S) {
  __shared__ double wsum[2][kMassScalarBlock / 64];
  if (stopped(S + kDone)) return;
  double z0 = 0.0, z1 = 0.0, x0 = 0.0, x1 = 0.0;
  int i = threadIdx.x;
  for (; i + kMassScalarBlock < nparts; i += 2 * kMassScalarBlock) {
    z0 += load_scalar(zz_part + i);
    z1 += load_scalar(zz_part + i + kMassScalarBlock);
    x0 += load_scalar(xx_part + i);
    x1 += load_scalar(xx_part + i + kMassScalarBlock);
  }
  for (; i < nparts; i += kMassScalarBlock) {
    z0 += load_scalar(zz_part + i);
    x0 += load_scalar(xx_part + i);
  }
  double zz = z0 + z1, xx = x0 + x1;
#pragma unroll
  for (int off = 32; off > 0; off >>= 1) {
    zz += __shfl_down(zz, off, 64);
    xx += __shfl_down(xx, off, 64);
  }
  if ((threadIdx.x & 63) == 0) {
    wsum[0][threadIdx.x >> 6] = zz;
    wsum[1][threadIdx.x >> 6] = xx;
  }
  __syncthreads();
  if (threadIdx.x != 0) return;
  zz = xx = 0.0;
  for (int w = 0; w < kMassScalarBlock / 64; ++w) {
    zz += wsum[0][w];
    xx += wsum[1][w];
  }
  const double k = load_scalar(S + kIter) + 1.0;
  const bool nan = !(zz == zz) || !(xx == xx);
  const double prev = load_scalar(S + kGamma);
  const double seen2 = (k > 1.0 && prev > 0.0) ? zz / prev : 0.0;
  const double c2 = fmax(contraction2, fmin(seen2, 1.0));
  if (nan || c2 * zz <= fmax(rtol2 * xx, atol2)) {
    store_scalar(S + kConvIt, k);
    store_scalar(S + kDone, nan ? 2.0 : 1.0);
  } else if (k > 1.0 && seen2 >= 1.0 && zz > 1.0e-26 * xx) {
    store_scalar(S + kConvIt, k);
    store_scalar(S + kTmp, sqrt(seen2));
    store_scalar(S + kDone, 3.0);
  }
  store_scalar(S + kGamma, zz);
  store_scalar(S + kIter, k);
  store_scalar(S + kRes2, zz);
  store_scalar(S + kB2, xx);
}

__global__ void mass_pack_kernel(int n, const int* __restrict__ rowptr,
                                 const int* __restrict__ diag_idx,
                                 const double* __restrict__ vals,
                                 __half* __restrict__ vals16) {
  for (int i = blockIdx.x * blockDim.x + threadIdx.x; i < n;
       i += gridDim.x * blockDim.x) {
    const double inv = 1.0 / vals[diag_idx[i]];
    for (int k = rowptr[i]; k < rowptr[i + 1]; ++k)
      vals16[k] = half_rn(vals[k] * inv);
  }
}

__global__ __launch_bounds__(kBlock) void mass_pack16_kernel(
    const int* __restrict__ rowblocks, const int* __restrict__ rowptr,
    const int* __restrict__ cols, const int* __restrict__ diag_idx,
    const double* __restrict__ vals, int* __restrict__ cbase,
    unsigned* __restrict__ packed, int* __restrict__ overflow) {
  const int tile = blockIdx.x;
  const int r0 = rowblocks[tile], r1 = rowblocks[tile + 1];
  const int base = tile_lowest_col(cols, rowptr[r0], rowptr[r1]);
  if (threadIdx.x == 0) cbase[tile] = base;
  const int r = r0 + threadIdx.x;
  if (r < r1) {
    const double inv = 1.0 / vals[diag_idx[r]];
    for (int k = rowptr[r]; k < rowptr[r + 1]; ++k) {
      const int off = cols[k] - base;
      if (off > 0xffff) atomicOr(overflow, 1);
      const unsigned short h = __half_as_ushort(half_rn(vals[k] * inv));
      packed[k] = (static_cast<unsigned>(off & 0xffff) << 16) | h;
    }
  }
}

namespace {

struct MassTiles {
  const int* rowblocks[16];
  int nblocks[16];
  int shift;
  int own_lo, own_hi;
};

template <class V, bool PACKED>
int correction(const flow_mass* M, const MassTiles& T, double* x,
               const double* xbase, double* zz_part, double* xx_part,
               const double* stop, hipStream_t st) {
  const flow_operator* A = M->A;
  const int n = A->n;
  const void* v16 = PACKED ? M->packed16 : M->vals16;
  const int* cols = PACKED ? M->cbase16 : A->cols;
  V* w = reinterpret_cast<V*>(M->work16) - T.shift;
  const size_t len = static_cast<size_t>(M->work16_rows > 0 ? M->work16_rows : n);
  V* rho0 = w;
  V* rho = rho0 + len;
  V* d[2] = {rho + len, rho + 2 * len};
  V* acc = rho + 3 * len;
  const dim3 blk(kBlock);
  Cheb ch(M->lam_min, M->lam_max);
  const float c0 = ch.first();
  float c1, c2;
  V* const none = nullptr;
  double* const nod = nullptr;
  ch.next(&c1, &c2);
  hipLaunchKernelGGL((mass_cheb_kernel<V, 0, PACKED>), dim3(T.nblocks[0]), blk, 0,
                     st, n, A->rowptr, cols, v16, T.rowblocks[0], A->rowmask, rho0,
                     rho0, rho, c0, c1, c2, d[0], acc, nod, nod, n, nod, nod, stop,
                     0, 0x7fffffff);
  const int products = M->steps - 1;
  for (int j = 1; j + 1 < products; ++j) {
    ch.next(&c1, &c2);
    hipLaunchKernelGGL((mass_cheb_kernel<V, 1, PACKED>), dim3(T.nblocks[j]), blk,
                       0, st, n, A->rowptr, cols, v16, T.rowblocks[j], A->rowmask,
                       d[(j - 1) & 1], rho, rho, 0.f, c1, c2, d[j & 1], acc, nod,
                       nod, n, nod, nod, stop, 0, 0x7fffffff);
  }
  ch.next(&c1, &c2);
  hipLaunchKernelGGL((mass_cheb_kernel<V, 2, PACKED>),
                     dim3(T.nblocks[products - 1]), blk, 0, st, n, A->rowptr, cols,
                     v16, T.rowblocks[products - 1], A->rowmask,
                     d[(products - 2) & 1], rho, none, 0.f, c1, c2, none, acc, x,
                     xbase, n, zz_part, xx_part, stop, T.own_lo, T.own_hi);
  FLOW_CHECK_LAUNCH();
  return FLOW_OK;
}

static MassTiles default_tiles(const flow_mass* M) {
  MassTiles T;
  for (int j = 0; j < 16; ++j) {
    T.rowblocks[j] = M->rowblocks16;
    T.nblocks[j] = M->nblocks16;
  }
  T.shift = 0;
  T.own_lo = 0;
  T.own_hi = 0x7fffffff;
  return T;
}

}

static int mass_check(const flow_mass* M) {
  FLOW_REQUIRE(M != nullptr && M->A != nullptr, "flow_mass is NULL");
  int rc = check_operator(M->A);
  if (rc) return rc;
  FLOW_REQUIRE(M->A->kind == 0 || M->A->kind == 4,
               "flow_mass: operator kind 0 (scalar) or 4 (one plane, two "
               "components)");
  FLOW_REQUIRE(M->dinv && M->rowblocks16 && (M->vals16 || M->packed16) &&
                   M->work16 && M->nblocks16 > 0,
               "flow_mass pointers");
  FLOW_REQUIRE(reinterpret_cast<uintptr_t>(M->vals16) % 16 == 0 &&
                   reinterpret_cast<uintptr_t>(M->packed16) % 16 == 0 &&
                   reinterpret_cast<uintptr_t>(M->A->cols) % 16 == 0 &&
                   reinterpret_cast<uintptr_t>(M->work16) % 16 == 0,
               "flow_mass: vals16 / packed16, cols and work16 must be 16-byte "
               "aligned");
  FLOW_REQUIRE(M->packed16 == nullptr || M->cbase16 != nullptr,
               "flow_mass: the packed stream needs the tiles' base columns");
  FLOW_REQUIRE(M->lam_max > M->lam_min && M->lam_min > 0.0,
               "Chebyshev interval (0 < lam_min < lam_max)");
  FLOW_REQUIRE(M->steps >= 3 && M->steps <= 16, "Chebyshev steps (3..16)");
  FLOW_REQUIRE(M->contraction > 0.0 && M->contraction <= 1.0,
               "contraction bound in (0, 1]");
  return FLOW_OK;
}

static int mass_solve(const flow_mass* M, const double* b, double* x,
                      const double* xbase, bool x_is_zero, double rtol,
                      double atol, int maxit, int first_check, double* work,
                      int* iters_host, double* resid_host, hipStream_t st) {
  const flow_operator* A = M->A;
  double* S = work + 3 * kRedBlocks;
  double* zz_part = work + FLOW_REDUCE_WORK;
  double* xx_part = zz_part + M->nblocks16;
  const double* stop = S + kDone;
  const double c2 = M->contraction * M->contraction;
  int rc;
  if ((rc = fill(kNumSlots, 0.0, S, st))) return rc;
  auto one = [&]() -> int {
    if (x_is_zero) {
      hipLaunchKernelGGL(mass_rho0_kernel, dim3(grid_for(A->n)), dim3(kBlock), 0,
                         st, A->n, A->kind == 4 ? 2 : 1, b, M->dinv, M->work16,
                         stop);
      x_is_zero = false;
    } else if (A->kind == 4) {
      hipLaunchKernelGGL(mass_residual_pair_kernel, dim3(A->nblocks), dim3(kBlock),
                         0, st, A->n, A->rowptr, A->cols, A->vals[0], A->rowblocks,
                         A->rowmask, x, A->n, b, M->dinv,
                         reinterpret_cast<float2*>(M->work16), stop);
    } else {
      hipLaunchKernelGGL(mass_residual_kernel, dim3(A->nblocks), dim3(kBlock), 0, st,
                         A->rowptr, A->cols, A->vals[0], A->rowblocks, x, b, M->dinv,
                         M->work16, stop);
    }
    const MassTiles T = default_tiles(M);
    if (A->kind == 4) {
      rc = M->packed16 ? correction<float2, true>(M, T, x, xbase, zz_part, xx_part,
                                                  stop, st)
                       : correction<float2, false>(M, T, x, xbase, zz_part,
                                                   xx_part, stop, st);
    } else {
      rc = M->packed16 ? correction<float, true>(M, T, x, xbase, zz_part, xx_part,
                                                 stop, st)
                       : correction<float, false>(M, T, x, xbase, zz_part, xx_part,
                                                  stop, st);
    }
    if (rc) return rc;
    hipLaunchKernelGGL(mass_scalar_kernel, dim3(1), dim3(kMassScalarBlock), 0, st,
                       M->nblocks16, zz_part, xx_part, c2, rtol * rtol, atol * atol,
                       S);
    FLOW_CHECK_LAUNCH();
    return FLOW_OK;
  };
  const bool replay = replay_wanted(A->n, kReplayMass);
  KeyHash base;
  if (replay) {
    base.pod(0x6d73ull);
    key_operator(base, A);
    base.obj(M).pod(b).pod(x).pod(xbase).pod(work).pod(rtol).pod(atol);
  }
  auto one_replayed = [&]() -> int {
    if (!replay) return one();
    KeyHash key = base;
    key.pod(x_is_zero);
    hipGraphExec_t graph = nullptr;
    int nodes = 0, r;
    const bool was_zero = x_is_zero;
    if ((r = replay_prepare(key.h, kReplayMass, st, one, &graph, &nodes))) return r;
    x_is_zero = was_zero;
    if (!graph) return one();
    x_is_zero = false;
    return replay_launch(graph, nodes, st);
  };
  double state[kNumSlots];
  int launched = 0;
  while (true) {
    const int batch = (launched == 0 && first_check > 0) ? first_check : 1;
    const int todo = (maxit - launched < batch) ? maxit - launched : batch;
    for (int k = 0; k < todo; ++k)
      if ((rc = one_replayed())) return rc;
    launched += todo;
    if ((rc = read_state(S, state, st))) return rc;
    const double zz = state[kRes2];
    if (state[kDone] == 2.0 || !(zz == zz)) {
      *iters_host = static_cast<int>(state[kConvIt]);
      *resid_host = zz;
      set_error("mass solve broke down (NaN) at correction %d", *iters_host);
      return FLOW_NOT_CONVERGED;
    }
    if (state[kDone] == 1.0) {
      *iters_host = static_cast<int>(state[kConvIt]);
      *resid_host = sqrt(zz);
      return FLOW_OK;
    }
    if (state[kDone] == 3.0) {
      *iters_host = static_cast<int>(state[kConvIt]);
      *resid_host = sqrt(zz);
      set_error("mass solve: correction %d contracted by %.3f (no "
                "contraction; the vouched bound is %.3f: not the mass matrix "
                "of straight P1/P2 triangles?)", *iters_host, state[kTmp],
                M->contraction);
      return FLOW_NOT_CONVERGED;
    }
    if (launched >= maxit) {
      *iters_host = launched;
      *resid_host = sqrt(zz);
      set_error("mass solve did not converge in %d defect corrections: |z| = "
                "%.3e, |x| = %.3e", launched, sqrt(zz), sqrt(state[kB2]));
      return FLOW_NOT_CONVERGED;
    }
  }
}


constexpr int kMassPackBlock = 1024;

__global__ __launch_bounds__(kMassPackBlock) void shard_mass_pack_kernel(
    flow_rows R, int ncomp, int first, int nparts,
    const double* __restrict__ zz_part, const double* __restrict__ xx_part,
    const float* __restrict__ rho0, double* __restrict__ buf,
    const double* __restrict__ stop) {
  if (stopped(stop)) return;
  if (blockIdx.x > 0) {
    const int total = ncomp * R.nhalo;
    for (int t = (blockIdx.x - 1) * blockDim.x + threadIdx.x; t < total;
         t += (gridDim.x - 1) * blockDim.x) {
      const int a = t / R.nhalo, k = t - a * R.nhalo;
      double v = 0.0;
#pragma unroll
      for (int sd = 0; sd < 2; ++sd)
        if (k >= R.send_slot[sd] && k < R.send_slot[sd] + R.send_len[sd])
          v = static_cast<double>(
              rho0[static_cast<size_t>(R.send_row[sd] + (k - R.send_slot[sd])) *
                       ncomp + a]);
      buf[4 + t] = v;
    }
    return;
  }
  __shared__ double wsum[2][kMassPackBlock / 64];
  double zz = 0.0, xx = 0.0;
  if (!first)
    for (int i = threadIdx.x; i < nparts; i += kMassPackBlock) {
      zz += load_scalar(zz_part + i);
      xx += load_scalar(xx_part + i);
    }
#pragma unroll
  for (int off = 32; off > 0; off >>= 1) {
    zz += __shfl_down(zz, off, 64);
    xx += __shfl_down(xx, off, 64);
  }
  if ((threadIdx.x & 63) == 0) {
    wsum[0][threadIdx.x >> 6] = zz;
    wsum[1][threadIdx.x >> 6] = xx;
  }
  __syncthreads();
  if (threadIdx.x == 0) {
    zz = xx = 0.0;
    for (int w = 0; w < kMassPackBlock / 64; ++w) {
      zz += wsum[0][w];
      xx += wsum[1][w];
    }
    buf[0] = zz;
    buf[1] = xx;
    buf[2] = 0.0;
    buf[3] = 0.0;
  }
}

__global__ void shard_mass_unpack_kernel(flow_rows R, int ncomp, int first,
                                         int applied, double contraction2,
                                         double rtol2, double atol2,
                                         const double* __restrict__ buf,
                                         float* __restrict__ rho0,
                                         double* __restrict__ S) {
  if (stopped(S + kDone)) return;
  const int per = R.recv_len[0] + R.recv_len[1];
  for (int t = blockIdx.x * blockDim.x + threadIdx.x; t < ncomp * per;
       t += gridDim.x * blockDim.x) {
    const int a = t / per, k = t - a * per;
    const int sd = k < R.recv_len[0] ? 0 : 1;
    const int j = sd == 0 ? k : k - R.recv_len[0];
    rho0[static_cast<size_t>(R.recv_row[sd] + j) * ncomp + a] = static_cast<float>(
        load_scalar(buf + 4 + static_cast<size_t>(a) * R.nhalo + R.recv_slot[sd] + j));
  }
  if (blockIdx.x != 0 || threadIdx.x != 0 || first) return;
  const double zz = load_scalar(buf), xx = load_scalar(buf + 1);
  const bool nan = !(zz == zz) || !(xx == xx);
  const double prev = load_scalar(S + kGamma);
  const double seen2 = (applied > 1 && prev > 0.0) ? zz / prev : 0.0;
  const double c2 = fmax(contraction2, fmin(seen2, 1.0));
  if (nan || c2 * zz <= fmax(rtol2 * xx, atol2)) {
    store_scalar(S + kConvIt, static_cast<double>(applied));
    store_scalar(S + kDone, nan ? 2.0 : 1.0);
  } else if (applied > 1 && seen2 >= 1.0 && zz > 1.0e-26 * xx) {
    store_scalar(S + kConvIt, static_cast<double>(applied));
    store_scalar(S + kTmp, sqrt(seen2));
    store_scalar(S + kDone, 3.0);
  }
  store_scalar(S + kGamma, zz);
  store_scalar(S + kIter, static_cast<double>(applied));
  store_scalar(S + kRes2, zz);
  store_scalar(S + kB2, xx);
}

static int shard_mass_solve(const flow_comm* C, const flow_rows* R,
                            const flow_mass* M, const flow_mass_strips* L,
                            const double* b, double* x, const double* xbase,
                            bool x_is_zero, double rtol, double atol, int maxit,
                            int first_check, double* work, int* iters_host,
                            double* resid_host, hipStream_t st) {
  const flow_operator* A = M->A;
  const int ncomp = A->kind == 4 ? 2 : 1;
  const int products = M->steps - 1;
  double* S = work + 3 * kRedBlocks;
  double* zz_part = work + FLOW_REDUCE_WORK;
  const int nlast = L->nblocks16[products - 1];
  double* xx_part = zz_part + nlast;
  const double* stop = S + kDone;
  const double c2 = M->contraction * M->contraction;
  MassTiles T;
  for (int j = 0; j < products; ++j) {
    T.rowblocks[j] = L->rowblocks16[j];
    T.nblocks[j] = L->nblocks16[j];
  }
  T.shift = R->e0;
  T.own_lo = R->r0;
  T.own_hi = R->r1;
  float* rho0 = M->work16 - static_cast<ptrdiff_t>(R->e0) * ncomp;
  const int count = 4 + ncomp * R->nhalo;
  const int gp = 1 + grid_for(ncomp * R->nhalo > 0 ? ncomp * R->nhalo : 1,
                              kMassPackBlock, 64);
  const int per = R->recv_len[0] + R->recv_len[1];
  const int gs = grid_for(ncomp * per > 0 ? ncomp * per : 1);
  int rc;
  if ((rc = fill(kNumSlots, 0.0, S, st))) return rc;
  int k = 0;
  auto one = [&]() -> int {
    if (x_is_zero && k == 0) {
      hipLaunchKernelGGL(mass_rho0_kernel, dim3(grid_for(R->r1 - R->r0)),
                         dim3(kBlock), 0, st, A->n, ncomp, b, M->dinv, rho0, stop,
                         R->r0, R->r1);
    } else if (A->kind == 4) {
      hipLaunchKernelGGL(mass_residual_pair_kernel, dim3(A->nblocks), dim3(kBlock),
                         0, st, A->n, A->rowptr, A->cols, A->vals[0], A->rowblocks,
                         A->rowmask, x, A->n, b, M->dinv,
                         reinterpret_cast<float2*>(rho0), stop);
    } else {
      hipLaunchKernelGGL(mass_residual_kernel, dim3(A->nblocks), dim3(kBlock), 0, st,
                         A->rowptr, A->cols, A->vals[0], A->rowblocks, x, b, M->dinv,
                         rho0, stop);
    }
    hipLaunchKernelGGL(shard_mass_pack_kernel, dim3(gp), dim3(kMassPackBlock), 0,
                       st, *R, ncomp, k == 0 ? 1 : 0, nlast, zz_part, xx_part, rho0,
                       C->buf, stop);
    FLOW_CHECK_LAUNCH();
    (void)count;
    if ((rc = exchange_halo(C, R, ncomp, 4, 4, st))) return rc;
    hipLaunchKernelGGL(shard_mass_unpack_kernel, dim3(gs), dim3(kBlock), 0, st, *R,
                       ncomp, k == 0 ? 1 : 0, k, c2, rtol * rtol, atol * atol,
                       C->buf, rho0, S);
    FLOW_CHECK_LAUNCH();
    if (A->kind == 4)
      rc = correction<float2, false>(M, T, x, xbase, zz_part, xx_part, stop, st);
    else
      rc = correction<float, false>(M, T, x, xbase, zz_part, xx_part, stop, st);
    ++k;
    return rc;
  };
  double state[kNumSlots];
  bool started = false;
  while (true) {
    int todo = (!started && first_check > 0) ? first_check + 1 : 1;
    if (!started && first_check == 0) todo = 2;
    started = true;
    if (k + todo > maxit + 1) todo = maxit + 1 - k;
    for (int i = 0; i < todo; ++i)
      if ((rc = one())) return rc;
    if ((rc = read_state(S, state, st))) return rc;
    const double zz = state[kRes2];
    if (state[kDone] == 2.0 || !(zz == zz)) {
      *iters_host = static_cast<int>(state[kConvIt]);
      *resid_host = zz;
      set_error("sharded mass solve broke down (NaN) at correction %d",
                *iters_host);
      return FLOW_NOT_CONVERGED;
    }
    if (state[kDone] == 1.0) {
      *iters_host = static_cast<int>(state[kConvIt]);
      *resid_host = sqrt(zz);
      return FLOW_OK;
    }
    if (state[kDone] == 3.0) {
      *iters_host = static_cast<int>(state[kConvIt]);
      *resid_host = sqrt(zz);
      set_error("sharded mass solve: correction %d contracted by %.3f (no "
                "contraction; the vouched bound is %.3f)", *iters_host,
                state[kTmp], M->contraction);
      return FLOW_NOT_CONVERGED;
    }
    if (k > maxit) {
      *iters_host = maxit;
      *resid_host = sqrt(zz);
      set_error("sharded mass solve did not converge in %d defect corrections: "
                "|z| = %.3e, |x| = %.3e", maxit, sqrt(zz), sqrt(state[kB2]));
      return FLOW_NOT_CONVERGED;
    }
  }
}

}

using namespace flow;

extern "C" int flow_mass_pack(int n, const int* rowptr, const int* diag_idx,
                              const double* vals, void* vals16, void* stream) {
  FLOW_REQUIRE(n > 0 && rowptr && diag_idx && vals && vals16,
               "flow_mass_pack arguments");
  hipLaunchKernelGGL(mass_pack_kernel, dim3(grid_for(n)), dim3(kBlock), 0,
                     as_stream(stream), n, rowptr, diag_idx, vals,
                     static_cast<__half*>(vals16));
  FLOW_CHECK_LAUNCH();
  return FLOW_OK;
}

extern "C" int flow_mass_pack16(int n, int nblocks16, const int* rowblocks16,
                                const int* rowptr, const int* cols,
                                const int* diag_idx, const double* vals,
                                int* cbase16, void* packed16, int* overflow_dev,
                                void* stream) {
  FLOW_REQUIRE(n > 0 && nblocks16 > 0 && rowblocks16 && rowptr && cols &&
                   diag_idx && vals && cbase16 && packed16 && overflow_dev,
               "flow_mass_pack16 arguments");
  hipLaunchKernelGGL(mass_pack16_kernel, dim3(nblocks16), dim3(kBlock), 0,
                     as_stream(stream), rowblocks16, rowptr, cols, diag_idx, vals,
                     cbase16, static_cast<unsigned*>(packed16), overflow_dev);
  FLOW_CHECK_LAUNCH();
  return FLOW_OK;
}

extern "C" int flow_mass_solve(const flow_mass* M, const double* b, double* x,
                               double rtol, double atol, int maxit,
                               int first_check, double* work, size_t work_len,
                               int* iters_host, double* resid_host,
                               void* stream) {
  int rc = mass_check(M);
  if (rc) return rc;
  FLOW_REQUIRE(b && x && work && iters_host && resid_host, "solver pointers");
  FLOW_REQUIRE(rtol >= 0.0 && atol >= 0.0 && maxit >= 1 && first_check >= 0,
               "solver tolerances");
  FLOW_REQUIRE(work_len >= FLOW_REDUCE_WORK + 2 * static_cast<size_t>(M->nblocks16),
               "mass solve workspace too small");
  return mass_solve(M, b, x, nullptr, false, rtol, atol, maxit, first_check, work,
                    iters_host, resid_host, as_stream(stream));
}

__global__ void mass_sum_kernel(int n, const double* __restrict__ a,
                                const double* __restrict__ b,
                                double* __restrict__ y) {
  for (int i = blockIdx.x * blockDim.x + threadIdx.x; i < n;
       i += gridDim.x * blockDim.x)
    y[i] = b ? a[i] + b[i] : a[i];
}

extern "C" int flow_mass_solve_increment(const flow_mass* M, const double* g,
                                         const double* xbase,
                                         const double* delta0, double* x,
                                         double rtol, double atol, int maxit,
                                         int first_check, double* work,
                                         size_t work_len, int* iters_host,
                                         double* resid_host, void* stream) {
  int rc = mass_check(M);
  if (rc) return rc;
  FLOW_REQUIRE(g && xbase && x && work && iters_host && resid_host,
               "solver pointers");
  FLOW_REQUIRE(rtol >= 0.0 && atol >= 0.0 && maxit >= 1 && first_check >= 0,
               "solver tolerances");
  const size_t N = M->A->kind == 4 ? 2 * static_cast<size_t>(M->A->n) : M->A->n;
  const size_t head = FLOW_REDUCE_WORK + 2 * static_cast<size_t>(M->nblocks16);
  FLOW_REQUIRE(work_len >= head + (head & 1) + N, "mass solve workspace too small");
  hipStream_t st = as_stream(stream);
  double* delta = work + head + (head & 1);
  if (delta0) {
    hipLaunchKernelGGL(mass_sum_kernel, dim3(grid_for(N)), dim3(kBlock), 0, st,
                       static_cast<int>(N), delta0, static_cast<const double*>(nullptr),
                       delta);
// ... 84 lines not shown
```

include/flow_hip.h:

```cpp
#ifndef FLOW_HIP_H
#define FLOW_HIP_H

#include <stddef.h>

#ifdef __cplusplus
extern "C" {
#endif

#define FLOW_OK 0
#define FLOW_NOT_CONVERGED 1
#define FLOW_INVALID 2
#define FLOW_HIP_ERROR 3

#define FLOW_SPMV_ROWS_PER_BLOCK 256
#define FLOW_SPMV_NNZ_PER_BLOCK 1022
int flow_spmv_tile_nnz(int kind);

const char* flow_last_error(void);
int flow_abi_version(void);
int flow_launch_count(unsigned long long* count_host);
int flow_graph_mode(int mode, long long auto_rows);
int flow_graph_stats(unsigned long long* stats_host);
int flow_xcd_tile_host(int block, int nblocks);

typedef struct {
  int kind;
  int n;
  int nnz;
  int nblocks;
  const int* rowptr;
  const int* cols;
  const int* rowblocks;
  const double* vals[4];
  const void* matfree;
  const unsigned char* rowmask;
} flow_operator;

int flow_operator_apply(const flow_operator* A, const double* x, double* y,
                        void* stream);
int flow_operator_diag_inv(const flow_operator* A, const int* diag_idx,
                           double* dinv, void* stream);

int flow_profile_spmv_begin(int rows, int max_launches);
int flow_profile_spmv_end(double* total_us, int* launches);
int flow_profile_event_overhead(double* overhead_us, void* stream);
int flow_profile_marker(int id, void* stream);
int flow_profile_stream_copy(size_t n, const double* src, double* dst,
                             void* stream);
int flow_profile_stream_read(size_t n, const double* src, double* sink,
                             void* stream);

int flow_dot_host(int n, const double* x, const double* y, double* work,
                  double* result_host, void* stream);
int flow_scale_rows(int n, const int* rowptr, const double* d, double* vals,
                    void* stream);

int flow_norm_host(int n, const double* x, int kind, double* work,
                   double* result_host, void* stream);
int flow_axpby(int n, double a, const double* x, double b, double* y,
               void* stream);
int flow_vmul(int n, double a, const double* x, const double* y, double* out,
              void* stream);
int flow_fill(int n, double value, double* y, void* stream);
int flow_fingerprint(int nfields, const double* const* x_host,
                     const int* n_host, double* work, double* slots,
                     void* stream);
int flow_read_doubles(const double* dev, int n, double* host, void* stream);
int flow_lincomb(int n, int nterms, const double* coef_host,
                 const double* const* x_host, double* y, void* stream);
int flow_extrapolation_weights(int m, const double* dts_host, double dt,
                               int power, int degree, double* w_host);
int flow_gather_rows(int ncomp, const int* idx, int m, const double* src,
                     int src_stride, double* dst, int dst_stride, void* stream);
#define FLOW_REDUCE_WORK 4096

typedef struct {
  int n;
  int nc;
  const int* agg_ptr;
  const int* agg_dofs;
  const int* agg_of;
  int lda;
  const float* Ainv;
} flow_coarse;

#define FLOW_MG_MAX_LEVELS 8
typedef struct {
  int nlevels;
  flow_operator Ah[FLOW_MG_MAX_LEVELS];
  const double* dinv[FLOW_MG_MAX_LEVELS];
  flow_operator Ps[FLOW_MG_MAX_LEVELS];
  flow_operator R[FLOW_MG_MAX_LEVELS];
  double* r[FLOW_MG_MAX_LEVELS];
  double* x[FLOW_MG_MAX_LEVELS];
  double* t[FLOW_MG_MAX_LEVELS];
  int nc, lda;
  const float* Ainv;
  double omega;
  flow_operator C[FLOW_MG_MAX_LEVELS];
  const int* up_rowblocks[FLOW_MG_MAX_LEVELS];
  int up_nblocks[FLOW_MG_MAX_LEVELS];
} flow_mg;
int flow_two_level_apply(const flow_coarse* coarse, const double* dinv,
                         const double* r, double* z, double* work,
                         void* stream);

int flow_mg_apply(const flow_mg* mg, int n, const double* r, double* z,
                  void* stream);

#define FLOW_ILU_SLICE 64
typedef struct {
  int n, nnz, ncolors;
  int nnz_l, nnz_u;
  int off_l, off_u, off_d, lu_size;
  int max_row;
  int nslices;
  const int* color_ptr_host;
  const int* slice_ptr_host;
  const int* rowptr;
  const int* cols;
  const int* diag;
  const int* src_pos;
  const int* old_of_new;
  const int* new_of_old;
  const int* slice_row;
  const int* l_slice_off;
  const int* l_cols;
  const int* l_pos;
  const int* u_slice_off;
  const int* u_cols;
  const int* u_pos;
} flow_ilu_plan;
typedef struct {
  const flow_ilu_plan* plan;
  int nblocks;
  const double* lu;
  const float* packed;
  int single_vector;
  const void* cycle;
} flow_ilu;
int flow_color_greedy_host(int n, const int* rowptr, const int* cols,
                           int* colour, int* ncolors);
int flow_color_iterate_host(int n, const int* rowptr, const int* cols,
                            int* colour, int* ncolors, int rounds);
int flow_ilu0_factor(const flow_ilu_plan* plan, int nblocks,
                     const double* avals0, const double* avals1, double* lu,
                     void* stream);
int flow_ilu0_pack(const flow_ilu* ilu, float* packed, void* stream);
int flow_ilu0_solve(const flow_ilu* ilu, const double* r, double* z,
                    double* work, void* stream);

#define FLOW_PMG_NNZ_PER_BLOCK 2044
typedef struct {
  int n, nnz, nblocks;
  const int* rowptr;
  const int* cols;
  const int* rowblocks;
  const void* vals;
  const float* diag;
  const float* dinv;
  double lam_min, lam_max;
  const void* cols16;
  const int* cbase;
  const void* packed;
  const unsigned char* idrows;
} flow_pmg_level;
typedef struct {
  flow_pmg_level fine, coarse;
  int pre, post, coarse_steps;
  const int* ends;
  const int* rptr;
  const int* rsrc;
  const unsigned char* bc_fine;
  const unsigned char* bc_coarse;
  float* work;
  int scalar;
} flow_pmg;
int flow_pmg_pack(int n, int nnz, const int* rowptr, const int* diag_idx,
                  const double* a00, const double* a11,
                  const unsigned char* keep, void* vals, float* diag,
                  float* dinv, void* stream);
int flow_pmg_pack1(int n, int nnz, int nblocks, const int* rowblocks,
                   const int* rowptr, const int* cols, const int* diag_idx,
                   const double* a00, const double* a11,
                   const unsigned char* keep, const int* cbase,
                   unsigned char* idrows, void* packed, float* diag,
                   float* dinv, void* stream);
int flow_pmg_cols16(int nblocks, const int* rowblocks, const int* rowptr,
                    const int* cols, int* cbase, void* cols16,
                    int* overflow_dev, void* stream);
int flow_pmg_lambda_max(const flow_pmg_level* level, int iterations, float* work,
                        double* dwork, float* start, double* result_host,
                        void* stream);
int flow_pmg_apply(const flow_pmg* pmg, const double* r, double* z, void* stream);

int flow_aggregate_host(int n, const int* rowptr, const int* cols,
                        const double* vals, double theta,
                        const unsigned char* free_rows, int* agg,
                        int* naggregates);

typedef struct {
  const flow_ilu* fine;
  const flow_ilu* coarse;
  const flow_operator* fine_op;
  const flow_operator* coarse_op;
  int pre, post;
  int coarse_sweeps;
  const int* ends;
  const int* rptr;
  const int* rsrc;
  const unsigned char* bc_fine;
  const unsigned char* bc_coarse;
  const double* rscale;
  double* work;
} flow_tl;
int flow_tl_apply(const flow_tl* tl, const double* r, double* z, void* stream);

typedef struct {
  const flow_operator* A;
  const double* dinv;
  int nblocks16;
  const int* rowblocks16;
  const void* vals16;
  double lam_min, lam_max;
  int steps;
  double contraction;
  float* work16;
  const void* packed16;
  const int* cbase16;
  int work16_rows;
} flow_mass;
int flow_mass_pack(int n, const int* rowptr, const int* diag_idx,
                   const double* vals, void* vals16, void* stream);
int flow_mass_pack16(int n, int nblocks16, const int* rowblocks16,
                     const int* rowptr, const int* cols, const int* diag_idx,
                     const double* vals, int* cbase16, void* packed16,
                     int* overflow_dev, void* stream);
int flow_mass_solve(const flow_mass* M, const double* b, double* x, double rtol,
                    double atol, int maxit, int first_check, double* work,
                    size_t work_len, int* iters_host, double* resid_host,
                    void* stream);

int flow_mass_solve_increment(const flow_mass* M, const double* g,
                              const double* xbase, const double* delta0,
                              double* x, double rtol,
                              double atol, int maxit, int first_check,
                              double* work, size_t work_len, int* iters_host,
                              double* resid_host, void* stream);

int flow_cg_solve(const flow_operator* A, const double* dinv,
                  const flow_coarse* coarse, const flow_mg* mg,
                  const double* b, double* x,
                  double rtol, double atol, int maxit, int check_every,
                  int first_check, double* work, size_t work_len,
                  int* iters_host, double* resid_host, void* stream);
int flow_cg_solve_guarded(const flow_operator* A, const double* dinv,
                          const flow_coarse* coarse, const flow_mg* mg,
                          const double* b, double* x, const double* x_fallback,
                          double rtol, double atol, int maxit, int check_every,
                          int first_check, double* work, size_t work_len,
                          int* iters_host, double* resid_host,
                          int* starts_dropped_host, void* stream);
int flow_bicgstab_solve(const flow_operator* A, const double* dinv,
                        const flow_ilu* ilu, const double* b, double* x,
                        double rtol, double atol, int maxit, int check_every,
                        int first_check, double* work, size_t work_len,
                        int* iters_host, double* resid_host, void* stream);
#define FLOW_GMRES_MAX_RESTART 30
#define FLOW_GMRES_PARTIALS ((FLOW_GMRES_MAX_RESTART + 2) * 1024)
#define FLOW_GMRES_STATE 1280
int flow_gmres_solve(const flow_operator* A, const double* dinv,
                     const flow_ilu* ilu, const flow_pmg* pmg, const double* b,
                     double* x,
                     double rtol, double atol, int maxit, int restart,
                     int x_is_zero, int expected_its, int verify, double* work,
                     size_t work_len, int* iters_host, double* resid_host,
                     void* stream);

typedef int (*flow_allreduce_fn)(void* user, int count);
#define FLOW_PEER_FLAGS 16
typedef struct {
  unsigned long long* flags;
  double* land;
  int land_cap;
  int spin_limit;
  unsigned long long* nb_flags[2];
  double* nb_land[2];
  unsigned long long* seq_host;
} flow_peer;
typedef struct {
  int rank, world;
  double* buf;
  int capacity;
  flow_allreduce_fn allreduce;
  void* user;
  const flow_peer* peer;
} flow_comm;
int flow_peer_alloc(int land_cap, void** base_out, char* handle_out);
int flow_peer_open(const char* handle, void** base_out);
int flow_peer_close(void* mapped_base);
int flow_peer_free(void* base);
int flow_peer_status(const flow_peer* peer, unsigned long long* error_host,
                     void* stream);

#define FLOW_RCCL_ID_BYTES 128
typedef struct {
  void* comm;
  double* buf;
  void* stream;
} flow_rccl_binding;
int flow_rccl_load(const char* librccl_path);
int flow_rccl_unique_id(char* id_host);
int flow_rccl_comm_create(const char* id_host, int rank, int world,
                          void** comm_out);
int flow_rccl_comm_destroy(void* comm);
int flow_rccl_allreduce(void* user, int count);

typedef struct {
  int n;
  int r0, r1;
  int e0, e1;
  int nhalo;
  int send_row[2], send_len[2], send_slot[2];
// ... 506 lines not shown
```

Baseline: 128.0.

## Publish solver convergence state to mapped host mailbox and poll instead of syncing

Result: no change. 129.7, median of 6 (+1.4%).

```diff
diff --git a/flow_amd/_hip.py b/flow_amd/_hip.py
--- a/flow_amd/_hip.py
+++ b/flow_amd/_hip.py
@@ -364,6 +364,8 @@
 SYMBOLS = {
     'flow_abi_version': [],
     'flow_launch_count': [_P(ctypes.c_ulonglong)],
+    'flow_verdict_mode': [_I],
+    'flow_verdict_counts': [_P(ctypes.c_ulonglong)],
     'flow_graph_mode': [_I, ctypes.c_longlong],
     'flow_graph_stats': [_P(ctypes.c_ulonglong)],
     'flow_xcd_tile_host': [_I, _I],
@@ -605,6 +607,16 @@
     return int(n.value)
 
 
+def verdict_mode(mode):
+    check(load_library().flow_verdict_mode(int(mode)))
+
+
+def verdict_counts():
+    n = (ctypes.c_ulonglong * 3)()
+    check(load_library().flow_verdict_counts(n))
+    return tuple(int(v) for v in n)
+
+
 _GRAPHS = {'mode': None}
 
 
diff --git a/flow_amd/csrc/common.h b/flow_amd/csrc/common.h
--- a/flow_amd/csrc/common.h
+++ b/flow_amd/csrc/common.h
@@ -52,6 +52,13 @@
   kBreak, kTarget2, kDone, kConvIt, kIter, kNumSlots = 16
 };
 int read_state(const double* S, double* host, hipStream_t st);
+constexpr int kMailbox = 64;
+struct Verdict {
+  double* mailbox;
+  unsigned long long seq;
+};
+int verdict_begin(Verdict* v);
+int read_published(const Verdict& v, int n, double* host, hipStream_t st);
 int check_comm(const flow_comm* c, long long need);
 int check_rows(const flow_rows* R);
 int exchange(const flow_comm* c, int count);
@@ -135,6 +142,19 @@
   __hip_atomic_store(p, v, __ATOMIC_RELAXED, __HIP_MEMORY_SCOPE_SYSTEM);
 }
 
+__device__ __forceinline__ void publish_values(const double* src, int n,
+                                               Verdict v) {
+  if (v.mailbox == nullptr) return;
+  volatile double* m = v.mailbox;
+  for (int i = 0; i < n; ++i) m[i] = load_scalar(src + i);
+  __threadfence_system();
+  __hip_atomic_store(reinterpret_cast<unsigned long long*>(v.mailbox + kMailbox),
+                     v.seq, __ATOMIC_RELAXED, __HIP_MEMORY_SCOPE_SYSTEM);
+}
+__device__ __forceinline__ void publish_state(const double* S, Verdict v) {
+  publish_values(S, kNumSlots, v);
+}
+
 __device__ __forceinline__ bool stopped(const double* stop) {
   return stop != nullptr && load_scalar(stop) != 0.0;
 }
diff --git a/flow_amd/csrc/krylov_kernels.hip b/flow_amd/csrc/krylov_kernels.hip
--- a/flow_amd/csrc/krylov_kernels.hip
+++ b/flow_amd/csrc/krylov_kernels.hip
@@ -87,9 +87,13 @@
 __global__ __launch_bounds__(kScalarBlock) void cg_scalar_kernel(
     int nparts, int ndelta, int first, const double* __restrict__ gpart,
     const double* __restrict__ rpart, const double* __restrict__ dpart,
-    double rtol2, double atol2, double* __restrict__ S) {
+    double rtol2, double atol2, double* __restrict__ S,
+    Verdict pub = Verdict{nullptr, 0}) {
   __shared__ double wsum[3][kScalarBlock / 64];
-  if (stopped(S + kDone)) return;
+  if (stopped(S + kDone)) {
+    if (threadIdx.x == 0) publish_state(S, pub);
+    return;
+  }
   double g = 0.0, rr = 0.0;
   for (int i = threadIdx.x; i < nparts; i += kScalarBlock) {
     g += load_scalar(gpart + i);
@@ -137,6 +141,7 @@
         store_scalar(S + kConvIt, 0.0);
         store_scalar(S + kRes2, rr);
         store_scalar(S + kDone, 5.0);
+        publish_state(S, pub);
         return;
       }
     } else {
@@ -158,6 +163,7 @@
     store_scalar(S + kAlpha, alpha);
     store_scalar(S + kBeta, beta);
     store_scalar(S + kRes2, rr);
+    publish_state(S, pub);
   }
 }
 
@@ -430,8 +436,8 @@
 
 static int run_batches(const char* solver, const char* norm, int maxit,
                        int first_check, int check_every, const double* S,
-                       hipStream_t st, bool* rejected,
-                       const std::function<int(int)>& iteration,
+                       hipStream_t st, bool* rejected, bool publishes,
+                       const std::function<int(int, const Verdict&)>& iteration,
                        int* iters_host, double* resid_host) {
   if (rejected) *rejected = false;
   double state[kNumSlots];
@@ -440,11 +446,18 @@
     const int batch = (launched == 0 && first_check > 0) ? first_check
                                                          : check_every;
     const int todo = (maxit - launched < batch) ? maxit - launched : batch;
-    for (int k = 0; k < todo; ++k)
-      if ((rc = iteration(launched + k))) return rc;
+    Verdict pub = {nullptr, 0};
+    for (int k = 0; k < todo; ++k) {
+      if (publishes && k + 1 == todo && (rc = verdict_begin(&pub))) return rc;
+      if ((rc = iteration(launched + k, pub))) return rc;
+    }
     FLOW_CHECK_LAUNCH();
     launched += todo;
-    if ((rc = read_state(S, state, st))) return rc;
+    if (pub.mailbox) {
+      if ((rc = read_published(pub, kNumSlots, state, st))) return rc;
+    } else if ((rc = read_state(S, state, st))) {
+      return rc;
+    }
     const double res2 = state[kRes2];
     if (state[kDone] == 2.0 || !(res2 == res2)) {
       *iters_host = static_cast<int>(state[kConvIt]);
@@ -528,7 +541,7 @@
                      dpart, rtol2, atol2, S);
   FLOW_CHECK_LAUNCH();
 
-  auto body = [&]() -> int {
+  auto body = [&](const Verdict& pub) -> int {
     int r;
     if (C) {
       hipLaunchKernelGGL(cg_update_kernel<false>, dim3(gv), dim3(kBlock), 0,
@@ -549,7 +562,7 @@
     }
     if ((r = apply(A, z, w, st, dpart, stop))) return r;
     hipLaunchKernelGGL(cg_scalar_kernel, dim3(1), dim3(kScalarBlock), 0, st,
-                       np, nd, 0, gpart, rpart, dpart, 0.0, 0.0, S);
+                       np, nd, 0, gpart, rpart, dpart, 0.0, 0.0, S, pub);
     FLOW_CHECK_LAUNCH();
     return FLOW_OK;
   };
@@ -560,12 +573,18 @@
     key.pod(0x6367ull);
     key_operator(key, A);
     key.obj(C).obj(M).pod(dinv).pod(x).pod(work).pod(N);
-    if ((rc = replay_prepare(key.h, kReplayCg, st, body, &graph, &graph_nodes))) return rc;
+    if ((rc = replay_prepare(key.h, kReplayCg, st,
+                             [&]() { return body(Verdict{nullptr, 0}); }, &graph,
+                             &graph_nodes)))
+      return rc;
   }
 
   return run_batches(
       "CG", "|B r|", maxit, first_check, check_every, S, st, rejected,
-      [&](int) { return graph ? replay_launch(graph, graph_nodes, st) : body(); },
+      graph == nullptr,
+      [&](int, const Verdict& pub) {
+        return graph ? replay_launch(graph, graph_nodes, st) : body(pub);
+      },
       iters_host, resid_host);
 }
 
@@ -692,7 +711,7 @@
                      rtol2, atol2, partial, S);
   FLOW_CHECK_LAUNCH();
 
-  auto body = [&](int) -> int {
+  auto body = [&](int, const Verdict&) -> int {
     int rc;
     hipLaunchKernelGGL(bicg_p_kernel, dim3(gv), dim3(kBlock), 0, st, N, S, dinv,
                        r, v, p, y);
@@ -716,7 +735,7 @@
     return FLOW_OK;
   };
   return run_batches("BiCGStab", "|r|", maxit, first_check, check_every, S, st,
-                     nullptr, body, iters_host, resid_host);
+                     nullptr, false, body, iters_host, resid_host);
 }
 
 }
@@ -813,13 +832,16 @@
 __global__ __launch_bounds__(kBlock) void gmres_step_kernel(
     int nparts, int j, int last, double beta, double target,
     const double* __restrict__ partial, double* __restrict__ G,
-    double* __restrict__ S) {
+    double* __restrict__ S, flow::Verdict pub) {
   constexpr int ld = kGmresMax + 1;
   __shared__ double val[kGmresMax + 2];
   __shared__ double Hs[kGmresMax * ld];
   __shared__ double nrm[kGmresMax + 1], eta[kGmresMax];
   __shared__ double g[kGmresMax + 1], cs[kGmresMax], sn[kGmresMax], y[kGmresMax];
-  if (stopped(S + kDone)) return;
+  if (stopped(S + kDone)) {
+    if (threadIdx.x == 0) publish_state(S, pub);
+    return;
+  }
   if (beta < 0.0) {
     beta = load_scalar(S + kBeta);
     target = load_scalar(S + kTarget2);
@@ -894,6 +916,7 @@
   if (!(ww == ww) || !(nj > 0.0)) {
     store_scalar(S + kConvIt, static_cast<double>(j));
     store_scalar(S + kDone, 2.0);
+    publish_state(S, pub);
     return;
   }
   const double e2 = ww - sum;
@@ -935,11 +958,13 @@
     if (done) store_scalar(S + kDone, 1.0);
     if (lucky) store_scalar(S + kDone, 3.0);
   }
+  publish_state(S, pub);
 }
 
 __global__ __launch_bounds__(kBlock) void gmres_begin_kernel(
     int nparts, int have_b2, int first, int accept10, double rtol, double atol,
-    const double* __restrict__ partial, double* __restrict__ S) {
+    const double* __restrict__ partial, double* __restrict__ S,
+    Verdict pub = Verdict{nullptr, 0}) {
   double r = 0.0, b = 0.0;
   for (int i = threadIdx.x; i < nparts; i += kBlock) {
     r += load_scalar(partial + i);
@@ -969,6 +994,7 @@
     store_scalar(S + kDone, 2.0);
   else if (beta <= target || (accept10 && beta <= 10.0 * target))
     store_scalar(S + kDone, 4.0);
+  publish_state(S, pub);
 }
 
 __global__ void gmres_drop_start_kernel(int n, const double* __restrict__ S,
@@ -1049,8 +1075,9 @@
 
 static int gmres_cycle(const char* solver, int m, int maxit, int it0,
                        int expected, const double* S, hipStream_t st,
-                       const std::function<int(int, bool)>& arnoldi, int* cols,
-                       double* resid, int* done, int* iters_host,
+                       bool publishes,
+                       const std::function<int(int, bool, const Verdict&)>& arnoldi,
+                       int* cols, double* resid, int* done, int* iters_host,
                        double* resid_host) {
   double state[kNumSlots];
   int enq = 0, rc;
@@ -1061,11 +1088,17 @@
     int plan = expected - (it0 + enq);
     if (plan < 1) plan = 1;
     if (plan > room) plan = room;
+    Verdict pub = {nullptr, 0};
     for (int k = 0; k < plan; ++k, ++enq) {
       const bool last = enq + 1 >= m || it0 + enq + 1 >= maxit;
-      if ((rc = arnoldi(enq, last))) return rc;
-    }
-    if ((rc = read_state(S, state, st))) return rc;
+      if (publishes && k + 1 == plan && (rc = verdict_begin(&pub))) return rc;
+      if ((rc = arnoldi(enq, last, pub))) return rc;
+    }
+    if (pub.mailbox) {
+      if ((rc = read_published(pub, kNumSlots, state, st))) return rc;
+    } else if ((rc = read_state(S, state, st))) {
+      return rc;
+    }
     *cols = static_cast<int>(state[kConvIt]);
     if (state[kDone] == 2.0) {
       *iters_host = it0 + *cols;
@@ -1112,7 +1145,8 @@
                          in, out, stop);
     return FLOW_OK;
   };
-  auto arnoldi = [&](int j, double beta, double target, bool last) -> int {
+  auto arnoldi = [&](int j, double beta, double target, bool last,
+                     const Verdict& pub) -> int {
     int r;
     double* w = V + static_cast<size_t>(j + 1) * N;
     if ((r = precondition(j))) return r;
@@ -1121,7 +1155,7 @@
       return r;
     arnoldi_dots(N, j, w, V, gd, P, Pww, stop, st);
     hipLaunchKernelGGL(gmres_step_kernel, dim3(1), dim3(kBlock), 0, st, gd, j,
-                       last ? 1 : 0, beta, target, P, G, S);
+                       last ? 1 : 0, beta, target, P, G, S, pub);
     FLOW_CHECK_LAUNCH();
     if (!last &&
         (r = gmres_combine_dev(N, j + 1, G + kGCoef, G + kGCw, w, V, w, Pnn, false,
@@ -1144,17 +1178,19 @@
         return rc;
     }
   }
-  auto arnoldi_replayed = [&](int j, bool last) -> int {
-    if (!replay) return arnoldi(j, -1.0, 0.0, last);
+  const Verdict nopub = {nullptr, 0};
+  auto arnoldi_replayed = [&](int j, bool last, const Verdict& pub) -> int {
+    if (!replay) return arnoldi(j, -1.0, 0.0, last, pub);
     KeyHash key = base;
     key.pod(j).pod(last);
     hipGraphExec_t graph = nullptr;
     int nodes = 0, r;
     if ((r = replay_prepare(key.h, kReplayGmres, st,
-                            [&]() { return arnoldi(j, -1.0, 0.0, last); }, &graph,
-                            &nodes)))
+                            [&]() { return arnoldi(j, -1.0, 0.0, last, nopub); },
+                            &graph, &nodes)))
       return r;
-    return graph ? replay_launch(graph, nodes, st) : arnoldi(j, -1.0, 0.0, last);
+    return graph ? replay_launch(graph, nodes, st)
+                 : arnoldi(j, -1.0, 0.0, last, nopub);
   };
 
   if ((rc = fill(kNumSlots, 0.0, S, st))) return rc;
@@ -1178,9 +1214,11 @@
     const int have_b2 = first && !b_is_r0;
     if ((rc = dots(N, have_b2 ? 2 : 1, V, V, b, b, V, V, partial, &np, st)))
       return rc;
+    Verdict begun = {nullptr, 0};
+    if (it >= maxit && !replay && (rc = verdict_begin(&begun))) return rc;
     hipLaunchKernelGGL(gmres_begin_kernel, dim3(1), dim3(kBlock), 0, st, np,
                        have_b2, first ? 1 : 0, claimed ? 1 : 0, rtol, atol,
-                       partial, S);
+                       partial, S, begun);
     if (have_b2)
       hipLaunchKernelGGL(gmres_drop_start_kernel, dim3(gv), dim3(kBlock), 0, st,
                          N, S, b, V, x);
@@ -1188,7 +1226,11 @@
     first = false;
     claimed = false;
     if (it >= maxit) {
-      if ((rc = read_state(S, state, st))) return rc;
+      if (begun.mailbox) {
+        if ((rc = read_published(begun, kNumSlots, state, st))) return rc;
+      } else if ((rc = read_state(S, state, st))) {
+        return rc;
+      }
       resid = state[kBeta];
       if (state[kDone] == 4.0) break;
       *iters_host = it;
@@ -1203,7 +1245,7 @@
     }
 
     int cols, done;
-    if ((rc = gmres_cycle("GMRES", m, maxit, it, expected, S, st,
+    if ((rc = gmres_cycle("GMRES", m, maxit, it, expected, S, st, !replay,
                           arnoldi_replayed, &cols, &resid, &done, iters_host,
                           resid_host)))
       return rc;
diff --git a/flow_amd/csrc/la_internal.h b/flow_amd/csrc/la_internal.h
--- a/flow_amd/csrc/la_internal.h
+++ b/flow_amd/csrc/la_internal.h
@@ -26,14 +26,13 @@
          const double* b1, const double* a2, const double* b2, double* partial,
          int* nparts, hipStream_t st);
 
-constexpr int kMailbox = 64;
 int read_values(const double* dev, int n, double* host, hipStream_t st);
 
 __global__ __launch_bounds__(kBlock) void absmax_kernel(
     int n, const double* __restrict__ x, double* __restrict__ partial);
 __global__ __launch_bounds__(kBlock) void finish_kernel(
     int nparts, int nd, int is_max, const double* __restrict__ partial,
-    double* __restrict__ out);
+    double* __restrict__ out, Verdict pub = Verdict{nullptr, 0});
 __global__ void axpby_kernel(int n, double a, const double* __restrict__ x,
                              double b, double* __restrict__ y);
 __global__ void vmul_kernel(int n, double a, const double* x, const double* y,
@@ -153,4 +152,4 @@
 __global__ __launch_bounds__(flow::kBlock) void gmres_step_kernel(
     int nparts, int j, int last, double beta, double target,
     const double* __restrict__ partial, double* __restrict__ G,
-    double* __restrict__ S);
+    double* __restrict__ S, flow::Verdict pub = flow::Verdict{nullptr, 0});
diff --git a/flow_amd/csrc/la_kernels.hip b/flow_amd/csrc/la_kernels.hip
--- a/flow_amd/csrc/la_kernels.hip
+++ b/flow_amd/csrc/la_kernels.hip
@@ -1,6 +1,10 @@
 #include "common.h"
 #include "csr_stream.h"
 #include "la_internal.h"
+#include "verdict_wait.h"
+
+#include <atomic>
+#include <cstdlib>
 
 namespace flow {
 
@@ -276,7 +280,7 @@
 
 __global__ __launch_bounds__(kBlock) void finish_kernel(
     int nparts, int nd, int is_max, const double* __restrict__ partial,
-    double* __restrict__ out) {
+    double* __restrict__ out, Verdict pub) {
   for (int j = 0; j < nd; ++j) {
     double v = 0.0;
     for (int i = threadIdx.x; i < nparts; i += kBlock) {
@@ -286,6 +290,7 @@
     v = is_max ? block_max(v) : block_sum(v);
     if (threadIdx.x == 0) store_scalar(out + j, v);
   }
+  if (threadIdx.x == 0) publish_values(out, nd, pub);
 }
 
 __global__ void axpby_kernel(int n, double a, const double* __restrict__ x,
@@ -347,14 +352,76 @@
   __threadfence_system();
 }
 
-static int mailbox_of_thread(double** host, double** dev) {
+static int mailbox_of_thread(double** host, double** dev,
+                             VerdictSeq** seq = nullptr) {
   static thread_local double* mailbox = nullptr;
-  if (!mailbox)
+  static thread_local VerdictSeq numbers;
+  if (!mailbox) {
     FLOW_CHECK_HIP(hipHostMalloc(reinterpret_cast<void**>(&mailbox),
-                                 kMailbox * sizeof(double), hipHostMallocMapped));
+                                 (kMailbox + 8) * sizeof(double),
+                                 hipHostMallocMapped));
+    for (int i = 0; i < kMailbox + 8; ++i) mailbox[i] = 0.0;
+  }
   *host = mailbox;
+  if (seq) *seq = &numbers;
   FLOW_CHECK_HIP(
       hipHostGetDevicePointer(reinterpret_cast<void**>(dev), mailbox, 0));
+  return FLOW_OK;
+}
+
+static std::atomic<int> g_verdict_mode{-1};
+static std::atomic<unsigned long long> g_verdict_counts[3];
+constexpr long long kPollBudgetNs = 20 * 1000 * 1000;
+
+static int verdict_mode() {
+  const int m = g_verdict_mode.load(std::memory_order_relaxed);
+  if (m >= 0) return m;
+  const char* pub = getenv("FLOW_AMD_MAILBOX_PUBLISH");
+  if (pub && pub[0] == '0') return 0;
+  const char* poll = getenv("FLOW_AMD_MAILBOX_POLL");
+  return (poll && poll[0] == '0') ? 1 : 2;
+}
+
+int verdict_begin(Verdict* v) {
+  v->mailbox = nullptr;
+  v->seq = 0;
+  if (verdict_mode() == 0) return FLOW_OK;
+  double *mailbox = nullptr, *dev_view = nullptr;
+  VerdictSeq* numbers = nullptr;
+  int rc = mailbox_of_thread(&mailbox, &dev_view, &numbers);
+  if (rc) return rc;
+  v->mailbox = dev_view;
+  v->seq = numbers->next();
+  return FLOW_OK;
+}
+
+int read_published(const Verdict& v, int n, double* host, hipStream_t st) {
+  FLOW_REQUIRE(v.mailbox != nullptr && n >= 1 && n <= kMailbox,
+               "published verdict");
+  double *mailbox = nullptr, *dev_view = nullptr;
+  int rc = mailbox_of_thread(&mailbox, &dev_view);
+  if (rc) return rc;
+  FLOW_REQUIRE(dev_view == v.mailbox, "a verdict is read by the thread it was begun on");
+  const uint64_t* stamp = reinterpret_cast<const uint64_t*>(mailbox + kMailbox);
+  const bool poll = verdict_mode() == 2;
+  hipError_t err = hipSuccess;
+  int status = 0;
+  const VerdictWait w = wait_stamp(
+      stamp, v.seq, poll ? kPollBudgetNs : 0,
+      [&]() {
+        err = hipStreamSynchronize(st);
+        return err == hipSuccess ? 0 : 1;
+      },
+      &status);
+  if (w == kWaitSyncError) FLOW_CHECK_HIP(err);
+  if (w == kWaitLost) {
+    set_error("verdict %llu was not published (the stream is drained, the stamp "
+              "holds %llu)", v.seq,
+              static_cast<unsigned long long>(stamp_load(stamp)));
+    return FLOW_HIP_ERROR;
+  }
+  ++g_verdict_counts[w == kWaitPolled ? 0 : (poll ? 1 : 2)];
+  for (int i = 0; i < n; ++i) host[i] = static_cast<volatile double*>(mailbox)[i];
   return FLOW_OK;
 }
 
@@ -395,13 +462,22 @@
   return read_slots(S, slot, slot, host, &again, st);
 }
 
+static int finish_host(double* work, int nparts, int is_max, double* host,
+                       hipStream_t st) {
+  double* S = work + 3 * kRedBlocks;
+  Verdict pub;
+  int rc = verdict_begin(&pub);
+  if (rc) return rc;
+  hipLaunchKernelGGL(finish_kernel, dim3(1), dim3(kBlock), 0, st, nparts, 1,
+                     is_max, work, S, pub);
+  FLOW_CHECK_LAUNCH();
+  if (pub.mailbox) return read_published(pub, 1, host, st);
+  return read_slot(S, 0, host, st);
+}
+
 int sum_partials_host(double* work, int nparts, double* host, hipStream_t st) {
   FLOW_REQUIRE(nparts >= 1 && nparts <= kRedBlocks, "partial count");
-  double* S = work + 3 * kRedBlocks;
-  hipLaunchKernelGGL(finish_kernel, dim3(1), dim3(kBlock), 0, st, nparts, 1, 0,
-                     work, S);
-  FLOW_CHECK_LAUNCH();
-  return read_slot(S, 0, host, st);
+  return finish_host(work, nparts, 0, host, st);
 }
 
 __global__ void mailbox_copy_kernel(int n, const double* __restrict__ src,
@@ -429,6 +505,17 @@
 
 extern "C" const char* flow_last_error(void) { return g_error; }
 extern "C" int flow_abi_version(void) { return 30; }
+
+extern "C" int flow_verdict_mode(int mode) {
+  FLOW_REQUIRE(mode >= -1 && mode <= 2, "verdict mode (-1, 0, 1, 2)");
+  flow::g_verdict_mode.store(mode);
+  return FLOW_OK;
+}
+extern "C" int flow_verdict_counts(unsigned long long* counts_host) {
+  FLOW_REQUIRE(counts_host != nullptr, "flow_verdict_counts argument");
+  for (int i = 0; i < 3; ++i) counts_host[i] = flow::g_verdict_counts[i].load();
+  return FLOW_OK;
+}
 
 namespace flow {
 unsigned long long g_launches = 0;
@@ -499,11 +586,7 @@
   int np = 0;
   int rc = dots(n, 1, x, y, x, y, x, y, work, &np, st);
   if (rc) return rc;
-  double* S = work + 3 * kRedBlocks;
-  hipLaunchKernelGGL(finish_kernel, dim3(1), dim3(kBlock), 0, st, np, 1, 0, work,
-                     S);
-  FLOW_CHECK_LAUNCH();
-  return read_slot(S, 0, result_host, st);
+  return finish_host(work, np, 0, result_host, st);
 }
 
 extern "C" int flow_norm_host(int n, const double* x, int kind, double* work,
@@ -511,7 +594,6 @@
   FLOW_REQUIRE(n > 0 && x && work && result_host, "norm arguments");
   FLOW_REQUIRE(kind == 0 || kind == 1, "norm kind");
   hipStream_t st = as_stream(stream);
-  double* S = work + 3 * kRedBlocks;
   if (kind == 0) {
     int rc = flow_dot_host(n, x, x, work, result_host, stream);
     if (rc) return rc;
@@ -520,10 +602,8 @@
   }
   const int g = grid_for(n, kBlock * 4, kRedBlocks);
   hipLaunchKernelGGL(absmax_kernel, dim3(g), dim3(kBlock), 0, st, n, x, work);
-  hipLaunchKernelGGL(finish_kernel, dim3(1), dim3(kBlock), 0, st, g, 1, 1, work,
-                     S);
-  FLOW_CHECK_LAUNCH();
-  return read_slot(S, 0, result_host, st);
+  FLOW_CHECK_LAUNCH();
+  return finish_host(work, g, 1, result_host, st);
 }
 
 extern "C" int flow_axpby(int n, double a, const double* x, double b, double* y,
diff --git a/flow_amd/csrc/mass_kernels.hip b/flow_amd/csrc/mass_kernels.hip
--- a/flow_amd/csrc/mass_kernels.hip
+++ b/flow_amd/csrc/mass_kernels.hip
@@ -200,9 +200,12 @@
 __global__ __launch_bounds__(kMassScalarBlock) void mass_scalar_kernel(
     int nparts, const double* __restrict__ zz_part,
     const double* __restrict__ xx_part, double contraction2, double rtol2,
-    double atol2, double* __restrict__ S) {
+    double atol2, double* __restrict__ S, Verdict pub = Verdict{nullptr, 0}) {
   __shared__ double wsum[2][kMassScalarBlock / 64];
-  if (stopped(S + kDone)) return;
+  if (stopped(S + kDone)) {
+    if (threadIdx.x == 0) publish_state(S, pub);
+    return;
+  }
   double z0 = 0.0, z1 = 0.0, x0 = 0.0, x1 = 0.0;
   int i = threadIdx.x;
   for (; i + kMassScalarBlock < nparts; i += 2 * kMassScalarBlock) {
@@ -249,6 +252,7 @@
   store_scalar(S + kIter, k);
   store_scalar(S + kRes2, zz);
   store_scalar(S + kB2, xx);
+  publish_state(S, pub);
 }
 
 __global__ void mass_pack_kernel(int n, const int* __restrict__ rowptr,
@@ -388,6 +392,7 @@
   const double c2 = M->contraction * M->contraction;
   int rc;
   if ((rc = fill(kNumSlots, 0.0, S, st))) return rc;
+  Verdict pub = {nullptr, 0};
   auto one = [&]() -> int {
     if (x_is_zero) {
       hipLaunchKernelGGL(mass_rho0_kernel, dim3(grid_for(A->n)), dim3(kBlock), 0,
@@ -419,7 +424,7 @@
     if (rc) return rc;
     hipLaunchKernelGGL(mass_scalar_kernel, dim3(1), dim3(kMassScalarBlock), 0, st,
                        M->nblocks16, zz_part, xx_part, c2, rtol * rtol, atol * atol,
-                       S);
+                       S, pub);
     FLOW_CHECK_LAUNCH();
     return FLOW_OK;
   };
@@ -448,10 +453,17 @@
   while (true) {
     const int batch = (launched == 0 && first_check > 0) ? first_check : 1;
     const int todo = (maxit - launched < batch) ? maxit - launched : batch;
-    for (int k = 0; k < todo; ++k)
+    pub = Verdict{nullptr, 0};
+    for (int k = 0; k < todo; ++k) {
+      if (!replay && k + 1 == todo && (rc = verdict_begin(&pub))) return rc;
       if ((rc = one_replayed())) return rc;
+    }
     launched += todo;
-    if ((rc = read_state(S, state, st))) return rc;
+    if (pub.mailbox) {
+      if ((rc = read_published(pub, kNumSlots, state, st))) return rc;
+    } else if ((rc = read_state(S, state, st))) {
+      return rc;
+    }
     const double zz = state[kRes2];
     if (state[kDone] == 2.0 || !(zz == zz)) {
       *iters_host = static_cast<int>(state[kConvIt]);
diff --git a/flow_amd/csrc/verdict_wait.h b/flow_amd/csrc/verdict_wait.h
--- /dev/null
+++ b/flow_amd/csrc/verdict_wait.h
@@ -0,0 +1,48 @@
+#pragma once
+#include <chrono>
+#include <cstdint>
+
+namespace flow {
+
+struct VerdictSeq {
+  uint64_t last = 0;
+  uint64_t next() { return ++last; }
+};
+
+inline uint64_t stamp_load(const uint64_t* stamp) {
+  return __atomic_load_n(stamp, __ATOMIC_ACQUIRE);
+}
+
+enum VerdictWait {
+  kWaitPolled = 0,
+  kWaitDrained = 1,
+  kWaitSyncError = 2,
+  kWaitLost = 3
+};
+
+template <class Sync>
+inline VerdictWait wait_stamp(const uint64_t* stamp, uint64_t expect,
+                              long long budget_ns, Sync&& sync,
+                              int* sync_status) {
+  *sync_status = 0;
+  if (budget_ns > 0) {
+    const auto t0 = std::chrono::steady_clock::now();
+    while (true) {
+      for (int i = 0; i < 256; ++i) {
+        if (stamp_load(stamp) == expect) return kWaitPolled;
+#if defined(__x86_64__) || defined(__i386__)
+        __builtin_ia32_pause();
+#endif
+      }
+      const auto dt = std::chrono::steady_clock::now() - t0;
+      if (std::chrono::duration_cast<std::chrono::nanoseconds>(dt).count() >=
+          budget_ns)
+        break;
+    }
+  }
+  *sync_status = sync();
+  if (*sync_status != 0) return kWaitSyncError;
+  return stamp_load(stamp) == expect ? kWaitDrained : kWaitLost;
+}
+
+}
diff --git a/include/flow_hip.h b/include/flow_hip.h
--- a/include/flow_hip.h
+++ b/include/flow_hip.h
@@ -19,6 +19,8 @@
 const char* flow_last_error(void);
 int flow_abi_version(void);
 int flow_launch_count(unsigned long long* count_host);
+int flow_verdict_mode(int mode);
+int flow_verdict_counts(unsigned long long* counts_host);
 int flow_graph_mode(int mode, long long auto_rows);
 int flow_graph_stats(unsigned long long* stats_host);
 int flow_xcd_tile_host(int block, int nblocks);
```
